# BirchKwok/lynsedb

Hardware: AMD Instinct MI355X
Metric: queries/sec, FLAT-IP 10000000x768 float32, batch=256, k=10 (higher is better)
Workload: dtype f32

## Files before the change

### include/lynse_hip.h

```cpp
#ifndef LYNSE_HIP_H
#define LYNSE_HIP_H

#include <stddef.h>
#include <stdint.h>

#ifdef __cplusplus
extern "C" {
#endif

#define LYNSE_HIP_ABI_VERSION 1

enum {
    LYNSE_OK = 0,
    LYNSE_ERR_INVALID_ARGUMENT = 1,
    LYNSE_ERR_DIMENSION_MISMATCH = 2,
    LYNSE_ERR_UNKNOWN_METRIC = 3,
    LYNSE_ERR_NOT_FINALIZED = 4,
    LYNSE_ERR_OUT_OF_MEMORY = 5,
    LYNSE_ERR_DEVICE = 6,
    LYNSE_ERR_INTERNAL = 7,
    LYNSE_ERR_INDEX_NOT_BUILT = 8,
    LYNSE_ERR_UNSUPPORTED = 9,
    LYNSE_ERR_TIMEOUT = 10
};
// ... 163 lines not shown
int lynse_hip_spann_replica_count(const lynse_hip_ivf *h, uint32_t *replica_count);
int lynse_hip_ivf_insert_f32(lynse_hip_ivf *h, const float *rows, uint64_t n);
int lynse_hip_ivf_delete_rows(lynse_hip_ivf *h, const uint64_t *row_ids, uint64_t n_ids);
int lynse_hip_ivf_assign_f32(lynse_hip_ivf *h, const float *rows, uint64_t n, uint32_t *out_assignments);
int lynse_hip_ivf_destroy(lynse_hip_ivf *h);
uint64_t lynse_hip_ivf_len(const lynse_hip_ivf *h);
uint32_t lynse_hip_ivf_nlist(const lynse_hip_ivf *h);
int lynse_hip_ivf_export(const lynse_hip_ivf *h, float *centroids, uint32_t *assignments,
                         uint64_t *offsets, uint32_t *original_ids);
int lynse_hip_ivf_set_row_map(lynse_hip_ivf *h, uint64_t stride, uint64_t offset);
int lynse_hip_ivf_set_routing(lynse_hip_ivf *h, int ivfflat_routing);
int lynse_hip_ivf_set_fused_search(lynse_hip_ivf *h, int on);
int lynse_hip_ivf_search_f32(lynse_hip_ivf *h, const float *queries, uint64_t nq, uint32_t k,
                             uint32_t nprobe, uint64_t *out_rows, float *out_dists,
                             uint32_t *out_counts);
int lynse_hip_ivf_build_device(const float *d_rows, uint64_t n, uint32_t dim, uint32_t nlist,
                               uint32_t max_iter, int metric, int l2_partitions, int device,
                               lynse_hip_ivf **out);
int lynse_hip_ivf_load_device(const float *d_rows, uint64_t n, uint32_t dim, const float *centroids,
                              uint32_t nlist, const uint32_t *assignments, int metric, int device,
                              lynse_hip_ivf **out);
int lynse_hip_ivf_search_f32_device(lynse_hip_ivf *h, const float *d_queries, uint64_t nq, uint32_t k,
                                    uint32_t nprobe, uint64_t *d_out_rows, float *d_out_dists,
                                    uint32_t *d_out_counts);
int lynse_hip_ivf_search_metric_f32(lynse_hip_ivf *h, const float *queries, uint64_t nq, uint32_t k,
                                    uint32_t nprobe, int metric, uint64_t *out_rows, float *out_dists,
                                    uint32_t *out_counts);
int lynse_hip_ivf_search_filtered_f32(lynse_hip_ivf *h, const float *queries, uint64_t nq, uint32_t k,
                                      uint32_t nprobe, const uint64_t *subset_rows, uint64_t n_subset,
                                      uint64_t *out_rows, float *out_dists, uint32_t *out_counts);
int lynse_hip_ivf_profile_enable(lynse_hip_ivf *h, int on);
int lynse_hip_ivf_profile_get(lynse_hip_ivf *h, lynse_hip_profile *out, int reset);

typedef struct lynse_hip_comm lynse_hip_comm;
int lynse_hip_comm_load_rccl(const char *path );
int lynse_hip_comm_unique_id(uint8_t *id128);
int lynse_hip_comm_create(const uint8_t *id128, int rank, int world, int device, lynse_hip_comm **out);
int lynse_hip_comm_destroy(lynse_hip_comm *c);
int lynse_hip_comm_rank(const lynse_hip_comm *c);
int lynse_hip_comm_world(const lynse_hip_comm *c);
int lynse_hip_comm_ranks_seen(lynse_hip_comm *c, int *out);
int lynse_hip_flat_search_sharded_f32_device(lynse_hip_flat *h, lynse_hip_comm *c, const float *d_queries,
                                             uint64_t nq, uint32_t k, int metric, uint64_t *d_out_rows,
                                             float *d_out_dists, uint32_t *d_out_counts);
int lynse_hip_flat_search_sharded_packed_u64_device(lynse_hip_flat *h, lynse_hip_comm *c,
                                                    const uint64_t *d_query_words, uint64_t nq, uint32_t k,
                                                    int metric, uint64_t *d_out_rows, float *d_out_dists,
                                                    uint32_t *d_out_counts);
int lynse_hip_ivf_search_sharded_f32_device(lynse_hip_ivf *h, lynse_hip_comm *c, const float *d_queries, uint64_t nq,
                                            uint32_t k, uint32_t nprobe, uint64_t *d_out_rows, float *d_out_dists,
                                            uint32_t *d_out_counts);
typedef int (*lynse_hip_reduce_fn)(void *ctx, void *buf, uint64_t count, int dtype);
int lynse_hip_ivf_kmeans_sharded(const float *rows_local, uint64_t n_local, int rows_on_device, uint64_t n_global,
                                 uint32_t rank, uint32_t world, uint32_t dim, uint32_t nlist, uint32_t max_iter, int metric,
                                 int device, lynse_hip_comm *c, lynse_hip_reduce_fn reduce, void *reduce_ctx,
                                 float *out_centroids, uint32_t *out_assignments, uint32_t *out_k);

int lynse_hip_ivf_build_sharded_device(const float *d_rows_local, uint64_t n_local, uint64_t n_global, uint32_t rank,
                                       uint32_t world, uint32_t dim, uint32_t nlist, uint32_t max_iter, int metric,
                                       int ivfflat_routing, int device, lynse_hip_comm *c, lynse_hip_reduce_fn reduce,
                                       void *reduce_ctx, lynse_hip_ivf **out);

typedef struct lynse_hip_ticket lynse_hip_ticket;
int lynse_hip_flat_search_submit_f32_device(lynse_hip_flat *h, lynse_hip_comm *c, const float *d_queries, uint64_t nq,
                                            uint32_t k, int metric, uint64_t *d_out_rows, float *d_out_dists,
                                            uint32_t *d_out_counts, lynse_hip_ticket **out);
int lynse_hip_flat_search_submit_packed_u64_device(lynse_hip_flat *h, lynse_hip_comm *c,
                                                   const uint64_t *d_query_words, uint64_t nq, uint32_t k, int metric,
                                                   uint64_t *d_out_rows, float *d_out_dists, uint32_t *d_out_counts,
                                                   lynse_hip_ticket **out);
int lynse_hip_flat_search_wait(lynse_hip_ticket *t);
int lynse_hip_set_wait_timeout_ms(uint32_t ms);

typedef struct lynse_hip_ivf_ticket lynse_hip_ivf_ticket;
int lynse_hip_ivf_search_submit_f32_device(lynse_hip_ivf *h, lynse_hip_comm *c, const float *d_queries, uint64_t nq, uint32_t k,
                                           uint32_t nprobe, uint64_t *d_out_rows, float *d_out_dists, uint32_t *d_out_counts,
                                           lynse_hip_ivf_ticket **out);
int lynse_hip_ivf_search_wait(lynse_hip_ivf_ticket *t);
int lynse_hip_ivf_ticket_stats(lynse_hip_ivf *h, uint64_t *out);

int lynse_hip_flat_coarse_scores(lynse_hip_flat *h, const float *queries, uint64_t nq, int metric, int coarse,
                                 float *out_scores, float *out_bound, int *out_form);


typedef struct lynse_hip_sparse lynse_hip_sparse;
int lynse_hip_sparse_normalize(const uint64_t *indptr , const uint32_t *indices, const float *values, uint64_t n,
                               uint64_t *out_indptr , uint32_t *out_indices, float *out_values);
int lynse_hip_sparse_create(int device, lynse_hip_sparse **out);
int lynse_hip_sparse_destroy(lynse_hip_sparse *h);
int lynse_hip_sparse_set_rows(lynse_hip_sparse *h, const uint64_t *indptr , const uint32_t *indices,
                              const float *values, uint64_t n);
int lynse_hip_sparse_len(lynse_hip_sparse *h, uint64_t *out_rows, uint64_t *out_nnz);
uint64_t lynse_hip_sparse_hbm_bytes(lynse_hip_sparse *h);
int lynse_hip_sparse_search(lynse_hip_sparse *h, const uint64_t *q_indptr , const uint32_t *q_indices,
                            const float *q_values, uint64_t nq, uint32_t k,
                            const uint64_t *bitset_words , uint64_t n_words,
                            uint64_t *out_rows , float *out_scores, uint32_t *out_counts ,
                            uint64_t *out_passed );
int lynse_hip_sparse_profile_enable(lynse_hip_sparse *h, int on);
int lynse_hip_sparse_profile_get(lynse_hip_sparse *h, lynse_hip_profile *out, int reset);


int lynse_hip_filter_tombstoned_limit(const uint64_t *ids, const float *dists, uint64_t n,
                                      const uint64_t *tombstones, uint64_t n_tombstones, uint64_t limit,
                                      uint64_t *out_ids, float *out_dists, uint64_t *out_n);
int lynse_hip_merge_row_results(const uint64_t *left_ids, const float *left_dists, uint64_t n_left,
                                const uint64_t *right_ids, const float *right_dists, uint64_t n_right,
                                uint64_t limit, int metric, uint64_t *out_ids, float *out_dists,
                                uint64_t *out_n);
int lynse_hip_encode_search_result(const uint64_t *ids, const float *dists, uint32_t n,
                                   const uint8_t *fields_json, uint32_t fields_len, uint8_t *buf,
                                   uint64_t cap, uint64_t *out_len);
int lynse_hip_decode_search_result(const uint8_t *buf, uint64_t len, uint64_t offset, uint64_t *out_ids,
                                   float *out_dists, uint32_t cap_n, uint32_t *out_n,
                                   uint64_t *fields_offset, uint32_t *fields_len, uint64_t *next_offset);

#ifdef __cplusplus
}
#endif
#endif
```

### lynsedb_amd/_lib.py

```python
from __future__ import annotations

import ctypes as C
from pathlib import Path

try:
    import torch as _torch
except ImportError:
    _torch = None

_HERE = Path(__file__).resolve().parent
LIB_PATH = _HERE / "liblynse_hip.so"

OK = 0
ERR_INVALID_ARGUMENT, ERR_DIMENSION_MISMATCH, ERR_UNKNOWN_METRIC, ERR_NOT_FINALIZED = 1, 2, 3, 4
ERR_OUT_OF_MEMORY, ERR_DEVICE, ERR_INTERNAL, ERR_INDEX_NOT_BUILT, ERR_UNSUPPORTED, ERR_TIMEOUT = 5, 6, 7, 8, 9, 10

METRIC_IP, METRIC_L2, METRIC_COSINE, METRIC_HAMMING, METRIC_JACCARD, METRIC_DICE, METRIC_TANIMOTO = range(7)
METRIC_L1, METRIC_CHEBYSHEV, METRIC_CANBERRA, METRIC_BRAY_CURTIS = 7, 8, 9, 10
IPFORM_AUTO, IPFORM_SINGLE, IPFORM_BATCH8 = 0, 1, 2


class Profile(C.Structure):
    _fields_ = [("searches", C.c_uint64), ("scan_launches", C.c_uint64), ("scan_us", C.c_double),
                ("scan_rows", C.c_uint64), ("scan_bytes", C.c_uint64), ("total_us", C.c_double),
# ... 45 lines not shown
    "lynse_hip_flat_drop_rabitq": (C.c_int, [_vp]),
    "lynse_hip_flat_search_rabitq_f32": (C.c_int, [_vp, _vp, C.c_uint64, C.c_uint32, C.c_int, C.c_uint32, _vp, _vp, _vp]),
    "lynse_hip_flat_rabitq_stage_times": (C.c_int, [_vp, _vp, C.c_int]),
    "lynse_hip_rabitq_sign_words": (C.c_int, [C.c_uint64, C.c_uint64, _vp]),
    "lynse_hip_flat_search_range_f32": (C.c_int, [_vp, _vp, C.c_uint64, _vp, C.c_uint32, C.c_int, _vp, C.c_uint64, _vp, _vp, _vp, _vp]),
    "lynse_hip_flat_set_dtype": (C.c_int, [_vp, C.c_int]),
    "lynse_hip_flat_append_f16_bits": (C.c_int, [_vp, _vp, C.c_uint64]),
    "lynse_hip_flat_search_filtered_f32": (C.c_int, [_vp, _vp, C.c_uint64, C.c_uint32, C.c_int, _vp, C.c_uint64, _vp, _vp, _vp]),
    "lynse_hip_flat_search_filtered_bitset_f32": (C.c_int, [_vp, _vp, C.c_uint64, C.c_uint32, C.c_int, _vp, C.c_uint64, _vp, _vp, _vp]),
    "lynse_hip_flat_search_f32_device": (C.c_int, [_vp, _vp, C.c_uint64, C.c_uint32, C.c_int, _vp, _vp, _vp, _vp]),
    "lynse_hip_flat_search_packed_u64": (C.c_int, [_vp, _vp, C.c_uint64, C.c_uint32, C.c_int, _vp, _vp, _vp]),
    "lynse_hip_flat_search_packed_u64_device": (C.c_int, [_vp, _vp, C.c_uint64, C.c_uint32, C.c_int, _vp, _vp, _vp, _vp]),
    "lynse_hip_flat_profile_enable": (C.c_int, [_vp, C.c_int]),
    "lynse_hip_flat_profile_get": (C.c_int, [_vp, C.POINTER(Profile), C.c_int]),
    "lynse_hip_flat_coarse_state": (C.c_int, [_vp, C.POINTER(C.c_int), _u64p]),
    "lynse_hip_flat_bpm_rows": (C.c_uint64, [_vp]),
    "lynse_hip_flat_prepare": (C.c_int, [_vp, C.c_int, C.c_uint64]),
    "lynse_hip_flat_hbm_bytes": (C.c_uint64, [_vp]),
    "lynse_hip_flat_set_fused_search": (C.c_int, [_vp, C.c_int]),
    "lynse_hip_flat_set_plan": (C.c_int, [_vp, C.c_uint32, C.c_uint32, C.c_uint32]),
    "lynse_hip_compute_distance": (C.c_int, [_vp, _vp, C.c_uint32, C.c_int, C.c_int, _f32p]),
    "lynse_hip_top_k_search": (C.c_int, [_vp, _vp, C.c_uint64, C.c_uint32, C.c_uint32, C.c_int, C.c_int, _vp, _vp, _u32p]),
    "lynse_hip_pack_binary_f32": (C.c_int, [_vp, C.c_uint64, C.c_uint32, C.c_int, _vp]),
    "lynse_hip_merge_topk": (C.c_int, [_vp, _vp, _vp, C.c_uint32, C.c_uint32, C.c_uint32, C.c_int, _vp, _vp, _u32p]),
    "lynse_hip_merge_topk_device": (C.c_int, [_vp, C.c_uint64, C.c_uint64, C.c_uint64, C.c_uint64, C.c_uint32,
                                              C.c_uint64, C.c_uint32, C.c_int, _vp, _vp, _vp, _vp]),
    "lynse_hip_ivf_build": (C.c_int, [_vp, C.c_uint64, C.c_uint32, C.c_uint32, C.c_uint32, C.c_int, C.c_int, C.c_int, C.POINTER(_vp)]),
    "lynse_hip_ivf_load": (C.c_int, [_vp, C.c_uint64, C.c_uint32, _vp, C.c_uint32, _vp, C.c_int, C.c_int, C.POINTER(_vp)]),
    "lynse_hip_ivf_load_binary": (C.c_int, [_vp, C.c_uint64, C.c_uint32, _vp, C.c_uint32, _vp, C.c_int, _vp, C.c_int, C.POINTER(_vp)]),
    "lynse_hip_ivf_thresholds": (C.c_int, [_vp, _vp, C.POINTER(C.c_int)]),
    "lynse_hip_ivf_destroy": (C.c_int, [_vp]),
    "lynse_hip_ivf_len": (C.c_uint64, [_vp]),
    "lynse_hip_ivf_nlist": (C.c_uint32, [_vp]),
    "lynse_hip_ivf_export": (C.c_int, [_vp, _vp, _vp, _vp, _vp]),
    "lynse_hip_ivf_set_row_map": (C.c_int, [_vp, C.c_uint64, C.c_uint64]),
    "lynse_hip_ivf_set_routing": (C.c_int, [_vp, C.c_int]),
    "lynse_hip_ivf_set_fused_search": (C.c_int, [_vp, C.c_int]),
    "lynse_hip_ivf_search_f32": (C.c_int, [_vp, _vp, C.c_uint64, C.c_uint32, C.c_uint32, _vp, _vp, _vp]),
    "lynse_hip_ivf_build_device": (C.c_int, [_vp, C.c_uint64, C.c_uint32, C.c_uint32, C.c_uint32, C.c_int, C.c_int, C.c_int, C.POINTER(_vp)]),
    "lynse_hip_ivf_load_device": (C.c_int, [_vp, C.c_uint64, C.c_uint32, _vp, C.c_uint32, _vp, C.c_int, C.c_int, C.POINTER(_vp)]),
    "lynse_hip_ivf_search_f32_device": (C.c_int, [_vp, _vp, C.c_uint64, C.c_uint32, C.c_uint32, _vp, _vp, _vp]),
    "lynse_hip_ivf_search_metric_f32": (C.c_int, [_vp, _vp, C.c_uint64, C.c_uint32, C.c_uint32, C.c_int, _vp, _vp, _vp]),
    "lynse_hip_ivf_search_filtered_f32": (C.c_int, [_vp, _vp, C.c_uint64, C.c_uint32, C.c_uint32, _vp, C.c_uint64, _vp, _vp, _vp]),
    "lynse_hip_ivf_profile_enable": (C.c_int, [_vp, C.c_int]),
    "lynse_hip_filter_tombstoned_limit": (C.c_int, [_vp, _vp, C.c_uint64, _vp, C.c_uint64, C.c_uint64, _vp, _vp, C.POINTER(C.c_uint64)]),
    "lynse_hip_merge_row_results": (C.c_int, [_vp, _vp, C.c_uint64, _vp, _vp, C.c_uint64, C.c_uint64, C.c_int, _vp, _vp, C.POINTER(C.c_uint64)]),
    "lynse_hip_encode_search_result": (C.c_int, [_vp, _vp, C.c_uint32, _vp, C.c_uint32, _vp, C.c_uint64, C.POINTER(C.c_uint64)]),
    "lynse_hip_decode_search_result": (C.c_int, [_vp, C.c_uint64, C.c_uint64, _vp, _vp, C.c_uint32, C.POINTER(C.c_uint32),
                                                C.POINTER(C.c_uint64), C.POINTER(C.c_uint32), C.POINTER(C.c_uint64)]),
    "lynse_hip_ivf_profile_get": (C.c_int, [_vp, C.POINTER(Profile), C.c_int]),
    "lynse_hip_ivf_insert_f32": (C.c_int, [_vp, _vp, C.c_uint64]),
    "lynse_hip_ivf_search_sharded_f32_device": (C.c_int, [_vp, _vp, _vp, C.c_uint64, C.c_uint32, C.c_uint32, _vp, _vp, _vp]),
    "lynse_hip_ivf_delete_rows": (C.c_int, [_vp, _vp, C.c_uint64]),
    "lynse_hip_ivf_assign_f32": (C.c_int, [_vp, _vp, C.c_uint64, _vp]),
    "lynse_hip_ivf_build_sq8": (C.c_int, [_vp, C.c_uint64, C.c_uint32, C.c_uint32, C.c_uint32, C.c_int, C.c_int, C.POINTER(_vp)]),
    "lynse_hip_ivf_load_sq8": (C.c_int, [_vp, C.c_uint64, C.c_uint32, _vp, C.c_uint32, _vp, _vp, _vp, C.c_int, C.c_int, C.POINTER(_vp)]),
    "lynse_hip_ivf_sq8_params": (C.c_int, [_vp, _vp, _vp]),
    "lynse_hip_ivf_sq8_stage_times": (C.c_int, [_vp, _vp, C.c_int]),
    "lynse_hip_spann_build": (C.c_int, [_vp, C.c_uint64, C.c_uint32, C.c_uint32, C.c_uint32, C.c_int, C.c_uint32, C.c_int, C.c_int, C.POINTER(_vp)]),
    "lynse_hip_spann_load": (C.c_int, [_vp, C.c_uint64, C.c_uint32, _vp, C.c_uint32, _vp, _vp, C.c_uint32, C.c_int, _vp, _vp, C.c_int, C.POINTER(_vp)]),
    "lynse_hip_spann_postings": (C.c_int, [_vp, _vp, _vp, _vp]),
    "lynse_hip_spann_replica_count": (C.c_int, [_vp, _vp]),
    "lynse_hip_comm_load_rccl": (C.c_int, [C.c_char_p]),
    "lynse_hip_comm_unique_id": (C.c_int, [_vp]),
    "lynse_hip_comm_create": (C.c_int, [_vp, C.c_int, C.c_int, C.c_int, C.POINTER(_vp)]),
    "lynse_hip_comm_destroy": (C.c_int, [_vp]),
    "lynse_hip_comm_rank": (C.c_int, [_vp]),
    "lynse_hip_comm_world": (C.c_int, [_vp]),
    "lynse_hip_comm_ranks_seen": (C.c_int, [_vp, C.POINTER(C.c_int)]),
    "lynse_hip_flat_search_sharded_f32_device": (C.c_int, [_vp, _vp, _vp, C.c_uint64, C.c_uint32, C.c_int, _vp, _vp, _vp]),
    "lynse_hip_flat_search_sharded_packed_u64_device": (C.c_int, [_vp, _vp, _vp, C.c_uint64, C.c_uint32, C.c_int, _vp, _vp, _vp]),
    "lynse_hip_flat_search_submit_f32_device": (C.c_int, [_vp, _vp, _vp, C.c_uint64, C.c_uint32, C.c_int, _vp, _vp, _vp, C.POINTER(_vp)]),
    "lynse_hip_flat_search_submit_packed_u64_device": (C.c_int, [_vp, _vp, _vp, C.c_uint64, C.c_uint32, C.c_int, _vp, _vp, _vp, C.POINTER(_vp)]),
    "lynse_hip_flat_search_wait": (C.c_int, [_vp]),
    "lynse_hip_set_wait_timeout_ms": (C.c_int, [C.c_uint32]),
    "lynse_hip_ivf_search_submit_f32_device": (C.c_int, [_vp, _vp, _vp, C.c_uint64, C.c_uint32, C.c_uint32, _vp, _vp, _vp, C.POINTER(_vp)]),
    "lynse_hip_ivf_search_wait": (C.c_int, [_vp]),
    "lynse_hip_ivf_ticket_stats": (C.c_int, [_vp, _vp]),
    "lynse_hip_ivf_kmeans_sharded": (C.c_int, [_vp, C.c_uint64, C.c_int, C.c_uint64, C.c_uint32, C.c_uint32, C.c_uint32, C.c_uint32, C.c_uint32, C.c_int, C.c_int,
                                              _vp, _vp, _vp, _vp, _vp, C.POINTER(C.c_uint32)]),
    "lynse_hip_ivf_build_sharded_device": (C.c_int, [_vp, C.c_uint64, C.c_uint64, C.c_uint32, C.c_uint32, C.c_uint32, C.c_uint32, C.c_uint32, C.c_int, C.c_int, C.c_int,
                                                    _vp, _vp, _vp, C.POINTER(_vp)]),
    "lynse_hip_flat_coarse_scores": (C.c_int, [_vp, _vp, C.c_uint64, C.c_int, C.c_int, _vp, _vp, C.POINTER(C.c_int)]),
    "lynse_hip_sparse_normalize": (C.c_int, [_vp, _vp, _vp, C.c_uint64, _vp, _vp, _vp]),
    "lynse_hip_sparse_create": (C.c_int, [C.c_int, C.POINTER(_vp)]),
    "lynse_hip_sparse_destroy": (C.c_int, [_vp]),
    "lynse_hip_sparse_set_rows": (C.c_int, [_vp, _vp, _vp, _vp, C.c_uint64]),
    "lynse_hip_sparse_len": (C.c_int, [_vp, _u64p, _u64p]),
    "lynse_hip_sparse_hbm_bytes": (C.c_uint64, [_vp]),
    "lynse_hip_sparse_search": (C.c_int, [_vp, _vp, _vp, _vp, C.c_uint64, C.c_uint32, _vp, C.c_uint64, _vp, _vp, _vp, _vp]),
    "lynse_hip_sparse_profile_enable": (C.c_int, [_vp, C.c_int]),
    "lynse_hip_sparse_profile_get": (C.c_int, [_vp, C.POINTER(Profile), C.c_int]),
}

REDUCE_FN = C.CFUNCTYPE(C.c_int, C.c_void_p, C.c_void_p, C.c_uint64, C.c_int)

if not LIB_PATH.exists():
    raise ImportError(
        f"{LIB_PATH} is missing: the HIP extension has not been built and lynsedb_amd has no CPU "
        "fallback. Run `make -C lynsedb_amd/csrc` (hipcc --offload-arch=gfx950).")

lib = C.CDLL(str(LIB_PATH))
for _name, (_res, _args) in SIGNATURES.items():
    _fn = getattr(lib, _name)
    _fn.restype = _res
    _fn.argtypes = _args

if lib.lynse_hip_abi_version() != 1:
    raise ImportError("liblynse_hip.so ABI version mismatch; rebuild it")


class LynseHipError(RuntimeError):
    def __init__(self, code: int, message: str):
        super().__init__(message)
        self.code = code


class LynseUnsupportedError(LynseHipError, NotImplementedError):
    """LYNSE_ERR_UNSUPPORTED: valid in the reference, outside what this library implements (e.g. the metric 'l1')."""


def last_error() -> str:
    buf = C.create_string_buffer(1024)
    lib.lynse_hip_last_error(buf, 1024)
    return buf.value.decode("utf-8", "replace")


def check(code: int) -> None:
    if code == OK:
        return
    msg = last_error() or f"lynse_hip error {code}"
    if code in (ERR_INVALID_ARGUMENT, ERR_DIMENSION_MISMATCH, ERR_UNKNOWN_METRIC):
        raise ValueError(msg)
    if code == ERR_OUT_OF_MEMORY:
        raise MemoryError(msg)
    if code == ERR_UNSUPPORTED:
        raise LynseUnsupportedError(code, msg)
    if code == ERR_TIMEOUT:
        raise TimeoutError(msg)
    raise LynseHipError(code, msg)


def device_count() -> int:
    n = C.c_int(0)
    rc = lib.lynse_hip_device_count(C.byref(n))
    return n.value if rc == OK else 0
```

### lynsedb_amd/core.py

```python
from __future__ import annotations

import ctypes as C
import os
from pathlib import Path
from typing import Iterable, Optional, Sequence

import numpy as np

from . import _lib
from ._lib import check, lib

_METRIC_IS_BINARY = {_lib.METRIC_HAMMING, _lib.METRIC_JACCARD, _lib.METRIC_DICE, _lib.METRIC_TANIMOTO}


def visible_devices() -> list:
    v = os.environ.get("LYNSE_HIP_DEVICES", "").strip()
    if v:
        try:
            devs = [int(x) for x in v.split(",") if x.strip() != ""]
        except ValueError:
            raise ValueError(f"LYNSE_HIP_DEVICES must be a comma-separated list of device ordinals, got {v!r}") from None
        if not devs or min(devs) < 0:
            raise ValueError(f"LYNSE_HIP_DEVICES must name at least one non-negative device ordinal, got {v!r}")
        return devs
# ... 472 lines not shown
        rows, dists, counts = self.search_filtered_batch_arrays(q.reshape(1, -1), k, metric, subset_rows)
        c = int(counts[0])
        return rows[0, :c].astype(np.uint32), dists[0, :c].copy()

    def search_packed_arrays(self, query_words, k: int, metric):
        m = metric if isinstance(metric, int) else metric_from_str(metric)
        qw = np.ascontiguousarray(query_words, dtype=np.uint64)
        if qw.ndim == 1:
            qw = qw.reshape(1, -1)
        nq, k = qw.shape[0], int(k)
        rows = np.empty((nq, max(k, 1)), np.uint64)
        dists = np.empty((nq, max(k, 1)), np.float32)
        counts = np.zeros(nq, np.uint32)
        check(lib.lynse_hip_flat_search_packed_u64(self._h, _ptr(qw), nq, k, m, _ptr(rows), _ptr(dists), _ptr(counts)))
        return rows[:, :k], dists[:, :k], counts

    def search(self, query, k: int = 10, metric: str = "ip"):
        m = metric_from_str(metric)
        q = _f32(query, 1, "query")
        rows, dists, counts = self.search_batch_arrays(q.reshape(1, -1), k, m)
        c = int(counts[0])
        return rows[0, :c].astype(np.uint32), dists[0, :c].copy()

    def batch_search(self, queries, k: int = 10, metric: str = "ip"):
        m = metric_from_str(metric)
        rows, dists, counts = self.search_batch_arrays(queries, k, m)
        return [(rows[i, :int(c)].astype(np.uint32), dists[i, :int(c)].copy()) for i, c in enumerate(counts)]

    def search_device(self, d_queries, k: int, metric, d_rows, d_dists, d_counts, stream=None):
        m = metric if isinstance(metric, int) else metric_from_str(metric)
        nq = d_queries.shape[0]
        _sync_producer(d_queries)
        check(lib.lynse_hip_flat_search_f32_device(
            self._h, C.c_void_p(d_queries.data_ptr()), nq, int(k), m, C.c_void_p(d_rows.data_ptr()),
            C.c_void_p(d_dists.data_ptr()), C.c_void_p(d_counts.data_ptr()),
            C.c_void_p(stream) if stream else None))

    def search_packed_device(self, d_qwords, k: int, metric, d_rows, d_dists, d_counts, stream=None):
        m = metric if isinstance(metric, int) else metric_from_str(metric)
        nq = d_qwords.shape[0]
        _sync_producer(d_qwords)
        check(lib.lynse_hip_flat_search_packed_u64_device(
            self._h, C.c_void_p(d_qwords.data_ptr()), nq, int(k), m, C.c_void_p(d_rows.data_ptr()),
            C.c_void_p(d_dists.data_ptr()), C.c_void_p(d_counts.data_ptr()),
            C.c_void_p(stream) if stream else None))

    def search_submit(self, d_queries, k: int, metric, d_rows, d_dists, d_counts, comm=None) -> "SearchTicket":
        m = metric if isinstance(metric, int) else metric_from_str(metric)
        if _lib.METRIC_HAMMING <= m <= _lib.METRIC_TANIMOTO and d_queries.is_floating_point():
            if comm is not None:
                raise ValueError("sharded searches of a binary metric take packed u64 query words")
            self.search_device(d_queries, k, m, d_rows, d_dists, d_counts)
            return SearchTicket(None, None)
        _sync_producer(d_queries)
        t = C.c_void_p()
        fn = lib.lynse_hip_flat_search_submit_packed_u64_device if _lib.METRIC_HAMMING <= m <= _lib.METRIC_TANIMOTO else lib.lynse_hip_flat_search_submit_f32_device
        check(fn(self._h, comm, C.c_void_p(d_queries.data_ptr()), d_queries.shape[0], int(k), m, C.c_void_p(d_rows.data_ptr()),
                 C.c_void_p(d_dists.data_ptr()), C.c_void_p(d_counts.data_ptr()), C.byref(t)))
        return SearchTicket(t, (d_queries, d_rows, d_dists, d_counts))

    def profile_enable(self, on=True) -> None:
        check(lib.lynse_hip_flat_profile_enable(self._h, int(on)))

    def profile_get(self, reset: bool = True) -> dict:
        p = _lib.Profile()
        check(lib.lynse_hip_flat_profile_get(self._h, C.byref(p), 1 if reset else 0))
        return {f: getattr(p, f) for f, _ in _lib.Profile._fields_}

    def prepare(self, metric, nq: int = 256) -> None:
        m = metric if isinstance(metric, int) else metric_from_str(metric)
        check(lib.lynse_hip_flat_prepare(self._h, m, int(nq)))

    def hbm_bytes(self) -> int:
        return int(lib.lynse_hip_flat_hbm_bytes(self._h))

    def coarse_scores(self, queries, metric, coarse: str = "i8"):
        q = np.ascontiguousarray(np.atleast_2d(queries), dtype=np.float32)
        m = metric if isinstance(metric, int) else metric_from_str(metric)
        scores = np.empty((q.shape[0], len(self)), np.float32)
        bound = np.empty(q.shape[0], np.float32)
        form = C.c_int(0)
        check(lib.lynse_hip_flat_coarse_scores(self._h, _ptr(q), q.shape[0], m, 1 if coarse in ("i8", "int8", 1, True) else 0, _ptr(scores), _ptr(bound), C.byref(form)))
        return scores, bound, form.value

    def coarse_state(self) -> dict:
        strikes, rows = C.c_int(0), C.c_uint64(0)
        check(lib.lynse_hip_flat_coarse_state(self._h, C.byref(strikes), C.byref(rows)))
        return {"i8c_strikes": strikes.value, "sq8_rows": rows.value, "bpm_rows": int(lib.lynse_hip_flat_bpm_rows(self._h))}


class SearchTicket:

    def __init__(self, handle, keep, ivf: bool = False):
        self._t, self._keep, self._ivf = handle, keep, ivf

    def wait(self) -> None:
        t, self._t = self._t, None
        if t is not None:
            try:
                check((lib.lynse_hip_ivf_search_wait if self._ivf else lib.lynse_hip_flat_search_wait)(t))
            finally:
                self._keep = None

    def __del__(self):
        try:
            self.wait()
        except Exception:
            pass


class IvfFlatIndex:

    def __init__(self, handle, dim: int, sq8: bool = False):
        self._h = handle
        self._dim = dim
        self._sq8 = sq8

    def profile_enable(self, on=True) -> None:
        check(lib.lynse_hip_ivf_profile_enable(self._h, int(on)))

    def profile_get(self, reset: bool = True) -> dict:
        p = _lib.Profile()
        check(lib.lynse_hip_ivf_profile_get(self._h, C.byref(p), 1 if reset else 0))
        return {f: getattr(p, f) for f, _ in _lib.Profile._fields_}

    def __del__(self):
        h, self._h = getattr(self, "_h", None), None
        if h:
            lib.lynse_hip_ivf_destroy(h)

    @staticmethod
    def build(path, data, dim: int, n_partitions: int = 256, n_iters: int = 20, metric: str = "ip",
              device: Optional[int] = None, l2_partitions: bool = True, quantizer: Optional[str] = None) -> "IvfFlatIndex":
        m = metric if isinstance(metric, int) else metric_from_str(metric)
        a = _f32(data, 2, "data")
        if a.shape[1] != dim:
            raise ValueError(f"data dimension mismatch: expected {dim}, got {a.shape[1]}")
        if n_partitions <= 0:
            raise IOError("IVF partition count must be greater than zero")
        if quantizer is not None and str(quantizer).lower() != "sq8":
            raise NotImplementedError(f"IVF quantizer {quantizer!r} is outside this path (sq8 and the binary metrics are built)")
        if a.shape[0] < n_partitions and quantizer is None:
            raise IOError("IVF requires at least as many vectors as partitions")
        h = C.c_void_p()
        dev = default_device() if device is None else int(device)
        if quantizer is not None:
            check(lib.lynse_hip_ivf_build_sq8(_ptr(a), a.shape[0], dim, n_partitions, n_iters, m, dev, C.byref(h)))
            return IvfFlatIndex(h, dim, sq8=True)
        if m >= 3:
            l2_partitions = False
        check(lib.lynse_hip_ivf_build(_ptr(a), a.shape[0], dim, n_partitions, n_iters, m,
                                      1 if l2_partitions else 0, dev, C.byref(h)))
        return IvfFlatIndex(h, dim)

    @staticmethod
    def build_device(d_rows, dim: int, n_partitions: int = 256, n_iters: int = 20, metric: str = "ip",
                     l2_partitions: bool = True) -> "IvfFlatIndex":
        m = metric if isinstance(metric, int) else metric_from_str(metric)
        if d_rows.dim() != 2 or d_rows.shape[1] != dim or not d_rows.is_contiguous():
            raise ValueError("rows must be a contiguous (n, dim) float32 device tensor")
        _sync_producer(d_rows)
        h = C.c_void_p()
        check(lib.lynse_hip_ivf_build_device(C.c_void_p(d_rows.data_ptr()), d_rows.shape[0], dim, n_partitions, n_iters, m,
                                             1 if l2_partitions else 0, d_rows.device.index or 0, C.byref(h)))
        return IvfFlatIndex(h, dim)

# ... 1003 lines not shown
```

### lynsedb_amd/csrc/kernels.h

```cpp
#pragma once

#include "common.h"
#include <utility>

namespace lynse {

typedef _Float16 half8 __attribute__((ext_vector_type(8)));
typedef _Float16 half4 __attribute__((ext_vector_type(4)));
typedef float f32x16 __attribute__((ext_vector_type(16)));
typedef uint32_t u32x4 __attribute__((ext_vector_type(4)));
typedef float f32x4 __attribute__((ext_vector_type(4)));

#define LY_INF __builtin_huge_valf()

__device__ __forceinline__ float hsum8(float a) {
    float t = __fadd_rn(a, __shfl_xor(a, 4, 8));
    t = __fadd_rn(t, __shfl_xor(t, 1, 8));
    t = __fadd_rn(t, __shfl_xor(t, 2, 8));
    return t;
}

__device__ __forceinline__ float exact_score_f16seq(int metric, const float* __restrict__ q, const float* __restrict__ v_as_f32,
                                                    uint32_t D, int g) {
    const _Float16* __restrict__ v = reinterpret_cast<const _Float16*>(v_as_f32);
// ... 1956 lines not shown
                    volatile uint32_t* flag = reinterpret_cast<volatile uint32_t*>(const_cast<char*>(stv));
                    bool ok = fs_grid_sync(gs, gs + 2, gridDim.x, flag, tid);
                    if (stamp && tid == 0) stamp[2] = __builtin_amdgcn_s_memtime();
                    if (ok) {
                        for (uint32_t q = blockIdx.x; q < ea->nq; q += gridDim.x)
                            fused_sample_threshold<NW * 64>(ea->cand + (size_t)q * ea->cap, gridDim.x * (2 * WR * 2), ea->k, ea->marg2[q], METRIC, ea->ip_form,
                                                            ea->Qf + (size_t)q * ea->D, ea->V, ea->ld, ea->D, ea->thr_out + q, const_cast<char*>(stv),
                                                            const_cast<char*>(stq), tid);
                        if (stamp && tid == 0) stamp[3] = __builtin_amdgcn_s_memtime();
                        ok = fs_grid_sync(gs + 1, gs + 2, gridDim.x, flag, tid);
                        if (stamp && tid == 0) stamp[4] = __builtin_amdgcn_s_memtime();
                    }
                    if (!ok) return;
                    load_qc_thr(ea->thr, ea->nq);
                    if (stamp && tid == 0) stamp[5] = __builtin_amdgcn_s_memtime();
                }
            }
            if constexpr (!DEFER) s_in_tile = 0;
            tile += gridDim.x;
        }
        if constexpr (DEFER) {
            if (g == G) break;
            if (tile_done) load_frags(0, 0);
            ly_static_for<HK / 16 - 1>([&](auto kkc) {
                constexpr int kk = decltype(kkc)::value, cur = kk & 1;
                load_frags(kk + 1, cur ^ 1);
                __builtin_amdgcn_sched_barrier(0);
                ly_static_for<TR>([&](auto ic) {
                    group_at(std::integral_constant<int, cur>{}, ic);
                    slot_pieces(TR + kk * TR + decltype(ic)::value);
                });
                __builtin_amdgcn_sched_barrier(0);
            });
            q_advance();
            v_advance();
            pend_done = ++s_in_tile == a.nslab;
            if (pend_done) s_in_tile = 0;
        }
        if (timing) {
            asm volatile("" ::"v"(acc[0][0][0]));
            const unsigned long long t = __builtin_amdgcn_s_memtime(); t_comp += t - tp; tp = t;
        }
    }
#ifdef LYNSE_EXPERIMENTS
    if (timing && lane == 0) {
        unsigned long long* o = a.dbg + ((size_t)blockIdx.x * NW + wave) * 4;
        o[0] = t_wait; o[1] = t_bar; o[2] = (t_iq << 32) | (t_iv & 0xffffffffull); o[3] = t_comp;
    }
#endif
    if (!TILED) {
        const EpiArgsPtr ea = epi_args();
        if (FS && (ea->debug_flags & 128) && tid == 0) reinterpret_cast<unsigned long long*>(ea->gsync + 64)[(size_t)blockIdx.x * 8 + 6] = __builtin_amdgcn_s_memtime();
        if (ea->seg && (hi == 0 || DENSE)) {
#pragma unroll
            for (int j = 0; j < TQ; ++j) {
                const uint32_t n = qchunk + wq * (TQ * 32) + j * 32 + l32;
                const uint32_t sgm = DENSE ? (blockIdx.x * WR + wr) * 2 + hi : blockIdx.x * WR + wr;
                if (n < ea->nq) ea->segcnt[(size_t)n * ea->nseg + sgm] = (uint8_t)((segpk >> (8 * j)) & 0xffu);
            }
        }
    }
    asm volatile("s_waitcnt vmcnt(0)" ::: "memory");
}

template <typename T>
__global__ void __launch_bounds__(256) k_sq8_minmax(const T* __restrict__ V, uint32_t ld, uint32_t D, uint64_t n,
                                                    uint32_t* __restrict__ omin, uint32_t* __restrict__ omax,
                                                    const float* __restrict__ row_scale = nullptr) {
    const uint64_t rows_per_block = (n + gridDim.y - 1) / gridDim.y;
    const uint64_t r0 = (uint64_t)blockIdx.y * rows_per_block, r1 = r0 + rows_per_block < n ? r0 + rows_per_block : n;
    const uint32_t d = blockIdx.x * 256 + threadIdx.x;
    if (d >= D) return;
    float mn = LY_INF, mx = -LY_INF;
    for (uint64_t r = r0; r < r1; ++r) {
        const float v = row_scale ? __fmul_rn((float)V[r * ld + d], row_scale[r]) : (float)V[r * ld + d];
        if (v < mn) mn = v;
        if (v > mx) mx = v;
    }
    atomicMin(&omin[d], f32_to_ord(mn));
    atomicMax(&omax[d], f32_to_ord(mx));
}

__global__ void __launch_bounds__(256) k_sq8_scales(const uint32_t* __restrict__ omin, const uint32_t* __restrict__ omax, uint32_t D,
                                                    float* __restrict__ mins, float* __restrict__ scales) {
    const uint32_t d = blockIdx.x * 256 + threadIdx.x;
    if (d >= D) return;
    const float mn = ord_to_f32(omin[d]), mx = ord_to_f32(omax[d]);
    const float range = __fsub_rn(mx, mn);
    mins[d] = mn;
    scales[d] = range > 1e-30f ? __fdiv_rn(255.0f, range) : 0.0f;
}

__global__ void __launch_bounds__(256) k_mm_changed(const uint32_t* __restrict__ now, const uint32_t* __restrict__ before, uint32_t n, uint32_t* __restrict__ flag) {
    const uint32_t i = blockIdx.x * 256 + threadIdx.x;
    if (i < n && now[i] != before[i]) atomicOr(flag, 1u);
}

__global__ void __launch_bounds__(256) k_vec_minmax(const float* __restrict__ x, uint64_t n, uint32_t* __restrict__ omin, uint32_t* __restrict__ omax,
                                                    uint32_t ncopies) {
    float mn = LY_INF, mx = -LY_INF;
    for (uint64_t i = (uint64_t)blockIdx.x * blockDim.x + threadIdx.x; i < n; i += (uint64_t)gridDim.x * blockDim.x) {
        const float v = x[i];
        if (v < mn) mn = v;
        if (v > mx) mx = v;
    }
    for (int o = 32; o > 0; o >>= 1) { mn = fminf(mn, __shfl_xor(mn, o, 64)); mx = fmaxf(mx, __shfl_xor(mx, o, 64)); }
    if ((threadIdx.x & 63) == 0)
        for (uint32_t j = 0; j < ncopies; ++j) { atomicMin(omin + j, f32_to_ord(mn)); atomicMax(omax + j, f32_to_ord(mx)); }
}

__device__ __forceinline__ int sq8_code(float v, float mn, float sc) {
    float q = roundf(__fmul_rn(__fsub_rn(v, mn), sc));
    if (!(q == q)) return 0;
    q = q < 0.0f ? 0.0f : (q > 255.0f ? 255.0f : q);
    return (int)q;
}

template <typename T>
__global__ void __launch_bounds__(256) k_sq8_quantize(const T* __restrict__ V, uint32_t ld, uint32_t D, uint64_t n,
                                                      const float* __restrict__ mins, const float* __restrict__ scales,
                                                      int8_t* __restrict__ out, uint32_t ld8, int* __restrict__ sums,
                                                      int* __restrict__ sums2, uint32_t* __restrict__ stats,
                                                      const float* __restrict__ extra_col = nullptr, uint32_t n_extra = 0,
                                                      const float* __restrict__ row_scale = nullptr) {
    const int lane = threadIdx.x & 63;
    const uint64_t wave = ((uint64_t)blockIdx.x * blockDim.x + threadIdx.x) >> 6;
    const uint64_t nwaves = ((uint64_t)gridDim.x * blockDim.x) >> 6;
    uint32_t a1max = 0, a2max = 0, nonfinite = 0;
    float e2max = 0.0f;
    for (uint64_t row = wave; row < n; row += nwaves) {
        int s1 = 0, s2 = 0, l1 = 0;
        float e2 = 0.0f, e1 = 0.0f;
        for (uint32_t d = lane; d < ld8; d += 64) {
            int c = 0;
            if (d < D || (extra_col && d < D + n_extra)) {
                const float v = d < D ? (row_scale ? __fmul_rn((float)V[row * ld + d], row_scale[row]) : (float)V[row * ld + d]) : extra_col[row];
                if (!(fabsf(v) < LY_INF)) nonfinite += 1;
                const int code = sq8_code(v, mins[d], scales[d]);
                c = code - 128;
                s1 += c;
                s2 += c * c;
                l1 += c < 0 ? -c : c;
                const float e = __fsub_rn(__fmul_rn(__fsub_rn(v, mins[d]), scales[d]), (float)code);
                const float ea = fabsf(e);
                if (ea == ea) { e2 = __fmaf_rn(e, e, e2); e1 += ea; }
            }
            out[row * ld8 + d] = (int8_t)c;
        }
        for (int o = 32; o > 0; o >>= 1) {
            s1 += __shfl_xor(s1, o, 64); s2 += __shfl_xor(s2, o, 64); l1 += __shfl_xor(l1, o, 64);
            e2 += __shfl_xor(e2, o, 64); e1 += __shfl_xor(e1, o, 64);
        }
        if (lane == 0 && sums) { sums[row] = s1; sums2[row] = s2; }
        a1max = a1max > (uint32_t)l1 ? a1max : (uint32_t)l1;
        a2max = a2max > (uint32_t)s2 ? a2max : (uint32_t)s2;
        const float e2b = (e2 + 1.22e-4f * e1 + (float)(D + n_extra) * 3.8e-9f) * 1.00002f;
        e2max = e2b > e2max ? e2b : e2max;
    }
    for (int o = 32; o > 0; o >>= 1) nonfinite += __shfl_xor(nonfinite, o, 64);
    if (lane == 0 && stats) {
        atomicMax(&stats[0], a1max);
        if (nonfinite) atomicAdd(&stats[1], nonfinite);
        atomicMax(&stats[2], a2max);
        atomicMax(&stats[3], __float_as_uint(e2max));
    }
}

__global__ void __launch_bounds__(256) k_sq8_prep_queries(const float* __restrict__ Q, uint32_t D, uint32_t qpad, uint32_t nslab,
                                                          const float* __restrict__ mins, const float* __restrict__ scales,
                                                          int8_t* __restrict__ img, float* __restrict__ qconst, float* __restrict__ thr,
                                                          uint32_t* __restrict__ count, uint32_t* __restrict__ overflow, int ip) {
    __shared__ int red[2][4];
    const uint32_t q = blockIdx.x;
    const int tid = threadIdx.x, lane = tid & 63, wave = tid >> 6;
    int s1 = 0, s2 = 0;
    const uint32_t total = nslab * 128;
    for (uint32_t i = tid; i < total; i += 256) {
        int c = 0;
        if (i < D) {
            c = sq8_code(Q[(size_t)q * D + i], mins[i], scales[i]) - 128;
            s1 += c;
            s2 += c * c;
        }
        const uint32_t s = i / 128, k = i % 128, l = k >> 4, e = k & 15, p = l ^ ((q >> 1) & 7);
        img[(((size_t)s * qpad + q) * 8 + p) * 16 + e] = (int8_t)c;
    }
    for (int o = 32; o > 0; o >>= 1) { s1 += __shfl_xor(s1, o, 64); s2 += __shfl_xor(s2, o, 64); }
    if (lane == 0) { red[0][wave] = s1; red[1][wave] = s2; }
    __syncthreads();
    if (tid == 0) {
        s1 = red[0][0] + red[0][1] + red[0][2] + red[0][3];
        s2 = red[1][0] + red[1][1] + red[1][2] + red[1][3];
        const int c = ip ? 128 * s1 + 16384 * (int)D : s2;
        qconst[q] = __builtin_bit_cast(float, c);
        thr[q] = ip ? -LY_INF : LY_INF;
        count[q] = 0u;
        overflow[q] = 0u;
    }
}

struct I8cPrepArgs {
    const float* Q;
    uint32_t D, qpad, nslab;
    uint32_t nq;
    const float *mins, *scales;
    uint32_t a1;
    uint32_t a2sq;
    float eps2;
    float vmax;
    int8_t* img;
    float *sq, *bq, *marg2, *thr;
    uint32_t *count, *overflow;
    uint32_t* gsync;
    int aug;
    int l2n;
    int cosine;
    const int8_t* codes;
    uint32_t ld8, n_rows, tile_rows, dyn_ks, seed_rows;
    int *dyn_thr, *dyn_slot, *dyn_marg;
};

__global__ void __launch_bounds__(256) k_i8c_prep_queries(I8cPrepArgs a) {
    __shared__ double red[5][4];
    __shared__ float s_sq;
    __shared__ int s_slot[32];
    extern __shared__ __attribute__((aligned(16))) int8_t s_u[];
    const uint32_t q = blockIdx.x;
    const int tid = threadIdx.x, lane = tid & 63, wave = tid >> 6;
    if (a.nq && q >= a.nq) {
        for (uint32_t i = tid; i < a.nslab * 128; i += 256) a.img[((size_t)(i / 128) * a.qpad + q) * 128 + (i % 128)] = 0;
        return;
    }
    const float* qv = a.Q + (size_t)q * a.D;
    const uint32_t DA = a.D + (uint32_t)a.aug;
    double qrn = 1.0;
    if (a.cosine) {
        __shared__ double rs[4];
        double t = 0.0;
        for (uint32_t i = tid; i < a.D; i += 256) { const double o = (double)qv[i]; t += o * o; }
        for (int o = 32; o > 0; o >>= 1) t += __shfl_xor(t, o, 64);
        if (lane == 0) rs[wave] = t;
        __syncthreads();
        t = (rs[0] + rs[1]) + (rs[2] + rs[3]);
        qrn = t > 0.0 ? 1.0 / sqrt(t) : 0.0;
        __syncthreads();
    }
    auto qel = [&](uint32_t i) -> double {
        if (a.cosine) return (double)qv[i] * qrn;
        if (!a.aug) return (double)qv[i];
        return i < a.D ? 2.0 * (double)qv[i] : -1.0 / (double)a.aug;
    };
    double wmax = 0.0, sw = 0.0, swabs = 0.0, sqm = 0.0, s2 = 0.0, sw2 = 0.0;
    for (uint32_t i = tid; i < DA; i += 256) {
        const double x = qel(i);
        const float sc = a.scales[i];
        const double w = sc > 0.0f ? x / (double)sc : 0.0;
        wmax = fmax(wmax, fabs(w));
        sw += w;
        swabs += fabs(w);
        sw2 += w * w;
        sqm += x * (double)a.mins[i];
        if (i < a.D) { const double o = (double)qv[i]; s2 += o * o; }
    }
    for (int o = 32; o > 0; o >>= 1) {
        wmax = fmax(wmax, __shfl_xor(wmax, o, 64));
        sw += __shfl_xor(sw, o, 64);
        swabs += __shfl_xor(swabs, o, 64);
        sqm += __shfl_xor(sqm, o, 64);
        s2 += __shfl_xor(s2, o, 64);
        sw2 += __shfl_xor(sw2, o, 64);
    }
    __shared__ double red2[2][4];
    if (lane == 0) { red[0][wave] = wmax; red[1][wave] = sw; red[2][wave] = swabs; red[3][wave] = sqm; red[4][wave] = s2; red2[0][wave] = sw2; }
    __syncthreads();
    if (tid == 0) {
        wmax = fmax(fmax(red[0][0], red[0][1]), fmax(red[0][2], red[0][3]));
        float sq = 1.0f;
        if (wmax > 0.0 && wmax < 1.0e30) {
            sq = (float)(wmax / 127.0);
            if ((double)sq * 127.0 < wmax) sq = nextafterf(sq, LY_INF);
            if (!(sq > 0.0f)) sq = 1.1754944e-38f;
        }
        s_sq = sq;
    }
    __syncthreads();
    const double inv = 1.0 / (double)s_sq;
    const uint32_t total = a.nslab * 128;
    double eta2 = 0.0;
    for (uint32_t i = tid; i < total; i += 256) {
        int u = 0;
        if (i < DA) {
            const float sc = a.scales[i];
            const double w = sc > 0.0f ? qel(i) / (double)sc : 0.0;
            const double t = w * inv;
            double r = rint(t);
            r = r < -127.0 ? -127.0 : (r > 127.0 ? 127.0 : r);
            u = (r == r) ? (int)r : 0;
            const double eta = t - (double)u;
            if (eta == eta) eta2 += eta * eta;
        }
        const uint32_t s = i / 128, k = i % 128, l = k >> 4, e = k & 15, p = l ^ ((q >> 1) & 7);
        a.img[(((size_t)s * a.qpad + q) * 8 + p) * 16 + e] = (int8_t)u;
        if (a.dyn_thr) s_u[i] = (int8_t)u;
    }
    for (int o = 32; o > 0; o >>= 1) eta2 += __shfl_xor(eta2, o, 64);
    if (lane == 0) red2[1][wave] = eta2;
    __syncthreads();
    if (tid == 0) {
        wmax = fmax(fmax(red[0][0], red[0][1]), fmax(red[0][2], red[0][3]));
        sw = (red[1][0] + red[1][1]) + (red[1][2] + red[1][3]);
        swabs = (red[2][0] + red[2][1]) + (red[2][2] + red[2][3]);
        sqm = (red[3][0] + red[3][1]) + (red[3][2] + red[3][3]);
        s2 = (red[4][0] + red[4][1]) + (red[4][2] + red[4][3]);
        sw2 = (red2[0][0] + red2[0][1]) + (red2[0][2] + red2[0][3]);
        eta2 = (red2[1][0] + red2[1][1]) + (red2[1][2] + red2[1][3]);
        const float sq = s_sq;
        const double bq = sqm + 128.0 * sw - (a.aug ? s2 : 0.0) - (a.cosine ? 1.0 : 0.0);
        const float bqf = (float)bq;
        const double a1 = (double)a.a1;
        const double gam = 10.0 * (double)a.D * 5.9604645e-8;
        const double ref_term = a.cosine ? 9.0 * ((double)a.D + 8.0) * 5.9604645e-8
                                : a.aug  ? 8.0 * ((double)a.D + 8.0) * 5.9604645e-8 * (s2 + (double)a.vmax * (double)a.vmax)
                                         : gam * sqrt(s2) * (double)a.vmax;
        double tq = 0.5001 * (double)sq * a1, tr = 0.5001 * swabs;
        if (a.a2sq) { const double c2 = 1.0002 * (double)sq * sqrt(eta2) * sqrt((double)a.a2sq); tq = c2 < tq ? c2 : tq; }
        if (a.eps2 > 0.0f) { const double c2 = 1.0002 * sqrt(sw2) * sqrt((double)a.eps2); tr = c2 < tr ? c2 : tr; }
        double E = tr + tq + 2.5e-7 * (fabs(bq) + (a.cosine ? 1.0 : fabs(s2)) + 127.0 * (double)sq * a1) + ref_term;
        float bq_out = bqf;
        if (a.l2n) {
            const double vm2 = (double)a.vmax * (double)a.vmax;
            E = 2.0 * (tr + tq) + 5.0e-7 * (2.0 * fabs(bq) + s2 + vm2 + 2.0 * 127.0 * (double)sq * a1) +
                8.0 * ((double)a.D + 8.0) * 5.9604645e-8 * (s2 + vm2);
            bq_out = (float)(s2 - 2.0 * bq);
        }
        E *= 1.02;
        if (!(wmax < 1.0e30) || !(E == E) || E > 3.0e38) E = 3.0e38;
        a.sq[q] = sq;
        a.bq[q] = bq_out;
        a.marg2[q] = (float)(2.0 * E);
        a.thr[q] = a.l2n ? LY_INF : -LY_INF;
        a.count[q] = 0u;
        a.overflow[q] = 0u;
        if (q == 0 && a.gsync) { a.gsync[0] = 0u; a.gsync[1] = 0u; a.gsync[2] = 0u; }
        if (a.dyn_thr) {
            const double delta = 2.4e-7 * (fabs(bq) + 127.0 * (double)sq * a1);
            double md = ceil((2.0 * E + 2.0 * delta) / (double)sq) + 1.0;
            if (!(md < 1073741824.0)) md = 1073741824.0;
            a.dyn_marg[q] = (int)md;
        }
    }
    __syncthreads();
    if (a.dyn_thr) {
        const uint32_t ks = a.dyn_ks, rt = a.tile_rows;
        const uint32_t ntiles = (a.n_rows + rt - 1) / rt;
        if (tid < 32) s_slot[tid] = -2147483647 - 1;
        __syncthreads();
        const uint32_t per = a.seed_rows / ks;
        for (uint32_t i = tid; i < per * ks; i += 256) {
            const uint32_t p = i % ks, m = i / ks;
            const uint32_t up = (ntiles > p) ? (ntiles - p + ks - 1) / ks : 0u;
            if (!up) continue;
            const uint32_t u_idx = (uint32_t)(((uint64_t)m * up) / per);
            uint64_t row = (uint64_t)(p + ks * u_idx) * rt + (i * 7u) % rt;
            if (row >= a.n_rows) row = (uint64_t)(p + ks * u_idx) * rt;
            const int8_t* src = a.codes + row * a.ld8;
            int dot = 0;
            const uint32_t nb = a.nslab * 128;
            for (uint32_t d = 0; d < nb && d < a.ld8; d += 16) {
                typedef int i32x4_t __attribute__((ext_vector_type(4)));
                const i32x4_t c = *reinterpret_cast<const i32x4_t*>(src + d);
                const i32x4_t w = *reinterpret_cast<const i32x4_t*>(s_u + d);
#if defined(__HIP_DEVICE_COMPILE__)
                dot = __builtin_amdgcn_sdot4(c[0], w[0], dot, false);
                dot = __builtin_amdgcn_sdot4(c[1], w[1], dot, false);
                dot = __builtin_amdgcn_sdot4(c[2], w[2], dot, false);
                dot = __builtin_amdgcn_sdot4(c[3], w[3], dot, false);
#else
                (void)c; (void)w;
#endif
            }
            atomicMax(&s_slot[p], dot);
        }
        __syncthreads();
        if (tid < 32) a.dyn_slot[(size_t)q * 32 + tid] = tid < (int)ks ? s_slot[tid] : 2147483647;
        if (tid == 0) {
            int mn = 2147483647;
            for (uint32_t j = 0; j < ks; ++j) mn = s_slot[j] < mn ? s_slot[j] : mn;
            a.dyn_thr[q] = mn;
        }
    }
}

__global__ void __launch_bounds__(256) k_bits_to_fp4(const uint64_t* __restrict__ P, uint32_t W, uint32_t D, uint64_t r0, uint64_t r1,
                                                     uint8_t* __restrict__ out, uint32_t ldb) {
    const uint32_t cpr = ldb / 16;
    const uint64_t total = (r1 - r0) * cpr;
    for (uint64_t i = (uint64_t)blockIdx.x * blockDim.x + threadIdx.x; i < total; i += (uint64_t)gridDim.x * blockDim.x) {
        const uint64_t r = r0 + i / cpr;
        const uint32_t c0 = (uint32_t)(i % cpr) * 32;
        const uint32_t w = c0 >> 6;
        const uint32_t bits = w < W ? (uint32_t)(P[r * W + w] >> (c0 & 63)) : 0u;
        u32x4 v;
#pragma unroll
        for (int j = 0; j < 4; ++j) {
            uint32_t word = 0;
#pragma unroll
            for (int b = 0; b < 8; ++b) {
                const uint32_t col = c0 + j * 8 + b;
                const uint32_t nib = col < D ? (((bits >> (j * 8 + b)) & 1u) ? 0x2u : 0xAu) : 0u;
                word |= nib << (4 * b);
// ... 1634 lines not shown
```

### lynsedb_amd/csrc/lynse_hip.hip

```cpp
#include <algorithm>
#include <atomic>
#include <chrono>
#include <cmath>
#include <cstdio>
#include <cstring>
#include <functional>
#include <condition_variable>
#include <memory>
#include <mutex>
#include <shared_mutex>
#include <string>
#include <thread>
#include <type_traits>
#include <vector>
#include <sched.h>

#include "kernels.h"
#include "scan_qs.h"
#include "scan_qh.h"
#include "ivf.h"
#include "pq.h"
#include "rabitq.h"
#include "range.h"
#include "additive.h"
// ... 179 lines not shown
    uint32_t* h_hdr = nullptr;
    uint8_t* h_out = nullptr;
    unsigned long long* pool_total = nullptr;
    uint32_t* gsync = nullptr;
    int* dyn = nullptr;
    uint64_t* small_part = nullptr;
    uint32_t* small_ticket = nullptr;
    void release() {
        if (h_hdr) (void)hipHostFree(h_hdr);
        if (h_out) (void)hipHostFree(h_out);
        for (void* p : {(void*)cand, (void*)candB, (void*)segcnt, (void*)count, (void*)thr, (void*)qinv, (void*)qn2,
                        (void*)qrinv, (void*)marg2, (void*)Q16, (void*)Qf, (void*)QW, (void*)QWp, (void*)out_rows,
                        (void*)out_dists, (void*)out_counts, (void*)pool_total, (void*)small_part, (void*)small_ticket, (void*)gsync, (void*)dyn})
            if (p) (void)hipFree(p);
        *this = Workspace();
    }
};

struct PqState;
struct RbqState;
struct RangeState;

struct lynse_hip_flat {
    uint32_t dim = 0, ld = 0, words = 0;
    int device = 0;
    int num_cu = 256;
    std::shared_mutex rw;
    struct Ctx {
        hipStream_t stream = nullptr;
        Workspace ws;
        std::vector<hipEvent_t> ev_pool;
        uint32_t* d_mask = nullptr;
        uint64_t mask_words = 0;
        uint64_t* d_subset = nullptr;
        uint64_t subset_cap = 0;
    };
    static constexpr int MAX_CTX = 8;
    Ctx ctx[MAX_CTX];
    int n_ctx = 4;
    std::mutex ctx_mu;
    std::condition_variable ctx_cv;
    uint32_t ctx_busy = 0;
    std::mutex prof_mu;
    std::atomic<int> inflight{0};

    uint64_t n = 0, capacity = 0;
    float* rows = nullptr;
    _Float16* rows_h = nullptr;
    bool shadow_alias = false;
    _Float16* rows16 = nullptr;
    uint32_t ld16 = 0;
    uint64_t n16 = 0, cap16 = 0;
    float sv16 = 0.0f;
    uint64_t n_packed = 0, packed_capacity = 0;
    uint64_t* packed = nullptr;
    bool packed_only = false;

    uint64_t n_stats = 0;
    uint64_t stats_capacity = 0;
    float *vn2 = nullptr, *vrinv = nullptr;
    uint32_t* d_stats = nullptr;
    int rows_integer = 0, rows_nonneg = 0;
    float amax = 0.f, vmax = 0.f, vmin = 0.f, sv = 1.f;
    int cos_degenerate = 0;

    uint64_t row_stride = 1, row_offset = 0;
    int ip_form = LYNSE_IPFORM_AUTO;
    int no_fused = 0;
    uint32_t qchunk = 256;
    int dtype = LYNSE_DTYPE_F32;
    uint32_t stage0_rows = 4096, growth = 8, cap = 16384;

    int8_t* sq8 = nullptr;
    uint32_t ld8 = 0;
    uint64_t n_sq8 = 0, sq8_cap = 0;
    float *sq8_mins = nullptr, *sq8_scales = nullptr;
    int *sq8_sum = nullptr, *sq8_sum2 = nullptr;
    uint32_t* sq8_mm = nullptr;
    uint32_t* sq8_stats = nullptr;
    uint32_t* sq8_mm_prev = nullptr;
    uint32_t sq8_a1 = 0, sq8_a2sq = 0;
    float sq8_eps2 = 0.0f;
    bool sq8_finite = false;
    int8_t* sq8a = nullptr;
    uint32_t ld8a = 0, aug_cols = 1;
    uint64_t n_sq8a = 0, sq8a_cap = 0;
    float *sq8a_mins = nullptr, *sq8a_scales = nullptr;
    uint32_t *sq8a_mm = nullptr, *sq8a_stats = nullptr;
    uint32_t sq8a_a1 = 0, sq8a_a2sq = 0;
    float sq8a_eps2 = 0.0f;
    bool sq8a_finite = false;
    std::atomic<int> i8c_strikes_l2{0};
    int8_t* sq8c = nullptr;
    uint64_t n_sq8c = 0, sq8c_cap = 0;
    float *sq8c_mins = nullptr, *sq8c_scales = nullptr;
    uint32_t *sq8c_mm = nullptr, *sq8c_stats = nullptr;
    uint32_t sq8c_a1 = 0, sq8c_a2sq = 0;
    float sq8c_eps2 = 0.0f;
    bool sq8c_finite = false;
    std::atomic<int> i8c_strikes_cos{0};
    std::atomic<int> i8c_strikes{0};
    uint8_t* bpm = nullptr;
    uint32_t ld_bpm = 0;
    uint64_t n_bpm = 0, bpm_cap = 0;
    bool bpm_failed = false;
    _Float16* g_rows16 = nullptr;
    float *g_vn2 = nullptr, *g_vrinv = nullptr;
    uint32_t* g_ids32 = nullptr;
    uint64_t g_cap = 0;

    PqState* pq = nullptr;
    RbqState* rbq = nullptr;
    RangeState* range = nullptr;

    std::atomic<bool> profiling{false};
    std::atomic<uint32_t> prof_rate{1};
    std::atomic<uint32_t> prof_seq{0};
    lynse_hip_profile prof{};
};

static void pq_release(lynse_hip_flat* h);
static void rbq_release(lynse_hip_flat* h);
static void range_release(lynse_hip_flat* h);

static inline bool is_f16(const lynse_hip_flat* h) { return h->dtype == LYNSE_DTYPE_F16; }
static inline const float* score_rows(const lynse_hip_flat* h) { return is_f16(h) ? reinterpret_cast<const float*>(h->rows_h) : h->rows; }
static inline uint32_t score_ld(const lynse_hip_flat* h) { return is_f16(h) ? h->ld16 / 2 : h->ld; }

static thread_local bool tl_prof = false;
static thread_local int tl_ctx_slot = 0;
static inline lynse_hip_flat::Ctx& cur(lynse_hip_flat* h) { return h->ctx[tl_ctx_slot]; }
static inline const lynse_hip_flat::Ctx& cur(const lynse_hip_flat* h) { return h->ctx[tl_ctx_slot]; }

struct CtxLease {
    lynse_hip_flat* h = nullptr;
    int slot = 0, prev = 0;
    int acquire(lynse_hip_flat* hh) {
        h = hh;
        {
            std::unique_lock<std::mutex> lk(h->ctx_mu);
            for (;;) {
                int s = 0;
                while (s < h->n_ctx && ((h->ctx_busy >> s) & 1u)) ++s;
                if (s < h->n_ctx) { slot = s; h->ctx_busy |= 1u << s; break; }
                if (h->inflight.load(std::memory_order_acquire) >= h->n_ctx) {
                    h = nullptr;
                    return set_error(LYNSE_ERR_INVALID_ARGUMENT, "every search context of the handle is held by a ticket: wait for one first (LYNSE_HIP_CONTEXTS)");
                }
                h->ctx_cv.wait(lk);
            }
        }
        prev = tl_ctx_slot;
        tl_ctx_slot = slot;
        if (!h->ctx[slot].stream && hipStreamCreateWithFlags(&h->ctx[slot].stream, hipStreamNonBlocking) != hipSuccess) {
            release();
            return set_error(LYNSE_ERR_DEVICE, "hipStreamCreate failed");
        }
        return LYNSE_OK;
    }
    void release() {
        if (!h) return;
        tl_ctx_slot = prev;
        {
            std::lock_guard<std::mutex> lk(h->ctx_mu);
            h->ctx_busy &= ~(1u << slot);
        }
// ... 6 lines not shown

static int writer_lock(lynse_hip_flat* h, std::unique_lock<std::shared_mutex>& lk) {
    lk = std::unique_lock<std::shared_mutex>(h->rw);
    if (h->inflight.load(std::memory_order_acquire) != 0) {
        lk.unlock();
        return set_error(LYNSE_ERR_INVALID_ARGUMENT, "searches are in flight on this handle: wait for the outstanding tickets first");
    }
    return LYNSE_OK;
}
#define LY_WRITER(h, lk) std::unique_lock<std::shared_mutex> lk; LY_TRY(writer_lock((h), lk))

static bool profile_begin_search(lynse_hip_flat* h) {
    const uint32_t rate = h->prof_rate.load();
    tl_prof = h->profiling.load() && (rate <= 1 || h->prof_seq.fetch_add(1) % rate == 0);
    return tl_prof;
}

static int use_device(const lynse_hip_flat* h) {
    LY_HIP(hipSetDevice(h->device));
    return LYNSE_OK;
}

static uint32_t round_up(uint32_t x, uint32_t m) { return (x + m - 1) / m * m; }

extern "C" int lynse_hip_flat_create(uint32_t dim, int device, lynse_hip_flat** out) {
    if (!out) return set_error(LYNSE_ERR_INVALID_ARGUMENT, "out is NULL");
    *out = nullptr;
    if (dim == 0) return set_error(LYNSE_ERR_INVALID_ARGUMENT, "dimension must be greater than zero");
    int ndev = 0;
    LY_TRY(lynse_hip_device_count(&ndev));
    if (ndev <= 0) return set_error(LYNSE_ERR_DEVICE, "no HIP device available (this library has no CPU fallback)");
    if (device < 0 || device >= ndev) return set_error(LYNSE_ERR_INVALID_ARGUMENT, "device ordinal out of range");
    LY_HIP(hipSetDevice(device));
    auto* h = new lynse_hip_flat();
    h->dim = dim;
    h->ld = round_up(dim, 4);
    h->ld16 = round_up(dim, 8);
    if (((dim >= 48 && dim < 64) || (dim >= 96 && dim < 128)) && env_on("LYNSE_HIP_SHADOW_PAD", true))
        h->ld16 = round_up(dim, 64);
    h->ld8 = round_up(dim, 16);
    h->ld_bpm = round_up(dim, 256) / 2;
    h->ld8a = round_up(dim + 1, 128);
    while (h->aug_cols * 2 <= 32 && dim + h->aug_cols * 2 <= h->ld8a) h->aug_cols *= 2;
    h->words = (dim + 63) / 64;
    h->device = device;
    hipDeviceProp_t prop;
    if (hipGetDeviceProperties(&prop, device) == hipSuccess && prop.multiProcessorCount > 0)
        h->num_cu = prop.multiProcessorCount;
    if (const char* ce = env_str("LYNSE_HIP_CONTEXTS")) h->n_ctx = std::max(1, std::min((int)lynse_hip_flat::MAX_CTX, atoi(ce)));
    hipError_t e = hipStreamCreateWithFlags(&h->ctx[0].stream, hipStreamNonBlocking);
    if (e != hipSuccess) {
        delete h;
        return set_error(LYNSE_ERR_DEVICE, std::string("hipStreamCreate: ") + hipGetErrorString(e));
    }
    e = hipMalloc(&h->d_stats, 5 * sizeof(uint32_t));
    if (e != hipSuccess) {
        (void)hipStreamDestroy(cur(h).stream);
        delete h;
        return set_error(LYNSE_ERR_OUT_OF_MEMORY, "hipMalloc(stats)");
    }
    const uint32_t init[5] = {0u, 0u, 0x7f800000u, 0u, 0u};
    (void)h2d_done(h->d_stats, init, sizeof init);
    *out = h;
    return LYNSE_OK;
}

extern "C" int lynse_hip_flat_destroy(lynse_hip_flat* h) {
    if (!h) return LYNSE_OK;
    (void)hipSetDevice(h->device);
    pq_release(h);
    rbq_release(h);
    range_release(h);
    for (auto& c : h->ctx) {
        if (c.stream) (void)hipStreamSynchronize(c.stream);
        c.ws.release();
        if (c.d_mask) (void)hipFree(c.d_mask);
        if (c.d_subset) (void)hipFree(c.d_subset);
        for (auto e : c.ev_pool) (void)hipEventDestroy(e);
    }
    if (h->shadow_alias) h->rows16 = nullptr;
    for (void* p : {(void*)h->rows, (void*)h->rows_h, (void*)h->rows16, (void*)h->packed, (void*)h->vn2, (void*)h->vrinv, (void*)h->d_stats,
                    (void*)h->g_rows16, (void*)h->g_vn2, (void*)h->g_vrinv, (void*)h->g_ids32,
                    (void*)h->bpm, (void*)h->sq8c, (void*)h->sq8c_mins, (void*)h->sq8c_scales, (void*)h->sq8c_mm, (void*)h->sq8c_stats, (void*)h->sq8a, (void*)h->sq8a_mins, (void*)h->sq8a_scales, (void*)h->sq8a_mm, (void*)h->sq8a_stats,
                    (void*)h->sq8, (void*)h->sq8_mins, (void*)h->sq8_scales, (void*)h->sq8_sum, (void*)h->sq8_sum2, (void*)h->sq8_mm, (void*)h->sq8_stats, (void*)h->sq8_mm_prev})
        if (p) (void)hipFree(p);
    for (auto& c : h->ctx)
        if (c.stream) (void)hipStreamDestroy(c.stream);
    delete h;
    return LYNSE_OK;
}

static int realloc_rows_h(lynse_hip_flat* h, uint64_t cap) {
    _Float16* nr = nullptr;
    LY_HIP(hipMalloc(&nr, (size_t)cap * h->ld16 * sizeof(_Float16) + 256));
    if (h->rows_h && h->n)
        LY_HIP(hipMemcpyAsync(nr, h->rows_h, (size_t)h->n * h->ld16 * sizeof(_Float16), hipMemcpyDeviceToDevice, cur(h).stream));
    LY_HIP(hipStreamSynchronize(cur(h).stream));
    if (h->rows_h) (void)hipFree(h->rows_h);
    h->rows_h = nr;
    h->capacity = cap;
    if (h->shadow_alias) { h->rows16 = h->rows_h; h->cap16 = cap; }
    return LYNSE_OK;
}

static int grow_rows(lynse_hip_flat* h, uint64_t need) {
    if (need <= h->capacity) return LYNSE_OK;
    uint64_t cap = std::max<uint64_t>(need, h->capacity + h->capacity / 2);
    cap = std::max<uint64_t>(cap, 1024);
    if (is_f16(h)) return realloc_rows_h(h, cap);
    float* nr = nullptr;
    LY_HIP(hipMalloc(&nr, (size_t)cap * h->ld * sizeof(float)));
    if (h->rows && h->n)
        LY_HIP(hipMemcpyAsync(nr, h->rows, (size_t)h->n * h->ld * sizeof(float), hipMemcpyDeviceToDevice, cur(h).stream));
    LY_HIP(hipStreamSynchronize(cur(h).stream));
    if (h->rows) (void)hipFree(h->rows);
    h->rows = nr;
    h->capacity = cap;
    return LYNSE_OK;
}

static int grow_packed(lynse_hip_flat* h, uint64_t need) {
    if (need <= h->packed_capacity) return LYNSE_OK;
    uint64_t cap = std::max<uint64_t>(need, h->packed_capacity + h->packed_capacity / 2);
    cap = std::max<uint64_t>(cap, 1024);
    uint64_t* np = nullptr;
    LY_HIP(hipMalloc(&np, (size_t)cap * h->words * sizeof(uint64_t)));
    if (h->packed && h->n_packed)
        LY_HIP(hipMemcpyAsync(np, h->packed, (size_t)h->n_packed * h->words * 8, hipMemcpyDeviceToDevice, cur(h).stream));
    LY_HIP(hipStreamSynchronize(cur(h).stream));
    if (h->packed) (void)hipFree(h->packed);
    h->packed = np;
    h->packed_capacity = cap;
    return LYNSE_OK;
}

extern "C" int lynse_hip_flat_reserve(lynse_hip_flat* h, uint64_t rows) {
    if (!h) return set_error(LYNSE_ERR_INVALID_ARGUMENT, "handle is NULL");
    LY_WRITER(h, lk);
    LY_TRY(use_device(h));
    if (rows > 0xfffffff0ull) return set_error(LYNSE_ERR_INVALID_ARGUMENT, "row count exceeds the u32 id capacity of one shard");
    if (h->packed_only) return grow_packed(h, rows);
    if (rows > h->capacity && is_f16(h)) return realloc_rows_h(h, rows);
    if (rows > h->capacity) {
        float* nr = nullptr;
        LY_HIP(hipMalloc(&nr, (size_t)rows * h->ld * sizeof(float)));
        if (h->rows && h->n)
            LY_HIP(hipMemcpyAsync(nr, h->rows, (size_t)h->n * h->ld * sizeof(float), hipMemcpyDeviceToDevice, cur(h).stream));
        LY_HIP(hipStreamSynchronize(cur(h).stream));
        if (h->rows) (void)hipFree(h->rows);
        h->rows = nr;
        h->capacity = rows;
    }
    return LYNSE_OK;
}

static int copy_rows_kernel(lynse_hip_flat* h, float* dst, uint32_t dp, const float* src, uint32_t sp, uint32_t width,
                            uint64_t n, int zero_pad) {
    const uint64_t total = n * (zero_pad ? dp : width);
    const uint32_t blocks = (uint32_t)std::min<uint64_t>((total + 255) / 256, (uint64_t)h->num_cu * 32);
    hipLaunchKernelGGL(k_copy_rows, dim3(std::max<uint32_t>(blocks, 1)), dim3(256), 0, cur(h).stream, dst, dp, src, sp, width, n, zero_pad);
    LY_HIP(hipGetLastError());
    return LYNSE_OK;
}

static int decode_rows_kernel(lynse_hip_flat* h, float* dst, uint32_t dp, uint64_t first, uint64_t n) {
    const uint64_t total = n * h->dim;
    hipLaunchKernelGGL(k_f16_to_f32_rows, dim3((uint32_t)std::max<uint64_t>(1, std::min<uint64_t>((total + 255) / 256, (uint64_t)h->num_cu * 32))), dim3(256), 0,
// ... 984 lines not shown
    h->n16 = h->n;
    h->sv16 = h->sv;
    return LYNSE_OK;
}

static int launch_scan_binary(const BinArgs& a, int metric, uint32_t grid, size_t lds, hipStream_t st) {
    constexpr size_t LDS_MAX = 160 * 1024 - 64;
    switch (metric) {
    case M_HAMMING: LY_TRY(ensure_lds<k_scan_binary<0>>(LDS_MAX)); hipLaunchKernelGGL(k_scan_binary<0>, dim3(grid), dim3(256), lds, st, a); break;
    case M_DICE: LY_TRY(ensure_lds<k_scan_binary<2>>(LDS_MAX)); hipLaunchKernelGGL(k_scan_binary<2>, dim3(grid), dim3(256), lds, st, a); break;
    default: LY_TRY(ensure_lds<k_scan_binary<1>>(LDS_MAX)); hipLaunchKernelGGL(k_scan_binary<1>, dim3(grid), dim3(256), lds, st, a); break;
    }
    LY_HIP(hipGetLastError());
    return LYNSE_OK;
}

static int launch_scan_binary_wide(const BinArgs& a, int metric, uint32_t grid, hipStream_t st) {
    switch (metric) {
    case M_HAMMING: hipLaunchKernelGGL(k_scan_binary_wide<0>, dim3(grid), dim3(256), 0, st, a); break;
    case M_DICE: hipLaunchKernelGGL(k_scan_binary_wide<2>, dim3(grid), dim3(256), 0, st, a); break;
    default: hipLaunchKernelGGL(k_scan_binary_wide<1>, dim3(grid), dim3(256), 0, st, a); break;
    }
    LY_HIP(hipGetLastError());
    return LYNSE_OK;
}

template <int KIND>
static int launch_scan_binary_rows_k(const BinArgs& a, uint32_t grid, hipStream_t st) {
    auto lds = [](int wcap) { return (size_t)4 * 64 * bin_rows_stride(wcap); };
    if (a.W & 1u) {
        if (a.W <= 1) return launch_lds<k_scan_binary_rows<KIND, 1, true>>(grid, 256, lds(1), st, a);
        if (a.W <= 4) return launch_lds<k_scan_binary_rows<KIND, 4, true>>(grid, 256, lds(4), st, a);
        if (a.W <= 8) return launch_lds<k_scan_binary_rows<KIND, 8, true>>(grid, 256, lds(8), st, a);
        if (a.W <= 16) return launch_lds<k_scan_binary_rows<KIND, 16, true>>(grid, 256, lds(16), st, a);
        if (a.W <= 32) return launch_lds<k_scan_binary_rows<KIND, 32, true>>(grid, 256, lds(32), st, a);
        return launch_lds<k_scan_binary_rows<KIND, 64, true>>(grid, 256, lds(64), st, a);
    }
    if (a.W <= 2) return launch_lds<k_scan_binary_rows<KIND, 2, false>>(grid, 256, lds(2), st, a);
    if (a.W <= 4) return launch_lds<k_scan_binary_rows<KIND, 4, false>>(grid, 256, lds(4), st, a);
    if (a.W <= 8) return launch_lds<k_scan_binary_rows<KIND, 8, false>>(grid, 256, lds(8), st, a);
    if (a.W <= 16) return launch_lds<k_scan_binary_rows<KIND, 16, false>>(grid, 256, lds(16), st, a);
    if (a.W <= 32) return launch_lds<k_scan_binary_rows<KIND, 32, false>>(grid, 256, lds(32), st, a);
    return launch_lds<k_scan_binary_rows<KIND, 64, false>>(grid, 256, lds(64), st, a);
}
static int launch_scan_binary_rows(const BinArgs& a, int metric, uint32_t grid, hipStream_t st) {
    switch (metric) {
    case M_HAMMING: return launch_scan_binary_rows_k<0>(a, grid, st);
    case M_DICE: return launch_scan_binary_rows_k<2>(a, grid, st);
    default: return launch_scan_binary_rows_k<1>(a, grid, st);
    }
}

constexpr size_t SEL_LDS_MAX = 150 * 1024;
static inline uint32_t sel_lds_bytes(uint32_t cap, uint32_t nq = 0) {
    if (nq > 512) return cap * 8u;
    static const size_t extra = (size_t)env_int("LYNSE_HIP_SEL_SCRATCH_KB", 48) * 1024;
    return (uint32_t)std::min<size_t>((size_t)cap * 8 + extra, SEL_LDS_MAX);
}

static int get_event(lynse_hip_flat* h, size_t idx, hipEvent_t* out) {
    while (cur(h).ev_pool.size() <= idx) {
        hipEvent_t e;
        LY_HIP(hipEventCreate(&e));
        cur(h).ev_pool.push_back(e);
    }
    *out = cur(h).ev_pool[idx];
    return LYNSE_OK;
}

static int dense_env_now() { return env_int("LYNSE_HIP_DENSE", -1); }
static int dense_env() { static const int v = dense_env_now(); return v; }
static int debug_flags_env() { static const int v = env_int("LYNSE_HIP_DEBUG_FLAGS", 0); return v; }
static int no_lane_max_env() { static const int v = env_int("LYNSE_HIP_NO_LANE_MAX", 0); return v; }
static bool i8c_cs_on() { static const bool v = env_on("LYNSE_HIP_I8C_CS", true); return v; }
static bool sel_stamps_on() { return env_str("LYNSE_HIP_SEL_STAMPS") != nullptr; }
static int fused_env() { static const int v = env_int("LYNSE_HIP_FUSED", 1); return v; }
#ifdef LYNSE_EXPERIMENTS
template <int DFLT>
static int scan_w16_env() { static const int v = env_int("LYNSE_HIP_SCAN_W16", DFLT); return v; }
#endif

static bool l2_plain(const lynse_hip_flat* h, uint64_t nqc, bool masked = false);
static thread_local bool tl_coarse_dump = false;
static thread_local bool tl_assign = false;

static int run_chunk(lynse_hip_flat* h, uint32_t nq, uint32_t k, uint32_t out_k, int metric, int level, hipStream_t st,
                     size_t* ev_used, std::vector<std::pair<size_t, uint64_t>>* scan_events, bool* sampled_plan,
                     const uint32_t* mask = nullptr, const uint32_t* row_ids = nullptr, bool i8c = false,
                     uint64_t* r_dst = nullptr, float* d_dst = nullptr, uint32_t* c2_dst = nullptr, uint32_t* any_ovf = nullptr,
                     const float* qsrc = nullptr, bool hdr_direct = false, bool allow_sts = true, bool* used_sts = nullptr) {
    Workspace& w = cur(h).ws;
    const float* Qf = qsrc ? qsrc : w.Qf;
    const bool binary = metric >= M_HAMMING;
    const bool asc = metric_ascending(metric);
    const bool h16 = scan_variant() == 3;
    const bool glds = scan_variant() == 0;
    const bool bin_mfma = h16 && bin_mfma_eligible(h, metric, mask != nullptr || row_ids != nullptr, nq) && h->bpm && h->n_bpm == h->n;
    if (bin_mfma) i8c = true;
    const bool l2n = i8c && !bin_mfma && metric == M_L2 && !row_ids && l2_plain(h, nq, mask != nullptr);
    const bool aug = i8c && !bin_mfma && metric == M_L2 && !l2n;
    const bool cosq = i8c && !bin_mfma && metric == M_COS;
    const int key_metric = (bin_mfma || aug || cosq) ? (int)M_IP : metric;
    const uint32_t nslab = bin_mfma ? h->ld_bpm / 128 : i8c ? ((aug ? h->dim + h->aug_cols : h->dim) + 127) / 128 : glds ? (h->dim + GL_BK - 1) / GL_BK : (h->dim + SCAN_BK - 1) / SCAN_BK;
    const bool small = nq <= SCAN_BQ_SMALL;
    const int mid_env = env_int("LYNSE_HIP_MID_TILINGS", 1);
    const bool qs_mid = env_on("LYNSE_HIP_QS_MID", true) && qs_variant() >= 1 && qs_variant() <= 3 && i8c && !bin_mfma &&
                        !small && !row_ids && h16 && !aug && qs_width_ok(h->ld8, (h->dim + 127) / 128, mask != nullptr) && !(l2n && (h->dim + 127) / 128 == 8) && nq <= 256 &&
                        (h->ld8 == 768 || nq > 64) &&
                        (!mask || (!l2n && qs_variant() != 2 && qs_masked_on()));
    const bool mid_ok = mid_env && !qs_mid && i8c && !bin_mfma && !small && !row_ids && h16 && (!mask || (aug ? h->ld8a : h->ld8) % 128 == 0);
    const bool mid64 = mid_ok && nq <= 64, mid128 = mid_ok && !mid64 && nq <= 128;
    const bool narrow = small || mid64;
    const uint32_t qpad = small ? SCAN_BQ_SMALL : mid64 ? 64u : mid128 ? 128u : round_up(nq, SCAN_BQ_LARGE);
    const uint32_t qchunks = (small || mid64 || mid128) ? 1u : qpad / SCAN_BQ_LARGE;
    if (qchunks > 1 && (binary || i8c || mask || row_ids || !h16 || h->n > w.cap || nq > w.qcap))
        return set_error(LYNSE_ERR_INTERNAL, "more than 256 queries per pass need the widened float pipeline over <= cap rows");
    int ip_form = h->ip_form;
    if (ip_form == LYNSE_IPFORM_AUTO) ip_form = h->n < 4096 ? LYNSE_IPFORM_SINGLE : LYNSE_IPFORM_BATCH8;
    if (mask || row_ids) ip_form = LYNSE_IPFORM_SINGLE;
    if (h->dtype == LYNSE_DTYPE_F16) ip_form = LYNSE_IPFORM_F16SEQ;

    LY_TRY(ensure_lds<k_select<SEL_NT>>(SEL_LDS_MAX));
    LY_TRY(ensure_lds<k_final<SEL_NT>>(SEL_LDS_MAX));
    LY_TRY(ensure_lds<k_select_final<SEL_NT>>(SEL_LDS_MAX));

    const uint32_t sts_ld8 = cosq ? h->ld8 : h->ld8;
    const bool sts = allow_sts && sts_env_on() && level == 0 && i8c && !bin_mfma && !aug && !l2n && !small && !mid64 && !mid128 && !mask && !row_ids && h16 &&
                     k >= 1 && k <= 32 && qs_variant() >= 1 && qs_variant() <= 3 && sts_ld8 == 768 && nslab == 6 && qpad == 256 && h->n >= 65536 &&
                     h->n < 0xffffff00ull && (metric == M_IP || cosq);
    if (used_sts) *used_sts = sts;
    if (bin_mfma) {
        BpmPrepArgs p{};
        p.QW = w.QW; p.W = h->words; p.D = h->dim; p.qpad = qpad; p.nslab = nslab; p.nq = nq; p.img = reinterpret_cast<uint8_t*>(w.Q16);
        p.sq = w.qinv; p.bq = w.qn2; p.marg2 = w.marg2; p.thr = w.thr; p.count = w.count; p.overflow = w.overflow;
        hipLaunchKernelGGL(k_bpm_prep_queries, dim3(qpad), dim3(256), 0, st, p);
        LY_HIP(hipGetLastError());
    } else if (binary) {
        std::vector<float> thr0(nq, INFINITY);
        LY_HIP(hipMemcpyAsync(w.thr, thr0.data(), nq * 4, hipMemcpyHostToDevice, st));
        LY_HIP(hipMemsetAsync(w.count, 0, nq * 4, st));
        LY_HIP(hipMemsetAsync(w.overflow, 0, nq * 4, st));
        LY_HIP(hipStreamSynchronize(st));
    } else if (i8c) {
        I8cPrepArgs p{};
        p.Q = Qf; p.D = h->dim; p.qpad = qpad; p.nslab = nslab; p.nq = nq; p.mins = aug ? h->sq8a_mins : (cosq ? h->sq8c_mins : h->sq8_mins);
        p.scales = aug ? h->sq8a_scales : (cosq ? h->sq8c_scales : h->sq8_scales);
        p.a1 = aug ? h->sq8a_a1 : (cosq ? h->sq8c_a1 : h->sq8_a1); p.vmax = h->vmax;
        if (i8c_cs_on()) { p.a2sq = aug ? h->sq8a_a2sq : (cosq ? h->sq8c_a2sq : h->sq8_a2sq); p.eps2 = aug ? h->sq8a_eps2 : (cosq ? h->sq8c_eps2 : h->sq8_eps2); } p.cosine = cosq ? 1 : 0; p.img = reinterpret_cast<int8_t*>(w.Q16); p.aug = aug ? (int)h->aug_cols : 0; p.l2n = l2n ? 1 : 0;
        p.sq = w.qinv; p.bq = w.qn2; p.marg2 = w.marg2; p.thr = w.thr; p.count = w.count; p.overflow = w.overflow;
        p.gsync = w.gsync;
        if (sts) {
            p.codes = cosq ? h->sq8c : h->sq8; p.ld8 = sts_ld8; p.n_rows = (uint32_t)h->n; p.tile_rows = 64; p.dyn_ks = k;
            p.seed_rows = std::min<uint32_t>(1024u, 32u * k);
            p.dyn_thr = w.dyn; p.dyn_marg = w.dyn + w.qcap; p.dyn_slot = w.dyn + 2 * (size_t)w.qcap;
        }
        hipLaunchKernelGGL(k_i8c_prep_queries, dim3(qpad), dim3(256), sts ? (size_t)nslab * 128 : 0, st, p);
        LY_HIP(hipGetLastError());
    } else {
        PrepArgs p{};
        p.Q = Qf; p.D = h->dim; p.nq = nq; p.qpad = qpad; p.nslab = nslab; p.metric = metric; p.layout = glds ? 1 : (h16 ? 2 : 0);
        p.sv = h->sv; p.vmax = h->vmax; p.vmin = h->vmin; p.cos_degenerate = h->cos_degenerate; p.rows_integer = h->rows_integer; p.rows_nonneg = h->rows_nonneg; p.amax_v = h->amax;
        p.Q16 = w.Q16; p.qinv = w.qinv; p.qn2 = w.qn2; p.qrinv = w.qrinv; p.marg2 = w.marg2; p.thr = w.thr;
        p.count = w.count; p.overflow = w.overflow;
        hipLaunchKernelGGL(k_prep_queries, dim3(qpad), dim3(256), 0, st, p);
        LY_HIP(hipGetLastError());
    }

    const uint32_t plan_tile = (h16 && !binary) ? (narrow ? 128u : 256u) : 0u;
    static const int no_sample = env_int("LYNSE_HIP_NO_SAMPLE_PLAN", 0);
#ifdef LYNSE_EXPERIMENTS
    const int w16env = scan_w16_env<-1>();
#else
    constexpr int w16env = -1;
#endif
    const bool filt = mask != nullptr || row_ids != nullptr;
    const int waves16 = l2n ? 0 : i8c ? 3 : (w16env >= 0 ? w16env : ((metric == M_IP && !filt) ? 3 : 0));
    const bool can_threshold_only = h16 && !binary && !filt && !no_lane_max_env() && k <= 128;
    Stage assign_stage{0u, (uint32_t)h->n};
    assign_stage.sample_tiles = (uint32_t)((h->n + 255) / 256);
    assign_stage.sample_stride = 256;
    const std::vector<Stage> plan = tl_assign ? std::vector<Stage>{assign_stage}
                                    : (sts || tl_coarse_dump) ? std::vector<Stage>{Stage{0u, (uint32_t)h->n}}
                                        : make_plan(h, k, (level == 0 && (!plan_tile || no_sample)) ? 1 : level, plan_tile, can_threshold_only,
                                                    (h16 && !i8c && !binary && k >= 64) ? 4u : 0u);
    const Stage sample = (!plan.empty() && plan[0].sample_tiles) ? plan[0] : Stage{0, 0};
    *sampled_plan = sample.sample_tiles != 0;
    const uint32_t sample_keys_per_tile = (small || mid64 || mid128 || waves16 != 0) ? 16u : 8u;
    const bool sample_threshold_only = h16 && !binary && !filt && sample.sample_tiles && !no_lane_max_env() && sample_keys_per_tile &&
                                       (k <= sample_keys_per_tile || (uint64_t)sample.sample_tiles * sample_keys_per_tile >= 8ull * k);
    const int fs_env = env_int("LYNSE_HIP_FUSED_SAMPLE", 0);
    const bool fs = fs_env != 0 && !debug_flags_env() && i8c && !aug && !cosq && !l2n && !bin_mfma && !mid64 && !mid128 && h->ld8 % 128 == 0 && sample_threshold_only && plan.size() >= 2 && k <= 32 &&
                    sample.sample_tiles == (uint32_t)h->num_cu && (plan[1].r1 - plan[1].r0 + 255) / 256 >= (uint32_t)h->num_cu &&
                    (uint64_t)k * 50000ull > (uint64_t)sample.sample_tiles * plan_tile &&
                    dense_env_now() != 0;
    bool plan_used_segments = false, plan_used_qs = false, plan_qs_sample = false, plan_used_qh = false;
    const int fused_tail_env = env_int("LYNSE_HIP_FUSED_TAIL", 1);
    const bool fused_tail = fused_tail_env != 0 && !plan.empty();
    SelectArgs sa_last{};
    for (size_t si = 0; si < plan.size(); ++si) {
        const Stage s = plan[si];
        const bool emit_all = si == 0 && !sts;
        if (fs && si == 0) continue;
        const bool fs_stage = fs && si == 1;
        uint32_t qs_sample_keys = 0;
        hipEvent_t e0 = nullptr, e1 = nullptr;
        if (tl_prof) {
            LY_TRY(get_event(h, (*ev_used)++, &e0));
            LY_TRY(get_event(h, (*ev_used)++, &e1));
            LY_HIP(hipEventRecord(e0, st));
        }
        uint32_t st_nseg = 0, st_seg = 0;
        int a_emit_all_last = -1;
        if (binary && !bin_mfma) {
            BinArgs b{};
            b.P = h->packed; b.W = h->words; b.row0 = s.r0; b.row1 = s.r1; b.QW = w.QW; b.nq = nq;
            b.thr = w.thr; b.cand = w.cand; b.count = w.count; b.cap = w.cap; b.emit_all = emit_all ? 1 : 0;
            b.mask = mask;
            static const int rows_minq = env_int("LYNSE_HIP_BIN_ROWS_MINQ", 1);
            if (h->words > 16u * BIN_MAX_CHUNKS) {
                const uint32_t groups = (s.r1 - s.r0 + 31) / 32;
                const uint32_t grid = std::max<uint32_t>(1, std::min<uint32_t>(groups, (uint32_t)h->num_cu * 8));
                LY_TRY(launch_scan_binary_wide(b, metric, grid, st));
            } else if ((int)nq >= rows_minq || mask) {
                uint32_t wcap = 1;
                while (wcap < h->words) wcap <<= 1;
                if (wcap != h->words) {
                    if (si == 0) {
                        hipLaunchKernelGGL(k_pad_words, dim3((nq * wcap + 255) / 256), dim3(256), 0, st, w.QW, h->words, w.QWp, wcap, nq);
                        LY_HIP(hipGetLastError());
                    }
                    b.QW = w.QWp;
                }
                const uint32_t groups = (s.r1 - s.r0 + 255) / 256;
                const uint32_t grid = std::max<uint32_t>(1, std::min<uint32_t>(groups, (uint32_t)h->num_cu * 8));
                LY_TRY(launch_scan_binary_rows(b, metric, grid, st));
            } else {
                const uint32_t groups = (s.r1 - s.r0 + 31) / 32;
                const uint32_t grid = std::max<uint32_t>(1, std::min<uint32_t>(groups, (uint32_t)h->num_cu * 8));
                const size_t lds = (size_t)nq * h->words * 8 + (size_t)nq * 4;
                LY_TRY(launch_scan_binary(b, metric, grid, lds, st));
            }
        } else {
            ScanArgs a{};
            a.V = score_rows(h); a.ld = score_ld(h); a.D = h->dim; a.row0 = s.r0; a.row1 = s.r1; a.Q16 = w.Q16;
            a.mask = mask;
            a.row_ids = row_ids;
            a.tile_stride = s.sample_stride;
            if (!s.sample_tiles && sample.sample_tiles && !sample_threshold_only) { a.skip_stride = sample.sample_stride; a.skip_tiles = sample.sample_tiles; }
            static const int big_rows = env_int("LYNSE_HIP_SCAN_BR", 256);
            uint32_t tile_rows = (glds && !small && big_rows == 256) ? 256u : (uint32_t)SCAN_BR;
            if (h16) tile_rows = narrow ? 128u : 256u;
            a.V16 = h->rows16; a.ld16 = h->ld16;
            if (i8c) { a.V16 = reinterpret_cast<const _Float16*>(bin_mfma ? (const int8_t*)h->bpm : (aug ? h->sq8a : (cosq ? h->sq8c : h->sq8))); a.ld16 = bin_mfma ? h->ld_bpm : (aug ? h->ld8a : h->ld8); }
            if (glds && !small && big_rows == 192 && metric == M_IP) tile_rows = 192u;
            a.qpad = qpad; a.nq = nq; a.nslab = nslab; a.ntiles = (s.r1 - s.r0 + tile_rows - 1) / tile_rows;
            if (s.sample_tiles) a.ntiles = s.sample_tiles;
            a.qinv = w.qinv; a.qn2 = w.qn2; a.qrinv = w.qrinv; a.thr = w.thr; a.vn2 = h->vn2; a.vrinv = h->vrinv;
            a.sv = h->sv; a.vmax2 = h->vmax * h->vmax; a.cand = w.cand; a.count = w.count; a.cap = w.cap; a.emit_all = emit_all ? 1 : 0;
            if (sample_threshold_only && s.sample_tiles) a.emit_all = 2;
            const int dbg = debug_flags_env();
            a.debug_flags = dbg;
            if (dbg & 2) a.emit_all = 0;
            if (dbg & 64) {
                static unsigned long long* d_dbg = nullptr;
                if (!d_dbg) LY_HIP(hipMalloc(&d_dbg, 4096 * 32 * 8));
                if (si == 0) LY_HIP(hipMemsetAsync(d_dbg, 0, 4096 * 32 * 8, st));
                a.dbg = d_dbg + (size_t)std::min<size_t>(plan.size() - 1 - si, 15) * 8192;
                g_dbg_ptr = d_dbg;
            }
            const int variant = scan_variant();
            if (i8c && small) {
                a.candB = w.candB; a.segcnt = w.segcnt;
                const uint32_t grid = std::min<uint32_t>(a.ntiles, (uint32_t)h->num_cu * 2);
                if (!a.emit_all) seg_geometry(grid, 4, &a.nseg, &a.seg);
                LY_TRY(launch_scan_i8c_small(a, grid, st, l2n, filt));
            } else if (mid64 || mid128) {
                a.candB = w.candB; a.segcnt = w.segcnt;
                const uint32_t grid = std::min<uint32_t>(a.ntiles, (uint32_t)h->num_cu * (mid64 ? 2u : 1u));
                if (!a.emit_all) seg_geometry(grid, 4, &a.nseg, &a.seg);
                LY_TRY(launch_scan_i8c_mid(a, grid, st, mid128, l2n, filt));
            } else if (l2n) {
                a.candB = w.candB; a.segcnt = w.segcnt;
                uint32_t grid = std::min<uint32_t>(a.ntiles, (uint32_t)h->num_cu);
                const uint64_t seen_before = s.sample_tiles ? 0 : (sample.sample_tiles ? std::max<uint64_t>((uint64_t)sample.sample_tiles * plan_tile, s.r0) : s.r0);
                a.dense = (!a.emit_all && seen_before) ? 1 : 0;
                const uint32_t qs_rt = qs_l2_rows(a);
                if (qs_rt) {
                    grid = std::min<uint32_t>((a.row1 - a.row0 + qs_rt - 1) / qs_rt, (uint32_t)h->num_cu);
                    seg_geometry(grid, 2, &a.nseg, &a.seg);
                    plan_used_qs = true;
                } else if (!a.emit_all) seg_geometry(grid, a.dense ? 4 : 2, &a.nseg, &a.seg);
                LY_TRY(launch_scan_i8l2(a, grid, st, qs_rt != 0));
            } else if (i8c) {
                a.candB = w.candB; a.segcnt = w.segcnt;
                const uint32_t grid = std::min<uint32_t>(a.ntiles, (uint32_t)h->num_cu);
                const uint64_t seen_before = s.sample_tiles ? 0 : (sample.sample_tiles ? std::max<uint64_t>((uint64_t)sample.sample_tiles * plan_tile, s.r0) : s.r0);
                a.dense = (!a.emit_all && a.ld16 % 128 == 0 && seen_before &&
                           (filt || (dense_env() >= 0 ? dense_env() != 0 : (uint64_t)k * 50000ull > seen_before))) ? 1 : 0;
                const bool ag = ag_env() && a.ld16 % 128 == 0 && !a.emit_all && !fs_stage && !filt && !bin_mfma;
                if (sts) {
                    a.dyn_thr = w.dyn; a.dyn_marg = w.dyn + w.qcap; a.dyn_slot = w.dyn + 2 * (size_t)w.qcap; a.dyn_ks = k;
                    a.dyn_warm = h->n >= 4000000ull ? 4u : 2u;
                }
                if (s.sample_tiles && !sts && qs_sample_ok(a, fs_stage, filt, bin_mfma, plan_tile)) {
                    const uint32_t nt64 = s.sample_tiles * 4u;
                    const uint32_t sgrid = std::min<uint32_t>(nt64, (uint32_t)h->num_cu);
                    if ((uint64_t)sgrid * 4u >= 8ull * k && sgrid * 4u <= w.cap && (nt64 + sgrid - 1) / sgrid <= 32u) {
                        a.ntiles = nt64;
                        LY_TRY(launch_scan_qs_sample(a, sgrid, st));
                        qs_sample_keys = sgrid * 4u;
                        plan_qs_sample = true;
                    }
                }
                if (!qs_sample_keys) {
                const bool qs = sts || (!ag && qs_scan_ok(a, fs_stage, filt, bin_mfma));
                uint32_t launch_grid = qs ? qs_grid(a, (uint32_t)h->num_cu) : grid;
                if (sts) {
                    const uint32_t nt = (a.row1 - a.row0 + 63) / 64;
                    uint32_t pitch = (nt + launch_grid - 1) / launch_grid;
                    auto gcd = [](uint32_t x, uint32_t y) { while (y) { const uint32_t t = x % y; x = y; y = t; } return x; };
                    while (gcd(pitch, k) != 1) ++pitch;
                    a.dyn_pitch = pitch;
                    launch_grid = (nt + pitch - 1) / pitch;
                }
                if (qs) { seg_geometry(launch_grid, 2, &a.nseg, &a.seg); plan_used_qs = true; }
                else
                if (!a.emit_all) seg_geometry(grid, (a.dense ? 8 : 4) / (ag ? 2 : 1), &a.nseg, &a.seg);
                if (fs_stage) {
                    a.fs_stride = sample.sample_stride; a.fs_rows = (uint32_t)h->n; a.gsync = w.gsync; a.Qf = Qf; a.marg2 = w.marg2;
                    a.thr_out = w.thr; a.k = k; a.ip_form = ip_form; a.metric = metric;
                    if (env_str("LYNSE_HIP_FS_STAMPS")) a.debug_flags |= 128;
                }
                LY_TRY(launch_scan_i8c(a, launch_grid, st, fs_stage, filt, bin_mfma, qs));
                }
            } else if (h16) {
                a.candB = w.candB; a.segcnt = w.segcnt;
// ... 23 lines not shown
                    if (waves16 == 2) { LY_TRY((launch_scan_h16<2, 4, 4, 2, 2, 2, false>(a, metric, grid, st))); }
                    else
#endif
                    if (waves16 == 3) { LY_TRY((launch_scan_h16<2, 4, 4, 2, 3, 2, false>(a, metric, grid, st, qchunks))); }
                    else { LY_TRY((launch_scan_h16<4, 2, 2, 4, 2, 2, false>(a, metric, grid, st, qchunks))); }
                }
            }
#ifdef LYNSE_EXPERIMENTS
            else if (glds) {
                const bool scale = h->sv != 1.0f;
                if (small) {
                    const uint32_t grid = std::min<uint32_t>(a.ntiles, (uint32_t)h->num_cu * 2);
                    LY_TRY((launch_scan_glds<1, 4, 1, 1, 4>(a, metric, scale, grid, st)));
                } else if (tile_rows == 192) {
                    const uint32_t grid = std::min<uint32_t>(a.ntiles, (uint32_t)h->num_cu);
                    LY_TRY((launch_scan_glds<4, 2, 2, 3, 4>(a, metric, scale, grid, st)));
                } else if (tile_rows == 256) {
                    const int gw16 = scan_w16_env<2>();
                    const uint32_t grid = std::min<uint32_t>(a.ntiles, (uint32_t)h->num_cu);
                    if (gw16 == 3) LY_TRY((launch_scan_glds<1, 8, 8, 1, 3>(a, metric, scale, grid, st)));
                    else if (gw16 == 0) LY_TRY((launch_scan_glds<4, 2, 2, 4, 3>(a, metric, scale, grid, st)));
                    else LY_TRY((launch_scan_glds<2, 4, 4, 2, 3>(a, metric, scale, grid, st)));
                } else {
                    const uint32_t grid = std::min<uint32_t>(a.ntiles, (uint32_t)h->num_cu);
                    LY_TRY((launch_scan_glds<4, 2, 2, 2, 4>(a, metric, scale, grid, st)));
                }
            } else {
                if (small) {
                    const uint32_t grid = std::min<uint32_t>(a.ntiles, (uint32_t)h->num_cu * 3);
                    if (variant == 1) LY_TRY((launch_scan<1, 4, 1, 1, 1>(h, a, metric, grid, st)));
                    else LY_TRY((launch_scan<1, 4, 1, 1, 2>(h, a, metric, grid, st)));
                } else {
                    const uint32_t grid = std::min<uint32_t>(a.ntiles, (uint32_t)h->num_cu);
                    if (variant == 1) LY_TRY((launch_scan<4, 2, 2, 2, 1>(h, a, metric, grid, st)));
                    else LY_TRY((launch_scan<4, 2, 2, 2, 2>(h, a, metric, grid, st)));
                }
            }
#endif
            (void)variant;
            a_emit_all_last = (int)a.emit_all;
            st_nseg = a.seg ? a.nseg : 0; st_seg = a.seg;
            plan_used_segments = plan_used_segments || a.seg != 0;
        }
        if (tl_coarse_dump) return LYNSE_OK;
        if (tl_assign) {
            if (a_emit_all_last != 2) return set_error(LYNSE_ERR_INTERNAL, "the assignment scan must run in lane-max mode");
            return LYNSE_OK;
        }
        if (tl_prof) {
            LY_HIP(hipEventRecord(e1, st));
            scan_events->push_back({*ev_used - 2, s.sample_tiles ? (uint64_t)s.sample_tiles * plan_tile
                                                                  : (uint64_t)(s.r1 - s.r0) + (fs_stage ? (uint64_t)sample.sample_tiles * plan_tile : 0ull)});
        }
        SelectArgs sa{};
        sa.cand = w.cand; sa.count = w.count; sa.overflow = w.overflow; sa.thr = w.thr; sa.marg2 = w.marg2;
        sa.k = k; sa.cap = w.cap; sa.keep_max = w.cap / 2; sa.metric = key_metric; sa.ip_form = ip_form;
        sa.neg_metric1 = (aug || cosq) ? metric + 1 : 0;
        sa.exact = binary ? 1 : 0;
        static const int tighten_env = env_int("LYNSE_HIP_TIGHTEN", 1);
        sa.tighten = (!binary && tighten_env && (i8c || k <= 32)) ? 1 : 0;
        sa.drop_sentinels = (mask && emit_all) ? 1 : 0;
        sa.emit_all_n = emit_all ? (s.sample_tiles ? (int)(s.sample_tiles * plan_tile) : (int)(s.r1 - s.r0)) : -1;
        if (!binary && emit_all && sample_threshold_only) {
            sa.threshold_only = 1;
            sa.drop_sentinels = 1;
            sa.emit_all_n = qs_sample_keys ? (int)qs_sample_keys : (int)(s.sample_tiles * sample_keys_per_tile);
        }
        sa.Qf = Qf; sa.V = score_rows(h); sa.ld = score_ld(h); sa.D = h->dim;
        sa.candB = w.candB; sa.segcnt = w.segcnt; sa.seg = st_seg; sa.nseg = st_nseg;
        sa.abort_word = fs_stage ? w.gsync + 2 : nullptr;
        if (sel_stamps_on())
            sa.stamps = reinterpret_cast<unsigned long long*>(w.gsync + 64) + (size_t)si * 256 * 8;
        if (fs_stage && env_str("LYNSE_HIP_DEBUG_FS")) return LYNSE_OK;
        if (fused_tail && si + 1 == plan.size()) { sa_last = sa; continue; }
        sa.lds_bytes = sel_lds_bytes(w.cap, nq);
        hipLaunchKernelGGL(k_select<SEL_NT>, dim3(nq), dim3(SEL_NT), sa.lds_bytes, st, sa);
        LY_HIP(hipGetLastError());
    }
    if (tl_prof && (!binary || bin_mfma)) {
        const uint64_t tiling = plan_used_qs ? 0x81u : plan_used_qh ? 0x82u : (small || mid64) ? 0x14u : ((mid128 || waves16 == 3 || waves16 == 2) ? 0x24u : 0x42u);
        std::lock_guard<std::mutex> plk(h->prof_mu);
        h->prof.last_plan = (sample.sample_tiles ? 1u : 0u) | ((sample.sample_tiles && sample_threshold_only) ? 2u : 0u) | (i8c ? 4u : 0u) |
                            (plan_used_segments ? 8u : 0u) | (small ? 16u : 0u) | (fs ? 128u : 0u) | ((uint64_t)(plan.size() & 0xff) << 8) | (tiling << 16) |
                            (sts ? (1ull << 24) : 0ull) | (plan_qs_sample ? (1ull << 25) : 0ull);
    }
    FinalArgs fa{};
    fa.cand = w.cand; fa.count = w.count; fa.k = k; fa.out_k = out_k; fa.cap = w.cap; fa.metric = key_metric; fa.ip_form = ip_form;
    fa.ham_dim = bin_mfma ? h->dim : 0u;
    fa.neg_metric1 = (aug || cosq) ? metric + 1 : 0;
    fa.exact = binary ? 1 : 0; fa.Qf = Qf; fa.V = score_rows(h); fa.ld = score_ld(h); fa.D = h->dim;
    fa.row_stride = h->row_stride; fa.row_offset = h->row_offset;
    fa.nan_rows = (!binary && !mask && !row_ids && h->n <= 0xffffffffull) ? (uint32_t)h->n : 0u;
    fa.out_rows = r_dst ? r_dst : w.out_rows; fa.out_dists = d_dst ? d_dst : w.out_dists; fa.out_counts = w.out_counts;
    fa.out_counts2 = c2_dst;
    fa.pool_total = tl_prof ? w.pool_total : nullptr;
    fa.overflow = w.overflow; fa.any_overflow = any_ovf;
    if (hdr_direct) { fa.h_hdr = w.h_hdr; fa.hdr_q = w.qcap; }
    if (fused_tail) {
        TailArgs ta{sa_last, fa};
        ta.s.hand_exact = env_int("LYNSE_HIP_HAND_EXACT", 1);
        ta.s.lds_bytes = ta.f.lds_bytes = sel_lds_bytes(w.cap, nq);
        hipLaunchKernelGGL(k_select_final<SEL_NT>, dim3(nq), dim3(SEL_NT), ta.s.lds_bytes, st, ta);
        LY_HIP(hipGetLastError());
        (void)asc;
        return LYNSE_OK;
    }
    if (i8c && !bin_mfma) {
        hipLaunchKernelGGL(k_rescore_pool<256>, dim3(nq, 4), dim3(256), 0, st, fa);
        LY_HIP(hipGetLastError());
        fa.exact = 1;
    }
    fa.lds_bytes = sel_lds_bytes(w.cap, nq);
    hipLaunchKernelGGL(k_final<SEL_NT>, dim3(nq), dim3(SEL_NT), fa.lds_bytes, st, fa);
    LY_HIP(hipGetLastError());
    (void)asc;
    return LYNSE_OK;
}

static int flat_assign_top1_device(lynse_hip_flat* h, const float* d_q, uint64_t nq, int metric, uint32_t* d_ids, uint32_t* d_redo,
                                   uint32_t* d_redo_count) {
    if (!h || !d_q || !d_ids || !d_redo || !d_redo_count) return set_error(LYNSE_ERR_INVALID_ARGUMENT, "NULL argument");
    if (metric < M_IP || metric > M_COS) return set_error(LYNSE_ERR_UNSUPPORTED, "float metrics only");
    LY_WRITER(h, lk);
    LY_TRY(use_device(h));
    if (scan_variant() != 3 || h->n == 0 || h->n > h->cap || h->qchunk <= QCHUNK || h->packed_only || h->dtype != LYNSE_DTYPE_F32)
        return set_error(LYNSE_ERR_UNSUPPORTED, "not the widened float shape of the assignment pass");
    struct Slot0 { int prev; Slot0() : prev(tl_ctx_slot) { tl_ctx_slot = 0; } ~Slot0() { tl_ctx_slot = prev; } } scope;
    LY_TRY(finalize_locked(h));
    if (metric == M_COS && h->cos_degenerate) return set_error(LYNSE_ERR_UNSUPPORTED, "degenerate norms: the exact search answers");
    LY_TRY(ensure_shadow_locked(h));
    LY_TRY(ensure_workspace(h, 1));
    Workspace& w = cur(h).ws;
    hipStream_t st = cur(h).stream;
    const uint32_t ntiles = (uint32_t)((h->n + 255) / 256);
    const uint32_t nkeys = ntiles * ((metric == M_IP) ? 16u : 8u);
    if (nkeys > w.cap) return set_error(LYNSE_ERR_UNSUPPORTED, "lane-max keys exceed the candidate slots");
    LY_HIP(hipMemsetAsync(d_redo_count, 0, 4, st));
    size_t ev_used = 0;
    std::vector<std::pair<size_t, uint64_t>> scan_events;
    struct Flag { Flag() { tl_assign = true; } ~Flag() { tl_assign = false; } } flag;
    const bool prof_prev = tl_prof;
    tl_prof = false;
    int rc = LYNSE_OK;
    for (uint64_t q0 = 0; q0 < nq && rc == LYNSE_OK; q0 += w.qcap) {
        const uint32_t nqc = (uint32_t)std::min<uint64_t>(w.qcap, nq - q0);
        bool sampled = false;
        rc = run_chunk(h, nqc, 1, 1, metric, 0, st, &ev_used, &scan_events, &sampled, nullptr, nullptr, false, nullptr, nullptr, nullptr, nullptr,
                       d_q + q0 * h->dim, false, false, nullptr);
        if (rc != LYNSE_OK) break;
        int ip_form = h->ip_form;
        if (ip_form == LYNSE_IPFORM_AUTO) ip_form = h->n < 4096 ? LYNSE_IPFORM_SINGLE : LYNSE_IPFORM_BATCH8;
        hipLaunchKernelGGL(k_assign_pick, dim3((nqc + 3) / 4), dim3(256), 0, st, w.cand, w.cap, nkeys, w.marg2, metric_ascending(metric) ? 1 : 0,
                           nqc, (uint32_t)q0, d_ids, d_redo, d_redo_count, d_q, score_rows(h), score_ld(h), h->dim, metric, ip_form);
        if (hipGetLastError() != hipSuccess) rc = set_error(LYNSE_ERR_DEVICE, "k_assign_pick launch failed");
    }
    tl_prof = prof_prev;
    if (rc != LYNSE_OK) { (void)hipStreamSynchronize(st); return rc; }
    LY_HIP(hipStreamSynchronize(st));
    return LYNSE_OK;
}

static bool small_path_ok(const lynse_hip_flat* h, uint64_t nq, uint32_t kk, int metric, bool filtered) {
    static const uint64_t max_bytes = (uint64_t)env_int("LYNSE_HIP_FUSED_MAX_MB", 64) << 20;
    return fused_env() && !h->no_fused && metric <= M_COS && !filtered && h->dtype == LYNSE_DTYPE_F32 && !h->packed_only && nq <= (uint64_t)SMALL_MAX_Q &&
           kk <= (uint32_t)SMALL_MAX_K && (uint64_t)h->n * h->ld * 4 * nq <= max_bytes &&
           (size_t)((h->dim + 3) / 4 * 4) * 4 + (size_t)128 * 1024 + 64 <= 150u * 1024u;
}
// ... 44 lines not shown
    if (small_dbg) {
        std::vector<unsigned long long> hd((size_t)grid * 4);
        LY_HIP(hipMemcpyAsync(hd.data(), d_dbg, hd.size() * 8, hipMemcpyDeviceToHost, st));
        LY_HIP(hipStreamSynchronize(st));
        unsigned long long t0 = ~0ull, s_last = 0, scan_end = 0, tick = 0, fin = 0, scan_end_min = ~0ull, scan_sum = 0, merge_sum = 0;
        for (uint32_t b = 0; b < grid; ++b) {
            t0 = std::min(t0, hd[b * 4]); s_last = std::max(s_last, hd[b * 4]);
            scan_end = std::max(scan_end, hd[b * 4 + 1]); scan_end_min = std::min(scan_end_min, hd[b * 4 + 1]);
            tick = std::max(tick, hd[b * 4 + 2]); fin = std::max(fin, hd[b * 4 + 3]);
            scan_sum += hd[b * 4 + 1] - hd[b * 4]; merge_sum += hd[b * 4 + 2] - hd[b * 4 + 1];
        }
        fprintf(stderr, "k_small_search grid %u lds %zu (10 ns ticks from the first start): last start %llu, first scan end %llu, last scan end %llu, last ticket %llu, end %llu; "
                        "mean scan %llu, mean wave merge %llu\n", grid, lds, s_last - t0, scan_end_min - t0, scan_end - t0, tick - t0, fin - t0, scan_sum / grid, merge_sum / grid);
    }
    if (timed) {
        LY_HIP(hipEventRecord(e1, st));
        scan_events->push_back({*ev_used - 2, (uint64_t)h->n * nq});
        std::lock_guard<std::mutex> plk(h->prof_mu);
        h->prof.last_plan = 32u | (1u << 8);
    }
    return LYNSE_OK;
}

static int sq8_merge_new_rows(lynse_hip_flat* h, uint32_t* mm, uint32_t D, uint64_t n_done, const float* row_scale, uint64_t* first_row, bool* mm_covers_all) {
    *first_row = 0;
    *mm_covers_all = false;
    if (n_done == 0 || n_done >= h->n) return LYNSE_OK;
    if (!h->sq8_mm_prev) LY_HIP(hipMalloc(&h->sq8_mm_prev, ((size_t)(h->dim + 64) * 2 + 1) * 4));
    hipStream_t st = cur(h).stream;
    uint32_t* flag = h->sq8_mm_prev + 2 * (size_t)D;
    LY_HIP(hipMemcpyAsync(h->sq8_mm_prev, mm, (size_t)D * 8, hipMemcpyDeviceToDevice, st));
    LY_HIP(hipMemsetAsync(flag, 0, 4, st));
    const uint64_t nn = h->n - n_done;
    const uint32_t gx = (D + 255) / 256;
    const uint32_t gy = (uint32_t)std::min<uint64_t>(std::max<uint64_t>(nn / 256, 1), (uint64_t)h->num_cu * 8);
    if (is_f16(h)) hipLaunchKernelGGL(k_sq8_minmax<_Float16>, dim3(gx, gy), dim3(256), 0, st, (const _Float16*)h->rows_h + n_done * h->ld16, h->ld16, D, nn, mm, mm + D,
                                      row_scale ? row_scale + n_done : nullptr);
    else hipLaunchKernelGGL(k_sq8_minmax<float>, dim3(gx, gy), dim3(256), 0, st, h->rows + n_done * h->ld, h->ld, D, nn, mm, mm + D, row_scale ? row_scale + n_done : nullptr);
    hipLaunchKernelGGL(k_mm_changed, dim3((2 * D + 255) / 256), dim3(256), 0, st, mm, h->sq8_mm_prev, 2 * D, flag);
    LY_HIP(hipGetLastError());
    uint32_t moved = 1;
    LY_HIP(hipMemcpyAsync(&moved, flag, 4, hipMemcpyDeviceToHost, st));
    LY_HIP(hipStreamSynchronize(st));
    *mm_covers_all = true;
    if (!moved) *first_row = n_done;
    return LYNSE_OK;
}

static int ensure_sq8_locked(lynse_hip_flat* h) {
    if (h->n_sq8 == h->n && h->sq8) return LYNSE_OK;
    bool kept = h->sq8 != nullptr && h->sq8_mins != nullptr && h->sq8_cap >= h->n;
    if (h->sq8_cap < h->n) {
        for (void* p : {(void*)h->sq8, (void*)h->sq8_sum, (void*)h->sq8_sum2})
            if (p) (void)hipFree(p);
        h->sq8 = nullptr; h->sq8_sum = nullptr; h->sq8_sum2 = nullptr;
        const uint64_t cap = std::max<uint64_t>(h->capacity, h->n);
        LY_HIP(hipMalloc(&h->sq8, (size_t)cap * h->ld8 + 256));
        LY_HIP(hipMalloc(&h->sq8_sum, ((size_t)cap + 256) * 4));
        LY_HIP(hipMalloc(&h->sq8_sum2, ((size_t)cap + 256) * 4));
        LY_HIP(hipMemsetAsync(h->sq8_sum, 0, ((size_t)cap + 256) * 4, cur(h).stream));
        LY_HIP(hipMemsetAsync(h->sq8_sum2, 0, ((size_t)cap + 256) * 4, cur(h).stream));
        h->sq8_cap = cap;
    }
    if (!h->sq8_mins) {
        LY_HIP(hipMalloc(&h->sq8_mins, (size_t)h->dim * 4));
        LY_HIP(hipMalloc(&h->sq8_scales, (size_t)h->dim * 4));
        LY_HIP(hipMalloc(&h->sq8_mm, (size_t)h->dim * 8));
        LY_HIP(hipMalloc(&h->sq8_stats, 16));
    }
    uint64_t r0 = 0;
    bool mm_done = false;
    if (kept) LY_TRY(sq8_merge_new_rows(h, h->sq8_mm, h->dim, h->n_sq8, nullptr, &r0, &mm_done));
    const uint32_t gx = (h->dim + 255) / 256;
    std::vector<uint32_t> init;
    if (!mm_done) {
        init.resize((size_t)h->dim * 2);
        for (uint32_t d = 0; d < h->dim; ++d) { init[d] = f32_to_ord(INFINITY); init[h->dim + d] = f32_to_ord(-INFINITY); }
        LY_HIP(hipMemcpyAsync(h->sq8_mm, init.data(), init.size() * 4, hipMemcpyHostToDevice, cur(h).stream));
        const uint32_t gy = (uint32_t)std::min<uint64_t>(std::max<uint64_t>(h->n / 256, 1), (uint64_t)h->num_cu * 8);
        if (is_f16(h)) hipLaunchKernelGGL(k_sq8_minmax<_Float16>, dim3(gx, gy), dim3(256), 0, cur(h).stream, (const _Float16*)h->rows_h, h->ld16, h->dim, h->n, h->sq8_mm, h->sq8_mm + h->dim);
        else hipLaunchKernelGGL(k_sq8_minmax<float>, dim3(gx, gy), dim3(256), 0, cur(h).stream, h->rows, h->ld, h->dim, h->n, h->sq8_mm, h->sq8_mm + h->dim);
    }
    if (r0 == 0) {
        LY_HIP(hipMemsetAsync(h->sq8_stats, 0, 16, cur(h).stream));
        hipLaunchKernelGGL(k_sq8_scales, dim3(gx), dim3(256), 0, cur(h).stream, h->sq8_mm, h->sq8_mm + h->dim, h->dim, h->sq8_mins, h->sq8_scales);
    }
    const uint64_t nn = h->n - r0;
    const uint32_t qgrid = (uint32_t)std::min<uint64_t>((nn + 3) / 4, (uint64_t)h->num_cu * 16);
    if (is_f16(h)) hipLaunchKernelGGL(k_sq8_quantize<_Float16>, dim3(qgrid), dim3(256), 0, cur(h).stream,
                       (const _Float16*)h->rows_h + r0 * h->ld16, h->ld16, h->dim, nn, h->sq8_mins, h->sq8_scales, h->sq8 + r0 * h->ld8, h->ld8, h->sq8_sum + r0, h->sq8_sum2 + r0, h->sq8_stats);
    else hipLaunchKernelGGL(k_sq8_quantize<float>, dim3(qgrid), dim3(256), 0, cur(h).stream,
                       h->rows + r0 * h->ld, h->ld, h->dim, nn, h->sq8_mins, h->sq8_scales, h->sq8 + r0 * h->ld8, h->ld8, h->sq8_sum + r0, h->sq8_sum2 + r0, h->sq8_stats);
    LY_HIP(hipGetLastError());
    uint32_t qst[4] = {0, 0, 0, 0};
    LY_HIP(hipMemcpyAsync(qst, h->sq8_stats, 16, hipMemcpyDeviceToHost, cur(h).stream));
    LY_HIP(hipStreamSynchronize(cur(h).stream));
    h->sq8_a1 = qst[0];
    h->sq8_a2sq = qst[2];
    memcpy(&h->sq8_eps2, &qst[3], 4);
    h->sq8_finite = qst[1] == 0;
    h->n_sq8 = h->n;
    return LYNSE_OK;
}

static int ensure_sq8a_locked(lynse_hip_flat* h) {
    if (h->n_sq8a == h->n && h->sq8a) return LYNSE_OK;
    const uint32_t DA = h->dim + h->aug_cols;
    if (h->sq8a_cap < h->n) {
        if (h->sq8a) (void)hipFree(h->sq8a);
        h->sq8a = nullptr;
        const uint64_t cap = std::max<uint64_t>(h->capacity, h->n);
        LY_HIP(hipMalloc(&h->sq8a, (size_t)cap * h->ld8a + 256));
        h->sq8a_cap = cap;
    }
    if (!h->sq8a_mins) {
        LY_HIP(hipMalloc(&h->sq8a_mins, (size_t)DA * 4));
        LY_HIP(hipMalloc(&h->sq8a_scales, (size_t)DA * 4));
        LY_HIP(hipMalloc(&h->sq8a_mm, (size_t)DA * 8));
        LY_HIP(hipMalloc(&h->sq8a_stats, 16));
    }
    LY_HIP(hipMemsetAsync(h->sq8a_stats, 0, 16, cur(h).stream));
    std::vector<uint32_t> init((size_t)DA * 2);
    for (uint32_t d = 0; d < DA; ++d) { init[d] = f32_to_ord(INFINITY); init[DA + d] = f32_to_ord(-INFINITY); }
    LY_HIP(hipMemcpyAsync(h->sq8a_mm, init.data(), init.size() * 4, hipMemcpyHostToDevice, cur(h).stream));
    const uint32_t gx = (h->dim + 255) / 256;
    const uint32_t gy = (uint32_t)std::min<uint64_t>(std::max<uint64_t>(h->n / 256, 1), (uint64_t)h->num_cu * 8);
    if (is_f16(h)) hipLaunchKernelGGL(k_sq8_minmax<_Float16>, dim3(gx, gy), dim3(256), 0, cur(h).stream, (const _Float16*)h->rows_h, h->ld16, h->dim, h->n, h->sq8a_mm, h->sq8a_mm + DA);
    else hipLaunchKernelGGL(k_sq8_minmax<float>, dim3(gx, gy), dim3(256), 0, cur(h).stream, h->rows, h->ld, h->dim, h->n, h->sq8a_mm, h->sq8a_mm + DA);
    hipLaunchKernelGGL(k_vec_minmax, dim3((uint32_t)std::min<uint64_t>((h->n + 255) / 256, (uint64_t)h->num_cu * 8)), dim3(256), 0, cur(h).stream,
                       h->vn2, h->n, h->sq8a_mm + h->dim, h->sq8a_mm + DA + h->dim, h->aug_cols);
    hipLaunchKernelGGL(k_sq8_scales, dim3((DA + 255) / 256), dim3(256), 0, cur(h).stream, h->sq8a_mm, h->sq8a_mm + DA, DA, h->sq8a_mins, h->sq8a_scales);
    if (is_f16(h)) hipLaunchKernelGGL(k_sq8_quantize<_Float16>, dim3((uint32_t)std::min<uint64_t>((h->n + 3) / 4, (uint64_t)h->num_cu * 16)), dim3(256), 0, cur(h).stream,
                       (const _Float16*)h->rows_h, h->ld16, h->dim, h->n, h->sq8a_mins, h->sq8a_scales, h->sq8a, h->ld8a, (int*)nullptr, (int*)nullptr, h->sq8a_stats, h->vn2, h->aug_cols);
    else hipLaunchKernelGGL(k_sq8_quantize<float>, dim3((uint32_t)std::min<uint64_t>((h->n + 3) / 4, (uint64_t)h->num_cu * 16)), dim3(256), 0, cur(h).stream,
                       h->rows, h->ld, h->dim, h->n, h->sq8a_mins, h->sq8a_scales, h->sq8a, h->ld8a, (int*)nullptr, (int*)nullptr, h->sq8a_stats, h->vn2, h->aug_cols);
    LY_HIP(hipGetLastError());
    uint32_t qst[4] = {0, 0, 0, 0};
    LY_HIP(hipMemcpyAsync(qst, h->sq8a_stats, 16, hipMemcpyDeviceToHost, cur(h).stream));
    LY_HIP(hipStreamSynchronize(cur(h).stream));
    h->sq8a_a1 = qst[0];
    h->sq8a_a2sq = qst[2];
    memcpy(&h->sq8a_eps2, &qst[3], 4);
    h->sq8a_finite = qst[1] == 0;
    h->n_sq8a = h->n;
    return LYNSE_OK;
}

static int ensure_sq8c_locked(lynse_hip_flat* h) {
    if (h->n_sq8c == h->n && h->sq8c) return LYNSE_OK;
    const uint32_t D = h->dim;
    const bool kept = h->sq8c != nullptr && h->sq8c_mins != nullptr && h->sq8c_cap >= h->n;
    if (h->sq8c_cap < h->n) {
        if (h->sq8c) (void)hipFree(h->sq8c);
        h->sq8c = nullptr;
        const uint64_t cap = std::max<uint64_t>(h->capacity, h->n);
        LY_HIP(hipMalloc(&h->sq8c, (size_t)cap * h->ld8 + 256));
        h->sq8c_cap = cap;
    }
    if (!h->sq8c_mins) {
        LY_HIP(hipMalloc(&h->sq8c_mins, (size_t)D * 4));
        LY_HIP(hipMalloc(&h->sq8c_scales, (size_t)D * 4));
        LY_HIP(hipMalloc(&h->sq8c_mm, (size_t)D * 8));
        LY_HIP(hipMalloc(&h->sq8c_stats, 16));
    }
    uint64_t r0 = 0;
    bool mm_done = false;
    if (kept) LY_TRY(sq8_merge_new_rows(h, h->sq8c_mm, D, h->n_sq8c, h->vrinv, &r0, &mm_done));
    const uint32_t gx = (D + 255) / 256;
    std::vector<uint32_t> init;
    if (!mm_done) {
        init.resize((size_t)D * 2);
        for (uint32_t d = 0; d < D; ++d) { init[d] = f32_to_ord(INFINITY); init[D + d] = f32_to_ord(-INFINITY); }
        LY_HIP(hipMemcpyAsync(h->sq8c_mm, init.data(), init.size() * 4, hipMemcpyHostToDevice, cur(h).stream));
        const uint32_t gy = (uint32_t)std::min<uint64_t>(std::max<uint64_t>(h->n / 256, 1), (uint64_t)h->num_cu * 8);
        if (is_f16(h)) hipLaunchKernelGGL(k_sq8_minmax<_Float16>, dim3(gx, gy), dim3(256), 0, cur(h).stream, (const _Float16*)h->rows_h, h->ld16, D, h->n, h->sq8c_mm, h->sq8c_mm + D, h->vrinv);
        else hipLaunchKernelGGL(k_sq8_minmax<float>, dim3(gx, gy), dim3(256), 0, cur(h).stream, h->rows, h->ld, D, h->n, h->sq8c_mm, h->sq8c_mm + D, h->vrinv);
    }
    if (r0 == 0) {
        LY_HIP(hipMemsetAsync(h->sq8c_stats, 0, 16, cur(h).stream));
        hipLaunchKernelGGL(k_sq8_scales, dim3(gx), dim3(256), 0, cur(h).stream, h->sq8c_mm, h->sq8c_mm + D, D, h->sq8c_mins, h->sq8c_scales);
    }
    const uint64_t nn = h->n - r0;
    const uint32_t qgrid = (uint32_t)std::min<uint64_t>((nn + 3) / 4, (uint64_t)h->num_cu * 16);
    if (is_f16(h)) hipLaunchKernelGGL(k_sq8_quantize<_Float16>, dim3(qgrid), dim3(256), 0, cur(h).stream,
                       (const _Float16*)h->rows_h + r0 * h->ld16, h->ld16, D, nn, h->sq8c_mins, h->sq8c_scales, h->sq8c + r0 * h->ld8, h->ld8, (int*)nullptr, (int*)nullptr, h->sq8c_stats,
                       (const float*)nullptr, 0u, h->vrinv + r0);
// ... 151 lines not shown
    if (c.load() >= 0) c.fetch_add(1);
}
static bool i8c_eligible(const lynse_hip_flat* h, int metric, bool filtered, uint64_t nqc, bool view = false, bool masked = false, bool ivf = false) {
    const int strikes = (metric == M_L2 ? h->i8c_strikes_l2 : (metric == M_COS ? h->i8c_strikes_cos : h->i8c_strikes)).load();
    static const int l2_off = []() { const char* e = env_str("LYNSE_HIP_COARSE_L2"); return e && !strcmp(e, "f16") ? 1 : 0; }();
    const bool l2_ok = metric == M_L2 && !l2_off &&
                       (l2_plain(h, nqc, masked) || (h->dim >= 256 && (uint64_t)h->ld8a * 4 <= (uint64_t)h->ld16 * 2 * 3));
    const bool cos_ok = metric == M_COS && !l2_off && h->dim >= 256 && !h->cos_degenerate;
    if (masked && metric != M_L2 && h->ld8 % 128 != 0) return false;
    static const int smallq = env_int("LYNSE_HIP_COARSE_SMALLQ", 1);
    const bool nq_ok = nqc > SCAN_BQ_SMALL || (smallq && nqc >= 1 && (coarse_env() == 2 || h->n >= 262144));
    const char* lowd_env = env_str("LYNSE_HIP_IP_LOWD");
    const bool lowd_i8 = lowd_env && !strcmp(lowd_env, "i8");
    if (metric == M_IP && !lowd_i8 && !ivf && !masked && !filtered && !view && coarse_env() != 2 && h->qchunk <= QCHUNK && qh_shape(h->ld16, nqc))
        return false;
    return (metric == M_IP || l2_ok || cos_ok) && !filtered && !view && nq_ok &&
           scan_variant() == 3 && coarse_env() != 1 && strikes >= 0 && strikes < 3 && (coarse_env() == 2 || h->n >= 65536);
}

static int search_large_k(lynse_hip_flat* h, const void* q_src, bool packed_queries, uint64_t nq, uint32_t k, int metric,
                          uint64_t* out_rows, float* out_dists, uint32_t* out_counts, bool on_device, hipStream_t user_stream,
                          const uint64_t* subset = nullptr, uint64_t n_subset = 0, bool filtered = false,
                          const uint64_t* bitset_words = nullptr, uint64_t n_words = 0);

static int prof_accumulate(lynse_hip_flat* h, lynse_hip_flat::Ctx& cx, hipEvent_t ev_begin, hipEvent_t ev_end,
                           const std::vector<std::pair<size_t, uint64_t>>& scan_events, bool binary, uint64_t fallback_queries) {
    LY_HIP(hipEventSynchronize(ev_end));
    float ms = 0.f;
    LY_HIP(hipEventElapsedTime(&ms, ev_begin, ev_end));
    std::lock_guard<std::mutex> plk(h->prof_mu);
    h->prof.total_us += (double)ms * 1000.0;
    const uint64_t row_bytes = binary ? (uint64_t)h->words * 8 : (uint64_t)h->dim * 4;
    for (auto& se : scan_events) {
        float sms = 0.f;
        LY_HIP(hipEventElapsedTime(&sms, cx.ev_pool[se.first], cx.ev_pool[se.first + 1]));
        h->prof.scan_us += (double)sms * 1000.0;
        h->prof.scan_launches += 1;
        h->prof.scan_rows += se.second;
        h->prof.scan_bytes += se.second * row_bytes;
    }
    h->prof.searches += 1;
    h->prof.fallback_queries += fallback_queries;
    return LYNSE_OK;
}

static int search_impl_once(lynse_hip_flat* h, const void* q_src, bool packed_queries, uint64_t nq, uint32_t k,
                            int metric, uint64_t* out_rows, float* out_dists, uint32_t* out_counts,
                            bool on_device, hipStream_t user_stream, const uint64_t* subset, uint64_t n_subset,
                            bool filtered, const uint64_t* bitset_words, uint64_t n_words, bool caller_holds_exclusive, bool force_shadow);
static int search_impl(lynse_hip_flat* h, const void* q_src, bool packed_queries, uint64_t nq, uint32_t k,
                       int metric, uint64_t* out_rows, float* out_dists, uint32_t* out_counts,
                       bool on_device, hipStream_t user_stream, const uint64_t* subset = nullptr, uint64_t n_subset = 0,
                       bool filtered = false, const uint64_t* bitset_words = nullptr, uint64_t n_words = 0,
                       bool caller_holds_exclusive = false) {
    int rc = search_impl_once(h, q_src, packed_queries, nq, k, metric, out_rows, out_dists, out_counts, on_device, user_stream, subset, n_subset,
                              filtered, bitset_words, n_words, caller_holds_exclusive, false);
    if (rc == LY_RESTART_EXCLUSIVE)
        rc = search_impl_once(h, q_src, packed_queries, nq, k, metric, out_rows, out_dists, out_counts, on_device, user_stream, subset, n_subset,
                              filtered, bitset_words, n_words, caller_holds_exclusive, true);
    return rc;
}
static int search_impl_once(lynse_hip_flat* h, const void* q_src, bool packed_queries, uint64_t nq, uint32_t k,
                            int metric, uint64_t* out_rows, float* out_dists, uint32_t* out_counts,
                            bool on_device, hipStream_t user_stream, const uint64_t* subset, uint64_t n_subset,
                            bool filtered, const uint64_t* bitset_words, uint64_t n_words, bool caller_holds_exclusive, bool force_shadow) {
    if (!h) return set_error(LYNSE_ERR_INVALID_ARGUMENT, "handle is NULL");
    LY_TRY(metric_check(metric));
    if (nq == 0) return LYNSE_OK;
    if (!q_src || !out_counts || (k && (!out_rows || !out_dists))) return set_error(LYNSE_ERR_INVALID_ARGUMENT, "NULL argument");
    LY_TRY(use_device(h));
    profile_begin_search(h);
    const bool binary = metric >= M_HAMMING;
    std::shared_lock<std::shared_mutex> rlk(h->rw, std::defer_lock);
    std::unique_lock<std::shared_mutex> xlk(h->rw, std::defer_lock);
    CtxLease lease;
    auto derived_ready = [&]() {
        if (binary) {
            if (!(h->packed_only || (h->packed != nullptr && h->n_packed == h->n))) return false;
            return !bin_mfma_eligible(h, metric, filtered, std::min<uint64_t>(nq, QCHUNK)) || (h->bpm && h->n_bpm == h->n);
        }
        if (h->packed_only) return true;
        if (h->n_stats != h->n) return false;
        if (force_shadow && !shadow_ready(h)) return false;
        if (i8c_eligible(h, metric, false, std::min<uint64_t>(nq, QCHUNK), caller_holds_exclusive, filtered)) return i8c_codes_ready(h, metric, std::min<uint64_t>(nq, QCHUNK), filtered);
        return shadow_ready(h) || small_path_ok(h, std::min<uint64_t>(nq, QCHUNK), (uint32_t)std::min<uint64_t>(k, h->n), metric, filtered);
    };
    auto needs_large_k = [&]() {
        if (h->n <= h->cap) return false;
        const uint64_t kk0 = std::min<uint64_t>(k, h->n);
        return (filtered ? std::min<uint64_t>(kk0, n_subset) : kk0) > h->cap / 4;
    };
    auto go_large_k = [&]() {
        return filtered ? search_large_k(h, q_src, packed_queries, nq, k, metric, out_rows, out_dists, out_counts, on_device, user_stream,
                                         subset, n_subset, true, bitset_words, n_words)
                        : search_large_k(h, q_src, packed_queries, nq, k, metric, out_rows, out_dists, out_counts, on_device, user_stream);
    };
    bool strategy_direct = false, strategy_known = false;
    auto choose_direct = [&]() -> bool {
        if (!filtered || binary) return false;
        const double rate = nq <= SCAN_BQ_SMALL ? 6.0e12 : 3.4e12;
        const double chunks = (double)((nq + QCHUNK - 1) / QCHUNK);
        const double row_b = (double)h->dim * 2.0;
        const double c_direct = (double)n_subset * row_b * 2.0 / 2.5e12 + (double)n_subset * row_b / rate * chunks + 120e-6;
        const bool mask_i8 = i8c_eligible(h, metric, false, std::min<uint64_t>(nq, QCHUNK), caller_holds_exclusive, true);
        const double c_scan = (mask_i8 ? (double)h->n * (double)h->dim / (nq <= SCAN_BQ_SMALL ? 6.5e12 : 3.6e12) : (double)h->n * row_b / rate) * chunks + 80e-6;
        const int force = env_int("LYNSE_HIP_FILTER_STRATEGY", 0);
        return (double)n_subset * row_b <= 8e9 && (force == 1 || (force == 0 && c_direct < c_scan));
    };
    if (!caller_holds_exclusive) {
        rlk.lock();
        if (needs_large_k()) { rlk.unlock(); return go_large_k(); }
        strategy_direct = filtered && n_subset != 0 && choose_direct();
        strategy_known = true;
        if (!user_stream && derived_ready() && !(filtered && (n_subset == 0 || strategy_direct))) {
            LY_TRY(lease.acquire(h));
        } else {
            rlk.unlock();
            LY_TRY(writer_lock(h, xlk));
            if (needs_large_k()) { xlk.unlock(); return go_large_k(); }
        }
    }
    hipStream_t st = user_stream ? user_stream : cur(h).stream;
    const hipMemcpyKind in_kind = on_device ? hipMemcpyDeviceToDevice : hipMemcpyHostToDevice;
    const hipMemcpyKind out_kind = on_device ? hipMemcpyDeviceToDevice : hipMemcpyDeviceToHost;

    if (packed_queries && !binary) return set_error(LYNSE_ERR_INVALID_ARGUMENT, "packed queries need a binary metric");
    if (!binary && h->packed_only) return set_error(LYNSE_ERR_INVALID_ARGUMENT, "store holds packed rows; float metrics unavailable");

    if (filtered && !binary && scan_variant() != 3)
        return set_error(LYNSE_ERR_UNSUPPORTED, "filtered search needs the default scan kernel (LYNSE_HIP_SCAN_VARIANT=3)");
    if (filtered && n_subset && !subset && !bitset_words) return set_error(LYNSE_ERR_INVALID_ARGUMENT, "subset is NULL");
    if (h->n == 0 || k == 0 || (filtered && n_subset == 0)) {
        if (on_device) LY_HIP(hipMemsetAsync(out_counts, 0, nq * 4, st));
        else memset(out_counts, 0, nq * 4);
        if (on_device) LY_HIP(hipStreamSynchronize(st));
        return LYNSE_OK;
    }
    uint32_t kk = (uint32_t)std::min<uint64_t>(k, h->n);
    if (filtered) kk = (uint32_t)std::min<uint64_t>(kk, n_subset);
    if (h->n > h->cap && kk > h->cap / 4)
        return set_error(LYNSE_ERR_UNSUPPORTED, "k > cap/4 over more than cap rows is not supported together with a subset filter");

    if (binary) {
        LY_TRY(ensure_packed_locked(h));
        if (xlk.owns_lock() && bin_mfma_eligible(h, metric, filtered, std::min<uint64_t>(nq, QCHUNK))) LY_TRY(ensure_bpm_locked(h));
    } else {
        LY_TRY(finalize_locked(h));
        if (force_shadow && (xlk.owns_lock() || caller_holds_exclusive)) LY_TRY(ensure_shadow_locked(h));
    }
    LY_TRY(ensure_workspace(h, k));
    Workspace& w = cur(h).ws;
    hipStream_t st0 = user_stream ? user_stream : cur(h).stream;
    auto need_shadow = [&]() -> int {
        if (binary || shadow_ready(h)) return LYNSE_OK;
        if (xlk.owns_lock() || caller_holds_exclusive) return ensure_shadow_locked(h);
        return LY_RESTART_EXCLUSIVE;
    };
    bool direct = false;
    std::vector<uint64_t> sorted_subset;
    auto& fc = cur(h);
    if (filtered) {
        direct = strategy_known ? strategy_direct : choose_direct();
        if (direct && !xlk.owns_lock() && !caller_holds_exclusive) return set_error(LYNSE_ERR_INTERNAL, "gathered-rows filter strategy without the exclusive lock");
        if (n_subset > fc.subset_cap && (direct || !bitset_words)) {
            if (fc.d_subset) (void)hipFree(fc.d_subset);
            fc.d_subset = nullptr;
            LY_HIP(hipMalloc(&fc.d_subset, n_subset * 8));
// ... 44 lines not shown
            if (words > fc.mask_words) {
                if (fc.d_mask) (void)hipFree(fc.d_mask);
                fc.d_mask = nullptr;
                LY_HIP(hipMalloc(&fc.d_mask, words * 4));
                fc.mask_words = words;
            }
            LY_HIP(hipMemsetAsync(fc.d_mask, 0, fc.mask_words * 4, st0));
            if (bitset_words) {
                const uint64_t bytes = std::min<uint64_t>(n_words * 8, (h->n + 63) / 64 * 8);
                LY_HIP(hipMemcpyAsync(fc.d_mask, bitset_words, bytes, hipMemcpyHostToDevice, st0));
            } else {
                const uint32_t blocks = (uint32_t)std::min<uint64_t>((n_subset + 255) / 256, (uint64_t)h->num_cu * 8);
                hipLaunchKernelGGL(k_mask_build, dim3(std::max<uint32_t>(blocks, 1)), dim3(256), 0, st0, fc.d_subset, n_subset, h->n, fc.d_mask);
                LY_HIP(hipGetLastError());
            }
        }
        if (direct && n_subset) {
            if (n_subset > h->g_cap) {
                for (void* p : {(void*)h->g_rows16, (void*)h->g_vn2, (void*)h->g_vrinv, (void*)h->g_ids32})
                    if (p) (void)hipFree(p);
                h->g_rows16 = nullptr; h->g_vn2 = h->g_vrinv = nullptr; h->g_ids32 = nullptr; h->g_cap = 0;
                LY_HIP(hipMalloc(&h->g_rows16, (size_t)n_subset * h->ld16 * 2 + 256));
                LY_HIP(hipMalloc(&h->g_vn2, ((size_t)n_subset + 256) * 4));
                LY_HIP(hipMalloc(&h->g_vrinv, ((size_t)n_subset + 256) * 4));
                LY_HIP(hipMalloc(&h->g_ids32, ((size_t)n_subset + 256) * 4));
                LY_HIP(hipMemsetAsync(h->g_vn2, 0, ((size_t)n_subset + 256) * 4, st0));
                LY_HIP(hipMemsetAsync(h->g_vrinv, 0, ((size_t)n_subset + 256) * 4, st0));
                h->g_cap = n_subset;
            }
            const uint64_t pieces = n_subset * (h->ld16 / 8);
            LY_TRY(need_shadow());
            hipLaunchKernelGGL(k_gather_rows16, dim3((uint32_t)std::min<uint64_t>((pieces + 255) / 256, (uint64_t)h->num_cu * 32)), dim3(256), 0,
                               st0, h->rows16, h->ld16, fc.d_subset, n_subset, h->g_rows16);
            LY_HIP(hipGetLastError());
            hipLaunchKernelGGL(k_gather_norms, dim3((uint32_t)std::min<uint64_t>((n_subset + 255) / 256, (uint64_t)h->num_cu * 8)), dim3(256), 0,
                               st0, h->vn2, h->vrinv, fc.d_subset, n_subset, h->g_vn2, h->g_vrinv, h->g_ids32);
            LY_HIP(hipGetLastError());
        }
        LY_HIP(hipStreamSynchronize(st0));
        if (direct && n_subset == 0) {
            if (on_device) LY_HIP(hipMemsetAsync(out_counts, 0, nq * 4, st0));
            else memset(out_counts, 0, nq * 4);
            if (on_device) LY_HIP(hipStreamSynchronize(st0));
            return LYNSE_OK;
        }
    }
    const uint32_t* mask = (filtered && !direct) ? fc.d_mask : nullptr;
    struct ViewGuard {
        lynse_hip_flat* h; bool on; _Float16* r16; uint64_t n; float *vn2, *vrinv;
        ~ViewGuard() { if (on) { h->rows16 = r16; h->n = n; h->vn2 = vn2; h->vrinv = vrinv; } }
    } view{h, direct, h->rows16, h->n, h->vn2, h->vrinv};
    if (direct) { h->rows16 = h->g_rows16; h->n = n_subset; h->vn2 = h->g_vn2; h->vrinv = h->g_vrinv; }

    hipEvent_t ev_begin = nullptr, ev_end = nullptr;
    size_t ev_used = 0;
    std::vector<std::pair<size_t, uint64_t>> scan_events;
    if (tl_prof) {
        LY_TRY(get_event(h, ev_used++, &ev_begin));
        LY_TRY(get_event(h, ev_used++, &ev_end));
        LY_HIP(hipEventRecord(ev_begin, st));
    }
    uint64_t fallback_queries = 0;
    bool i8c_attempted = false;

    const bool wide = h->qchunk > QCHUNK && !binary && !filtered && scan_variant() == 3 && h->n <= h->cap;
    const uint32_t QC = wide ? w.qcap : QCHUNK;
    for (uint64_t q0 = 0; q0 < nq; q0 += QC) {
        const uint32_t nqc = (uint32_t)std::min<uint64_t>(QC, nq - q0);
        if (binary) {
            if (packed_queries) {
                LY_HIP(hipMemcpyAsync(w.QW, (const uint64_t*)q_src + q0 * h->words, (size_t)nqc * h->words * 8, in_kind, st));
            } else {
                LY_HIP(hipMemcpyAsync(w.Qf, (const float*)q_src + q0 * h->dim, (size_t)nqc * h->dim * 4, in_kind, st));
                hipLaunchKernelGGL(k_pack_bits<float>, dim3((nqc + 3) / 4), dim3(256), 0, st, w.Qf, h->dim, h->dim, nqc, w.QW, h->words);
                LY_HIP(hipGetLastError());
            }
        } else if (!on_device) {
            LY_HIP(hipMemcpyAsync(w.Qf, (const float*)q_src + q0 * h->dim, (size_t)nqc * h->dim * 4, in_kind, st));
        }
        const float* qsrc = (on_device && !binary) ? (const float*)q_src + q0 * h->dim : nullptr;
        bool i8c = i8c_eligible(h, metric, filtered && direct, nqc, caller_holds_exclusive, filtered && !direct);
        if (i8c) {
            const bool msk = filtered && !direct;
            if (xlk.owns_lock()) LY_TRY(ensure_i8c_codes_locked(h, metric, nqc, msk));
            else if (!i8c_codes_ready(h, metric, nqc, msk)) i8c = false;
            if (i8c && !i8c_codes_finite(h, metric, nqc, msk)) { i8c_strike_counter(h, metric).store(-1); i8c = false; }
        }
        i8c_attempted = i8c_attempted || i8c;
        if (!binary && !i8c && !direct && !small_path_ok(h, nqc, kk, metric, filtered)) LY_TRY(need_shadow());
        if (small_path_ok(h, nqc, kk, metric, filtered)) {
            const size_t rows_b = (size_t)nqc * k * 8, dists_b = (size_t)nqc * k * 4;
            uint64_t* r_dst = on_device ? out_rows + q0 * k : reinterpret_cast<uint64_t*>(w.h_out);
            float* d_dst = on_device ? out_dists + q0 * k : reinterpret_cast<float*>(w.h_out + rows_b);
            uint32_t* c_dst = on_device ? out_counts + q0 : w.h_hdr;
            LY_TRY(run_small(h, nqc, kk, k, metric, st, &ev_used, &scan_events, r_dst, d_dst, c_dst, w.h_hdr + w.qcap,
                             on_device ? (const float*)q_src + q0 * h->dim : w.Qf));
            LY_HIP(hipStreamSynchronize(st));
            if (!on_device) {
                memcpy(out_rows + q0 * k, w.h_out, rows_b);
                memcpy(out_dists + q0 * k, w.h_out + rows_b, dists_b);
                memcpy(out_counts + q0, w.h_hdr, nqc * 4);
            }
            continue;
        }
        bool allow_sts = true;
        for (int level = 0; level < 3; ++level) {
            bool sampled = false, used_sts = false;
            const size_t rows_b = (size_t)nqc * k * 8, dists_b = (size_t)nqc * k * 4;
            const bool staged = !on_device && rows_b + dists_b <= H_OUT_BYTES;
            uint64_t* r_dst = on_device ? out_rows + q0 * k : (staged ? reinterpret_cast<uint64_t*>(w.h_out) : nullptr);
            float* d_dst = on_device ? out_dists + q0 * k : (staged ? reinterpret_cast<float*>(w.h_out + rows_b) : nullptr);
            LY_TRY(run_chunk(h, nqc, kk, k, metric, level, st, &ev_used, &scan_events, &sampled, mask, direct ? h->g_ids32 : nullptr, i8c,
                             r_dst, d_dst, on_device ? out_counts + q0 : nullptr, nullptr, qsrc, true, allow_sts, &used_sts));
            if (!on_device && !staged) {
                LY_HIP(hipMemcpyAsync(out_rows + q0 * k, w.out_rows, rows_b, out_kind, st));
                LY_HIP(hipMemcpyAsync(out_dists + q0 * k, w.out_dists, dists_b, out_kind, st));
            }
            LY_TRY(stream_wait(st));
            uint32_t nov = 0;
            for (uint32_t i = 0; i < nqc; ++i) nov += w.h_hdr[w.qcap + i] ? 1 : 0;
            if (nov == 0) {
                if (staged) { memcpy(out_rows + q0 * k, w.h_out, rows_b); memcpy(out_dists + q0 * k, w.h_out + rows_b, dists_b); }
                break;
            }
            if (level == 2) return set_error(LYNSE_ERR_INTERNAL, "candidate overflow on the exhaustive plan");
            fallback_queries += nov;
            if (used_sts) {
                allow_sts = false;
                --level;
                continue;
            }
            if (i8c) {
                i8c = false;
                i8c_add_strike(h, metric);
                LY_TRY(need_shadow());
                --level;
                continue;
            }
            if (level == 0 && !sampled) level = 1;
        }
        if (!on_device) memcpy(out_counts + q0, w.h_hdr, nqc * 4);
    }

    if (tl_prof) {
        LY_HIP(hipEventRecord(ev_end, st));
        LY_TRY(prof_accumulate(h, cur(h), ev_begin, ev_end, scan_events, binary, fallback_queries));
        if (i8c_attempted) {
            std::lock_guard<std::mutex> plk(h->prof_mu);
            h->prof.last_plan |= 64u;
        }
    }
    return LYNSE_OK;
}

extern "C" int lynse_hip_flat_coarse_scores(lynse_hip_flat* h, const float* queries, uint64_t nq, int metric, int coarse,
                                            float* out_scores, float* out_bound, int* out_form) {
    if (!h || !queries || !out_scores || !out_bound) return set_error(LYNSE_ERR_INVALID_ARGUMENT, "NULL argument");
    if (metric_additive(metric)) return metric_check(metric);
    if (metric < M_IP || metric > M_COS) return set_error(LYNSE_ERR_INVALID_ARGUMENT, "float metrics only");
    if (nq == 0 || nq > QCHUNK) return set_error(LYNSE_ERR_INVALID_ARGUMENT, "1..256 queries");
    LY_TRY(use_device(h));
    std::unique_lock<std::shared_mutex> xlk;
    LY_TRY(writer_lock(h, xlk));
    if (h->packed_only || h->n == 0 || h->n > h->cap) return set_error(LYNSE_ERR_INVALID_ARGUMENT, "a float shard of 1..cap rows");
    LY_TRY(finalize_locked(h));
    LY_TRY(ensure_workspace(h, 1));
    const bool i8c = coarse != 0;
    if (!i8c) LY_TRY(ensure_shadow_locked(h));
    if (i8c) {
        LY_TRY(ensure_i8c_codes_locked(h, metric, nq));
        if (!i8c_codes_finite(h, metric, nq)) return set_error(LYNSE_ERR_UNSUPPORTED, "the shard holds non-finite values: no int8 pass");
    }
    Workspace& w = cur(h).ws;
    hipStream_t st = cur(h).stream;
    LY_HIP(hipMemcpyAsync(w.Qf, queries, (size_t)nq * h->dim * 4, hipMemcpyHostToDevice, st));
    size_t ev_used = 0;
    std::vector<std::pair<size_t, uint64_t>> scan_events;
    bool sampled = false;
    tl_coarse_dump = true;
    const int rc = run_chunk(h, (uint32_t)nq, 1, 1, metric, 1, st, &ev_used, &scan_events, &sampled, nullptr, nullptr, i8c);
    tl_coarse_dump = false;
    LY_TRY(rc);
    LY_HIP(hipStreamSynchronize(st));
    const bool l2n = i8c && metric == M_L2 && l2_plain(h, nq, false);
    const bool aug = i8c && metric == M_L2 && !l2n, cosq = i8c && metric == M_COS;
    if (out_form) *out_form = (i8c ? 1 : 0) | (aug ? 2 : 0) | (l2n ? 4 : 0) | (cosq ? 8 : 0);
    const bool key_asc = metric_ascending((aug || cosq) ? (int)M_IP : metric);
    std::vector<uint64_t> keys(h->n);
    std::vector<float> m2(nq);
    LY_HIP(hipMemcpy(m2.data(), w.marg2, nq * 4, hipMemcpyDeviceToHost));
    for (uint64_t q = 0; q < nq; ++q) {
        LY_HIP(hipMemcpy(keys.data(), w.cand + (size_t)q * w.cap, (size_t)h->n * 8, hipMemcpyDeviceToHost));
        for (uint64_t r = 0; r < h->n; ++r) {
            if (key_row(keys[r]) != (uint32_t)r) return set_error(LYNSE_ERR_INTERNAL, "the emit-all stage did not leave row r in slot r");
            const float sc = key_score(keys[r], key_asc);
            out_scores[q * h->n + r] = (aug || cosq) ? -sc : sc;
        }
        out_bound[q] = 0.5f * m2[q];
    }
    return LYNSE_OK;
}

extern "C" int lynse_hip_flat_coarse_state(lynse_hip_flat* h, int* out_strikes, uint64_t* out_sq8_rows) {
    if (!h) return set_error(LYNSE_ERR_INVALID_ARGUMENT, "handle is NULL");
    std::shared_lock<std::shared_mutex> lk(h->rw);
    if (out_strikes) *out_strikes = h->i8c_strikes.load();
    if (out_sq8_rows) *out_sq8_rows = h->sq8 ? h->n_sq8 : 0;
    return LYNSE_OK;
}

extern "C" uint64_t lynse_hip_flat_bpm_rows(const lynse_hip_flat* h) {
    if (!h) return 0;
    std::shared_lock<std::shared_mutex> lk(const_cast<lynse_hip_flat*>(h)->rw);
    return h->bpm ? h->n_bpm : 0;
}

extern "C" int lynse_hip_flat_prepare(lynse_hip_flat* h, int metric, uint64_t nq) {
    if (!h) return set_error(LYNSE_ERR_INVALID_ARGUMENT, "handle is NULL");
    LY_TRY(metric_check(metric));
    LY_WRITER(h, lk);
    LY_TRY(use_device(h));
    if (h->n == 0) return LYNSE_OK;
    const uint64_t nqc = std::min<uint64_t>(std::max<uint64_t>(nq, 1), QCHUNK);
    if (metric >= M_HAMMING) {
        LY_TRY(ensure_packed_locked(h));
        if (bin_mfma_eligible(h, metric, false, nqc)) LY_TRY(ensure_bpm_locked(h));
        return LYNSE_OK;
    }
    if (h->packed_only) return set_error(LYNSE_ERR_INVALID_ARGUMENT, "store holds packed rows; float metrics unavailable");
    LY_TRY(finalize_locked(h));
    if (i8c_eligible(h, metric, false, nqc)) {
        LY_TRY(ensure_i8c_codes_locked(h, metric, nqc));
        if (!i8c_codes_finite(h, metric, nqc)) i8c_strike_counter(h, metric).store(-1);
    }
    if (!i8c_eligible(h, metric, false, nqc) && !small_path_ok(h, nqc, 10, metric, false)) LY_TRY(ensure_shadow_locked(h));
    return LYNSE_OK;
}

extern "C" uint64_t lynse_hip_flat_hbm_bytes(const lynse_hip_flat* h) {
    if (!h) return 0;
    std::shared_lock<std::shared_mutex> lk(const_cast<lynse_hip_flat*>(h)->rw);
    uint64_t b = 0;
    if (h->rows) b += h->capacity * h->ld * 4ull;
    if (h->rows_h) b += h->capacity * h->ld16 * 2ull;
    if (h->rows16 && !h->shadow_alias) b += h->cap16 * h->ld16 * 2ull;
    if (h->vn2) b += 2ull * (h->stats_capacity + 256) * 4;
    if (h->packed) b += h->packed_capacity * h->words * 8ull;
    if (h->sq8) b += h->sq8_cap * h->ld8 + 2ull * (h->sq8_cap + 256) * 4;
    if (h->sq8a) b += h->sq8a_cap * h->ld8a;
    if (h->sq8c) b += h->sq8c_cap * h->ld8;
    if (h->bpm) b += h->bpm_cap * h->ld_bpm;
    return b;
}

static int search_large_k(lynse_hip_flat* h, const void* q_src, bool packed_queries, uint64_t nq, uint32_t k, int metric,
                          uint64_t* out_rows, float* out_dists, uint32_t* out_counts, bool on_device, hipStream_t user_stream,
                          const uint64_t* subset, uint64_t n_subset, bool filtered, const uint64_t* bitset_words, uint64_t n_words) {
    LY_WRITER(h, xlk);
    LY_TRY(use_device(h));
    const bool binary = metric >= M_HAMMING;
    if (packed_queries && !binary) return set_error(LYNSE_ERR_INVALID_ARGUMENT, "packed queries need a binary metric");
    if (!binary && h->packed_only) return set_error(LYNSE_ERR_INVALID_ARGUMENT, "store holds packed rows; float metrics unavailable");
    if (binary) LY_TRY(ensure_packed_locked(h));
    else { LY_TRY(finalize_locked(h)); LY_TRY(ensure_shadow_locked(h)); }
    const uint64_t n = h->n, R = h->cap;
    std::vector<uint64_t> ids;
    if (filtered) {
        if (bitset_words) {
            const uint64_t nw = std::min<uint64_t>(n_words, (n + 63) / 64);
            for (uint64_t w = 0; w < nw; ++w)
                for (uint64_t bits = bitset_words[w]; bits; bits &= bits - 1) {
                    const uint64_t r = w * 64 + (uint64_t)__builtin_ctzll(bits);
                    if (r < n) ids.push_back(r);
                }
        } else {
            ids.assign(subset, subset + n_subset);
            std::sort(ids.begin(), ids.end());
            ids.erase(std::unique(ids.begin(), ids.end()), ids.end());
            while (!ids.empty() && ids.back() >= n) ids.pop_back();
        }
    }
    const uint32_t kk = (uint32_t)std::min<uint64_t>(std::min<uint64_t>(k, n), filtered ? ids.size() : n);
    const uint64_t n_ranges = (n + R - 1) / R;
    const size_t q_elems = packed_queries ? h->words : h->dim, q_bytes = q_elems * (packed_queries ? 8 : 4);
    if (kk == 0) {
        if (on_device) LY_TRY(memset_done(out_counts, 0, nq * 4));
        else memset(out_counts, 0, nq * 4);
        return LYNSE_OK;
    }
    std::vector<uint8_t> q_host;
    const uint8_t* qh = reinterpret_cast<const uint8_t*>(q_src);
    if (on_device) {
        q_host.resize((size_t)nq * q_bytes);
        LY_HIP(hipMemcpy(q_host.data(), q_src, q_host.size(), hipMemcpyDeviceToHost));
        qh = q_host.data();
    }
    struct View {
        lynse_hip_flat* h;
        float* rows; _Float16 *rows16, *rows_h; float *vn2, *vrinv; uint64_t* packed;
        uint64_t n, n_stats, n16, n_packed, row_offset;
        explicit View(lynse_hip_flat* hh) : h(hh), rows(hh->rows), rows16(hh->rows16), rows_h(hh->rows_h), vn2(hh->vn2), vrinv(hh->vrinv), packed(hh->packed),
                                            n(hh->n), n_stats(hh->n_stats), n16(hh->n16), n_packed(hh->n_packed), row_offset(hh->row_offset) {}
        void set(uint64_t r0, uint64_t r1) {
            h->rows = rows ? rows + r0 * h->ld : nullptr;
            h->rows_h = rows_h ? rows_h + r0 * h->ld16 : nullptr;
            h->rows16 = rows16 ? rows16 + r0 * h->ld16 : nullptr;
            h->vn2 = vn2 ? vn2 + r0 : nullptr;
            h->vrinv = vrinv ? vrinv + r0 : nullptr;
            h->packed = packed ? packed + r0 * h->words : nullptr;
            h->n = r1 - r0;
            h->n_stats = h->n; h->n16 = rows16 ? h->n : 0; h->n_packed = packed ? h->n : 0;
            h->row_offset = row_offset + r0 * h->row_stride;
        }
        ~View() {
            h->rows = rows; h->rows_h = rows_h; h->rows16 = rows16; h->vn2 = vn2; h->vrinv = vrinv; h->packed = packed;
            h->n = n; h->n_stats = n_stats; h->n16 = n16; h->n_packed = n_packed; h->row_offset = row_offset;
        }
    } view(h);
    struct FormGuard { lynse_hip_flat* h; int f; ~FormGuard() { h->ip_form = f; } } form_guard{h, h->ip_form};
    if (h->ip_form == LYNSE_IPFORM_AUTO) h->ip_form = n < 4096 ? LYNSE_IPFORM_SINGLE : LYNSE_IPFORM_BATCH8;
    const uint64_t qb = std::max<uint64_t>(1, std::min<uint64_t>(QCHUNK, (64ull << 20) / std::max<uint64_t>(1, n_ranges * kk * 12)));
    std::vector<uint64_t> l_rows((size_t)qb * n_ranges * kk), m_rows(kk);
    std::vector<float> l_dists((size_t)qb * n_ranges * kk), m_dists(kk);
    std::vector<uint32_t> l_counts((size_t)qb * n_ranges), r_counts(qb);
    std::vector<uint64_t> t_rows((size_t)qb * kk);
    std::vector<float> t_dists((size_t)qb * kk);
    std::vector<uint64_t> o_rows(on_device ? (size_t)nq * k : 0);
    std::vector<float> o_dists(on_device ? (size_t)nq * k : 0);
    std::vector<uint32_t> o_counts(on_device ? nq : 0);
    uint64_t* res_rows = on_device ? o_rows.data() : out_rows;
    float* res_dists = on_device ? o_dists.data() : out_dists;
// ... 106 lines not shown
    lk.unlock();
    for (uint64_t q = 0; q < nq; ++q) {
        LY_TRY(search_impl(h, queries + q * h->dim, false, 1, k, metric, out_rows + q * k, out_dists + q * k, out_counts + q, false, nullptr,
                           cand[q].data(), cand[q].size(), true));
        (void)kk;
    }
    return LYNSE_OK;
}

static int additive_search(lynse_hip_flat* h, const float* queries, uint64_t nq, uint32_t k, int metric, bool filtered,
                           const uint64_t* subset, uint64_t n_subset, const uint64_t* bitset_words, uint64_t n_words,
                           uint64_t* out_rows, float* out_dists, uint32_t* out_counts);

extern "C" int lynse_hip_flat_search_f32(lynse_hip_flat* h, const float* queries, uint64_t nq, uint32_t k, int metric,
                                         uint64_t* out_rows, float* out_dists, uint32_t* out_counts) {
    if (metric_additive(metric)) return additive_search(h, queries, nq, k, metric, false, nullptr, 0, nullptr, 0, out_rows, out_dists, out_counts);
    return search_impl(h, queries, false, nq, k, metric, out_rows, out_dists, out_counts, false, nullptr);
}

extern "C" int lynse_hip_flat_search_filtered_f32(lynse_hip_flat* h, const float* queries, uint64_t nq, uint32_t k, int metric,
                                                  const uint64_t* subset_rows, uint64_t n_subset, uint64_t* out_rows,
                                                  float* out_dists, uint32_t* out_counts) {
    if (metric_additive(metric)) return additive_search(h, queries, nq, k, metric, true, subset_rows, n_subset, nullptr, 0, out_rows, out_dists, out_counts);
    return search_impl(h, queries, false, nq, k, metric, out_rows, out_dists, out_counts, false, nullptr, subset_rows, n_subset, true);
}

extern "C" int lynse_hip_flat_search_filtered_bitset_f32(lynse_hip_flat* h, const float* queries, uint64_t nq, uint32_t k, int metric,
                                                         const uint64_t* bitset_words, uint64_t n_words, uint64_t* out_rows,
                                                         float* out_dists, uint32_t* out_counts) {
    if (!h) return set_error(LYNSE_ERR_INVALID_ARGUMENT, "handle is NULL");
    if (n_words && !bitset_words) return set_error(LYNSE_ERR_INVALID_ARGUMENT, "bitset is NULL");
    if (metric_additive(metric)) {
        static const uint64_t none = 0;
        return additive_search(h, queries, nq, k, metric, true, nullptr, 0, bitset_words ? bitset_words : &none, n_words, out_rows, out_dists, out_counts);
    }
    const uint64_t n = lynse_hip_flat_len(h);
    uint64_t count = 0;
    const uint64_t full = std::min<uint64_t>(n_words, n / 64);
    for (uint64_t w = 0; w < full; ++w) count += (uint64_t)__builtin_popcountll(bitset_words[w]);
    if (full < n_words && (n % 64)) count += (uint64_t)__builtin_popcountll(bitset_words[full] & ((1ull << (n % 64)) - 1ull));
    return search_impl(h, queries, false, nq, k, metric, out_rows, out_dists, out_counts, false, nullptr, nullptr, count, true,
                       bitset_words, n_words);
}

extern "C" int lynse_hip_flat_search_f32_device(lynse_hip_flat* h, const float* d_queries, uint64_t nq, uint32_t k,
                                                int metric, uint64_t* d_out_rows, float* d_out_dists,
                                                uint32_t* d_out_counts, void* stream) {
    return search_impl(h, d_queries, false, nq, k, metric, d_out_rows, d_out_dists, d_out_counts, true, (hipStream_t)stream);
}

extern "C" int lynse_hip_flat_search_packed_u64(lynse_hip_flat* h, const uint64_t* qw, uint64_t nq, uint32_t k, int metric,
                                                uint64_t* out_rows, float* out_dists, uint32_t* out_counts) {
    return search_impl(h, qw, true, nq, k, metric, out_rows, out_dists, out_counts, false, nullptr);
}

extern "C" int lynse_hip_flat_search_packed_u64_device(lynse_hip_flat* h, const uint64_t* d_qw, uint64_t nq, uint32_t k,
                                                       int metric, uint64_t* d_out_rows, float* d_out_dists,
                                                       uint32_t* d_out_counts, void* stream) {
    return search_impl(h, d_qw, true, nq, k, metric, d_out_rows, d_out_dists, d_out_counts, true, (hipStream_t)stream);
}

extern "C" int lynse_hip_top_k_search(const float* query, const float* candidates, uint64_t n, uint32_t dim, uint32_t k,
                                      int metric, int device, uint32_t* out_idx, float* out_dist, uint32_t* out_count) {
    if (!out_count) return set_error(LYNSE_ERR_INVALID_ARGUMENT, "out_count is NULL");
    *out_count = 0;
    if (!metric_valid(metric)) return set_error(LYNSE_ERR_UNKNOWN_METRIC, "Unknown metric id");
    if (dim == 0) return set_error(LYNSE_ERR_INVALID_ARGUMENT, "dimension must be greater than zero");
    if (n == 0 || k == 0) return LYNSE_OK;
    if (!query || !candidates || !out_idx || !out_dist) return set_error(LYNSE_ERR_INVALID_ARGUMENT, "NULL argument");
    struct Scratch {
        lynse_hip_flat* h = nullptr; int device = -1; uint32_t dim = 0;
        ~Scratch() { if (h) lynse_hip_flat_destroy(h); }
    };
    static thread_local Scratch sc;
    if (!sc.h || sc.device != device || sc.dim != dim) {
        if (sc.h) { lynse_hip_flat_destroy(sc.h); sc.h = nullptr; }
        LY_TRY(lynse_hip_flat_create(dim, device, &sc.h));
        sc.device = device; sc.dim = dim;
        LY_TRY(lynse_hip_flat_set_ip_form(sc.h, LYNSE_IPFORM_SINGLE));
    }
    lynse_hip_flat* h = sc.h;
    {
        std::unique_lock<std::shared_mutex> lk(h->rw);
        h->n = 0; h->n_stats = 0; h->n16 = 0; h->n_packed = 0; h->n_sq8 = 0; h->n_sq8a = 0; h->n_sq8c = 0; h->n_bpm = 0; h->i8c_strikes.store(0); h->i8c_strikes_l2.store(0); h->i8c_strikes_cos.store(0);
        h->amax = h->vmax = h->vmin = 0.f; h->sv = 1.f; h->cos_degenerate = 0; h->rows_integer = 0; h->rows_nonneg = 0;
        const uint32_t init[5] = {0u, 0u, 0x7f800000u, 0u, 0u};
        LY_TRY(use_device(h));
        LY_TRY(h2d_done(h->d_stats, init, sizeof init));
    }
    int rc = lynse_hip_flat_append_f32(h, candidates, n);
    const uint32_t kk = (uint32_t)std::min<uint64_t>(k, n);
    std::vector<uint64_t> rows(kk);
    uint32_t cnt = 0;
    if (rc == LYNSE_OK) rc = lynse_hip_flat_search_f32(h, query, 1, kk, metric, rows.data(), out_dist, &cnt);
    if (rc != LYNSE_OK) return rc;
    for (uint32_t i = 0; i < cnt; ++i) out_idx[i] = (uint32_t)rows[i];
    *out_count = cnt;
    return LYNSE_OK;
}

extern "C" int lynse_hip_compute_distance(const float* a, const float* b, uint32_t dim, int metric, int device, float* out) {
    if (!a || !b || !out) return set_error(LYNSE_ERR_INVALID_ARGUMENT, "NULL argument");
    uint32_t idx = 0, cnt = 0;
    float d = 0.f;
    LY_TRY(lynse_hip_top_k_search(a, b, 1, dim, 1, metric, device, &idx, &d, &cnt));
    if (cnt != 1) return set_error(LYNSE_ERR_INTERNAL, "distance kernel returned no result");
    *out = d;
    return LYNSE_OK;
}

extern "C" int lynse_hip_pack_binary_f32(const float* rows, uint64_t n, uint32_t dim, int device, uint64_t* out_words) {
    if (n == 0) return LYNSE_OK;
    if (!rows || !out_words) return set_error(LYNSE_ERR_INVALID_ARGUMENT, "NULL argument");
    lynse_hip_flat* h = nullptr;
    LY_TRY(lynse_hip_flat_create(dim, device, &h));
    int rc = lynse_hip_flat_append_f32(h, rows, n);
    if (rc == LYNSE_OK) rc = lynse_hip_flat_read_packed(h, 0, n, out_words);
    lynse_hip_flat_destroy(h);
    return rc;
}

extern "C" int lynse_hip_merge_topk(const uint64_t* ids, const float* dists, const uint32_t* counts, uint32_t n_lists,
                                    uint32_t stride, uint32_t k, int metric, uint64_t* out_ids, float* out_dists,
                                    uint32_t* out_count) {
    if (!out_count) return set_error(LYNSE_ERR_INVALID_ARGUMENT, "out_count is NULL");
    *out_count = 0;
    if (!metric_valid(metric)) return set_error(LYNSE_ERR_UNKNOWN_METRIC, "Unknown metric id");
    if (n_lists == 0 || k == 0) return LYNSE_OK;
    if (!ids || !dists || !counts || !out_ids || !out_dists) return set_error(LYNSE_ERR_INVALID_ARGUMENT, "NULL argument");
    const bool asc = metric_ascending(metric);
    struct E { float d; uint64_t id; };
    std::vector<E> all;
    for (uint32_t l = 0; l < n_lists; ++l) {
        if (counts[l] > stride) return set_error(LYNSE_ERR_INVALID_ARGUMENT, "count exceeds stride");
        for (uint32_t i = 0; i < counts[l]; ++i) all.push_back({dists[(size_t)l * stride + i], ids[(size_t)l * stride + i]});
    }
    auto before = [asc](const E& x, const E& y) {
        if (x.d < y.d) return asc;
        if (x.d > y.d) return !asc;
        return x.id < y.id;
    };
    const size_t kk = std::min<size_t>(k, all.size());
    std::partial_sort(all.begin(), all.begin() + kk, all.end(), before);
    for (size_t i = 0; i < kk; ++i) { out_ids[i] = all[i].id; out_dists[i] = all[i].d; }
    *out_count = (uint32_t)kk;
    return LYNSE_OK;
}

static int merge_topk_device_impl(const void* d_blocks, uint64_t block_bytes, uint64_t rows_off,
                                  uint64_t dists_off, uint64_t counts_off, uint32_t n_lists, uint64_t nq,
                                  uint32_t k, int metric, uint64_t* d_out_rows, float* d_out_dists,
                                  uint32_t* d_out_counts, void* stream, uint64_t status_off, uint32_t* out_status) {
    LY_TRY(metric_check(metric));
    if (nq == 0) return LYNSE_OK;
    if (!d_blocks || !d_out_counts || (k && (!d_out_rows || !d_out_dists))) return set_error(LYNSE_ERR_INVALID_ARGUMENT, "NULL argument");
    if (n_lists == 0) return set_error(LYNSE_ERR_INVALID_ARGUMENT, "n_lists is zero");
    if (k == 0) {
        LY_HIP(hipMemsetAsync(d_out_counts, 0, nq * 4, (hipStream_t)stream));
        return LYNSE_OK;
    }
    const uint64_t total = (uint64_t)n_lists * k;
    if (total > 8192) return set_error(LYNSE_ERR_UNSUPPORTED, "n_lists * k exceeds the merge kernel capacity (8192)");
    uint32_t np2 = 2;
    while (np2 < total) np2 <<= 1;
    LY_TRY(ensure_lds<k_merge<256>>(8192 * 12));
    MergeArgs a{};
    a.blocks = (const char*)d_blocks; a.block_bytes = block_bytes; a.rows_off = rows_off; a.dists_off = dists_off;
// ... 53 lines not shown
```

Measured before the change: 137,300.

## Add SQ7 zero-based int8 code copy for FLAT-IP coarse scan on nonnegative rows

Adds a second quantized copy of the rows using 7-bit codes (0..127, no -128 offset) for nonnegative data, used by the int8 coarse scan for FLAT-IP with 129..256-query chunks on stores of at least 10M rows. The per-query error bound is adjusted for the new offset, using the query rounding-error sum. A strike counter falls back to the SQ8 path if SQ7 results fail verification. This costs extra HBM for the copy and a build pass, and may cause reruns if the looser precision triggers fallbacks.

New measurement: 142,700 (median of 6 runs). 1.04x the previous value.

```diff
diff --git a/include/lynse_hip.h b/include/lynse_hip.h
--- a/include/lynse_hip.h
+++ b/include/lynse_hip.h
@@ -269,6 +269,9 @@
 int lynse_hip_flat_coarse_scores(lynse_hip_flat *h, const float *queries, uint64_t nq, int metric, int coarse,
                                  float *out_scores, float *out_bound, int *out_form);
 
+int lynse_hip_flat_coarse_scores_sq7(lynse_hip_flat *h, const float *queries, uint64_t nq, float *out_scores, float *out_bound, int *out_form);
+int lynse_hip_flat_sq7_state(lynse_hip_flat *h, uint64_t *out_rows, int *out_strikes);
+
 
 typedef struct lynse_hip_sparse lynse_hip_sparse;
 int lynse_hip_sparse_normalize(const uint64_t *indptr , const uint32_t *indices, const float *values, uint64_t n,
diff --git a/lynsedb_amd/_lib.py b/lynsedb_amd/_lib.py
--- a/lynsedb_amd/_lib.py
+++ b/lynsedb_amd/_lib.py
@@ -151,6 +151,8 @@
     "lynse_hip_ivf_build_sharded_device": (C.c_int, [_vp, C.c_uint64, C.c_uint64, C.c_uint32, C.c_uint32, C.c_uint32, C.c_uint32, C.c_uint32, C.c_int, C.c_int, C.c_int,
                                                     _vp, _vp, _vp, C.POINTER(_vp)]),
     "lynse_hip_flat_coarse_scores": (C.c_int, [_vp, _vp, C.c_uint64, C.c_int, C.c_int, _vp, _vp, C.POINTER(C.c_int)]),
+    "lynse_hip_flat_coarse_scores_sq7": (C.c_int, [_vp, _vp, C.c_uint64, _vp, _vp, C.POINTER(C.c_int)]),
+    "lynse_hip_flat_sq7_state": (C.c_int, [_vp, _u64p, C.POINTER(C.c_int)]),
     "lynse_hip_sparse_normalize": (C.c_int, [_vp, _vp, _vp, C.c_uint64, _vp, _vp, _vp]),
     "lynse_hip_sparse_create": (C.c_int, [C.c_int, C.POINTER(_vp)]),
     "lynse_hip_sparse_destroy": (C.c_int, [_vp]),
diff --git a/lynsedb_amd/core.py b/lynsedb_amd/core.py
--- a/lynsedb_amd/core.py
+++ b/lynsedb_amd/core.py
@@ -578,6 +578,19 @@
         form = C.c_int(0)
         check(lib.lynse_hip_flat_coarse_scores(self._h, _ptr(q), q.shape[0], m, 1 if coarse in ("i8", "int8", 1, True) else 0, _ptr(scores), _ptr(bound), C.byref(form)))
         return scores, bound, form.value
+
+    def coarse_scores_sq7(self, queries):
+        q = np.ascontiguousarray(np.atleast_2d(queries), dtype=np.float32)
+        scores = np.empty((q.shape[0], len(self)), np.float32)
+        bound = np.empty(q.shape[0], np.float32)
+        form = C.c_int(0)
+        check(lib.lynse_hip_flat_coarse_scores_sq7(self._h, _ptr(q), q.shape[0], _ptr(scores), _ptr(bound), C.byref(form)))
+        return scores, bound, form.value
+
+    def sq7_state(self) -> dict:
+        rows, strikes = C.c_uint64(0), C.c_int(0)
+        check(lib.lynse_hip_flat_sq7_state(self._h, C.byref(rows), C.byref(strikes)))
+        return {"sq7_rows": rows.value, "sq7_strikes": strikes.value}
 
     def coarse_state(self) -> dict:
         strikes, rows = C.c_int(0), C.c_uint64(0)
diff --git a/lynsedb_amd/csrc/kernels.h b/lynsedb_amd/csrc/kernels.h
--- a/lynsedb_amd/csrc/kernels.h
+++ b/lynsedb_amd/csrc/kernels.h
@@ -2062,13 +2062,13 @@
 }
 
 __global__ void __launch_bounds__(256) k_sq8_scales(const uint32_t* __restrict__ omin, const uint32_t* __restrict__ omax, uint32_t D,
-                                                    float* __restrict__ mins, float* __restrict__ scales) {
+                                                    float* __restrict__ mins, float* __restrict__ scales, float top = 255.0f) {
     const uint32_t d = blockIdx.x * 256 + threadIdx.x;
     if (d >= D) return;
     const float mn = ord_to_f32(omin[d]), mx = ord_to_f32(omax[d]);
     const float range = __fsub_rn(mx, mn);
-    mins[d] = mn;
-    scales[d] = range > 1e-30f ? __fdiv_rn(255.0f, range) : 0.0f;
+    if (mins) mins[d] = mn;
+    scales[d] = range > 1e-30f ? __fdiv_rn(top, range) : 0.0f;
 }
 
 __global__ void __launch_bounds__(256) k_mm_changed(const uint32_t* __restrict__ now, const uint32_t* __restrict__ before, uint32_t n, uint32_t* __restrict__ flag) {
@@ -2089,10 +2089,10 @@
         for (uint32_t j = 0; j < ncopies; ++j) { atomicMin(omin + j, f32_to_ord(mn)); atomicMax(omax + j, f32_to_ord(mx)); }
 }
 
-__device__ __forceinline__ int sq8_code(float v, float mn, float sc) {
+__device__ __forceinline__ int sq8_code(float v, float mn, float sc, float top = 255.0f) {
     float q = roundf(__fmul_rn(__fsub_rn(v, mn), sc));
     if (!(q == q)) return 0;
-    q = q < 0.0f ? 0.0f : (q > 255.0f ? 255.0f : q);
+    q = q < 0.0f ? 0.0f : (q > top ? top : q);
     return (int)q;
 }
 
@@ -2102,7 +2102,7 @@
                                                       int8_t* __restrict__ out, uint32_t ld8, int* __restrict__ sums,
                                                       int* __restrict__ sums2, uint32_t* __restrict__ stats,
                                                       const float* __restrict__ extra_col = nullptr, uint32_t n_extra = 0,
-                                                      const float* __restrict__ row_scale = nullptr) {
+                                                      const float* __restrict__ row_scale = nullptr, int sq7 = 0) {
     const int lane = threadIdx.x & 63;
     const uint64_t wave = ((uint64_t)blockIdx.x * blockDim.x + threadIdx.x) >> 6;
     const uint64_t nwaves = ((uint64_t)gridDim.x * blockDim.x) >> 6;
@@ -2116,11 +2116,12 @@
             if (d < D || (extra_col && d < D + n_extra)) {
                 const float v = d < D ? (row_scale ? __fmul_rn((float)V[row * ld + d], row_scale[row]) : (float)V[row * ld + d]) : extra_col[row];
                 if (!(fabsf(v) < LY_INF)) nonfinite += 1;
-                const int code = sq8_code(v, mins[d], scales[d]);
-                c = code - 128;
+                const int code = sq8_code(v, mins[d], scales[d], sq7 ? 127.0f : 255.0f);
+                c = sq7 ? code : code - 128;
+                const int cc = sq7 ? code - 64 : c;
                 s1 += c;
-                s2 += c * c;
-                l1 += c < 0 ? -c : c;
+                s2 += cc * cc;
+                l1 += cc < 0 ? -cc : cc;
                 const float e = __fsub_rn(__fmul_rn(__fsub_rn(v, mins[d]), scales[d]), (float)code);
                 const float ea = fabsf(e);
                 if (ea == ea) { e2 = __fmaf_rn(e, e, e2); e1 += ea; }
@@ -2195,6 +2196,7 @@
     int aug;
     int l2n;
     int cosine;
+    int sq7;
     const int8_t* codes;
     uint32_t ld8, n_rows, tile_rows, dyn_ks, seed_rows;
     int *dyn_thr, *dyn_slot, *dyn_marg;
@@ -2266,7 +2268,7 @@
     __syncthreads();
     const double inv = 1.0 / (double)s_sq;
     const uint32_t total = a.nslab * 128;
-    double eta2 = 0.0;
+    double eta2 = 0.0, eta1 = 0.0;
     for (uint32_t i = tid; i < total; i += 256) {
         int u = 0;
         if (i < DA) {
@@ -2277,14 +2279,15 @@
             r = r < -127.0 ? -127.0 : (r > 127.0 ? 127.0 : r);
             u = (r == r) ? (int)r : 0;
             const double eta = t - (double)u;
-            if (eta == eta) eta2 += eta * eta;
+            if (eta == eta) { eta2 += eta * eta; eta1 += eta; }
         }
         const uint32_t s = i / 128, k = i % 128, l = k >> 4, e = k & 15, p = l ^ ((q >> 1) & 7);
         a.img[(((size_t)s * a.qpad + q) * 8 + p) * 16 + e] = (int8_t)u;
         if (a.dyn_thr) s_u[i] = (int8_t)u;
     }
-    for (int o = 32; o > 0; o >>= 1) eta2 += __shfl_xor(eta2, o, 64);
-    if (lane == 0) red2[1][wave] = eta2;
+    for (int o = 32; o > 0; o >>= 1) { eta2 += __shfl_xor(eta2, o, 64); eta1 += __shfl_xor(eta1, o, 64); }
+    __shared__ double red3[4];
+    if (lane == 0) { red2[1][wave] = eta2; red3[wave] = eta1; }
     __syncthreads();
     if (tid == 0) {
         wmax = fmax(fmax(red[0][0], red[0][1]), fmax(red[0][2], red[0][3]));
@@ -2295,9 +2298,11 @@
         sw2 = (red2[0][0] + red2[0][1]) + (red2[0][2] + red2[0][3]);
         eta2 = (red2[1][0] + red2[1][1]) + (red2[1][2] + red2[1][3]);
         const float sq = s_sq;
-        const double bq = sqm + 128.0 * sw - (a.aug ? s2 : 0.0) - (a.cosine ? 1.0 : 0.0);
+        eta1 = (red3[0] + red3[1]) + (red3[2] + red3[3]);
+        const double bq = sqm + (a.sq7 ? 64.0 * (double)sq * eta1 : 128.0 * sw) - (a.aug ? s2 : 0.0) - (a.cosine ? 1.0 : 0.0);
         const float bqf = (float)bq;
         const double a1 = (double)a.a1;
+        const double a1mag = a.sq7 ? a1 + 64.0 * (double)DA : a1;
         const double gam = 10.0 * (double)a.D * 5.9604645e-8;
         const double ref_term = a.cosine ? 9.0 * ((double)a.D + 8.0) * 5.9604645e-8
                                 : a.aug  ? 8.0 * ((double)a.D + 8.0) * 5.9604645e-8 * (s2 + (double)a.vmax * (double)a.vmax)
@@ -2305,7 +2310,7 @@
         double tq = 0.5001 * (double)sq * a1, tr = 0.5001 * swabs;
         if (a.a2sq) { const double c2 = 1.0002 * (double)sq * sqrt(eta2) * sqrt((double)a.a2sq); tq = c2 < tq ? c2 : tq; }
         if (a.eps2 > 0.0f) { const double c2 = 1.0002 * sqrt(sw2) * sqrt((double)a.eps2); tr = c2 < tr ? c2 : tr; }
-        double E = tr + tq + 2.5e-7 * (fabs(bq) + (a.cosine ? 1.0 : fabs(s2)) + 127.0 * (double)sq * a1) + ref_term;
+        double E = tr + tq + 2.5e-7 * (fabs(bq) + (a.cosine ? 1.0 : fabs(s2)) + 127.0 * (double)sq * a1mag) + ref_term;
         float bq_out = bqf;
         if (a.l2n) {
             const double vm2 = (double)a.vmax * (double)a.vmax;
diff --git a/lynsedb_amd/csrc/lynse_hip.hip b/lynsedb_amd/csrc/lynse_hip.hip
--- a/lynsedb_amd/csrc/lynse_hip.hip
+++ b/lynsedb_amd/csrc/lynse_hip.hip
@@ -285,6 +285,14 @@
     uint32_t sq8_a1 = 0, sq8_a2sq = 0;
     float sq8_eps2 = 0.0f;
     bool sq8_finite = false;
+    uint64_t sq8_fit = 0;
+    int8_t* sq7 = nullptr;
+    uint64_t n_sq7 = 0, sq7_cap = 0, sq7_fit = 0;
+    float* sq7_scales = nullptr;
+    uint32_t* sq7_stats = nullptr;
+    uint32_t sq7_a1 = 0, sq7_a2sq = 0;
+    float sq7_eps2 = 0.0f;
+    std::atomic<int> sq7_strikes{0};
     int8_t* sq8a = nullptr;
     uint32_t ld8a = 0, aug_cols = 1;
     uint64_t n_sq8a = 0, sq8a_cap = 0;
@@ -457,7 +465,8 @@
     for (void* p : {(void*)h->rows, (void*)h->rows_h, (void*)h->rows16, (void*)h->packed, (void*)h->vn2, (void*)h->vrinv, (void*)h->d_stats,
                     (void*)h->g_rows16, (void*)h->g_vn2, (void*)h->g_vrinv, (void*)h->g_ids32,
                     (void*)h->bpm, (void*)h->sq8c, (void*)h->sq8c_mins, (void*)h->sq8c_scales, (void*)h->sq8c_mm, (void*)h->sq8c_stats, (void*)h->sq8a, (void*)h->sq8a_mins, (void*)h->sq8a_scales, (void*)h->sq8a_mm, (void*)h->sq8a_stats,
-                    (void*)h->sq8, (void*)h->sq8_mins, (void*)h->sq8_scales, (void*)h->sq8_sum, (void*)h->sq8_sum2, (void*)h->sq8_mm, (void*)h->sq8_stats, (void*)h->sq8_mm_prev})
+                    (void*)h->sq8, (void*)h->sq8_mins, (void*)h->sq8_scales, (void*)h->sq8_sum, (void*)h->sq8_sum2, (void*)h->sq8_mm, (void*)h->sq8_stats, (void*)h->sq8_mm_prev,
+                    (void*)h->sq7, (void*)h->sq7_scales, (void*)h->sq7_stats})
         if (p) (void)hipFree(p);
     for (auto& c : h->ctx)
         if (c.stream) (void)hipStreamDestroy(c.stream);
@@ -1608,13 +1617,17 @@
 
 static bool l2_plain(const lynse_hip_flat* h, uint64_t nqc, bool masked = false);
 static thread_local bool tl_coarse_dump = false;
+static int fused_sample_env() { return env_int("LYNSE_HIP_FUSED_SAMPLE", 0); }
+static bool sq7_wanted(const lynse_hip_flat* h, int metric, uint64_t nqc, bool masked);
+static bool sq7_ready(const lynse_hip_flat* h);
 static thread_local bool tl_assign = false;
 
 static int run_chunk(lynse_hip_flat* h, uint32_t nq, uint32_t k, uint32_t out_k, int metric, int level, hipStream_t st,
                      size_t* ev_used, std::vector<std::pair<size_t, uint64_t>>* scan_events, bool* sampled_plan,
                      const uint32_t* mask = nullptr, const uint32_t* row_ids = nullptr, bool i8c = false,
                      uint64_t* r_dst = nullptr, float* d_dst = nullptr, uint32_t* c2_dst = nullptr, uint32_t* any_ovf = nullptr,
-                     const float* qsrc = nullptr, bool hdr_direct = false, bool allow_sts = true, bool* used_sts = nullptr) {
+                     const float* qsrc = nullptr, bool hdr_direct = false, bool allow_sts = true, bool* used_sts = nullptr,
+                     bool allow_sq7 = false, bool* used_sq7 = nullptr) {
     Workspace& w = cur(h).ws;
     const float* Qf = qsrc ? qsrc : w.Qf;
     const bool binary = metric >= M_HAMMING;
@@ -1655,6 +1668,8 @@
                      k >= 1 && k <= 32 && qs_variant() >= 1 && qs_variant() <= 3 && sts_ld8 == 768 && nslab == 6 && qpad == 256 && h->n >= 65536 &&
                      h->n < 0xffffff00ull && (metric == M_IP || cosq);
     if (used_sts) *used_sts = sts;
+    const bool sq7 = allow_sq7 && i8c && !bin_mfma && !mask && !row_ids && sq7_wanted(h, metric, nq, false) && sq7_ready(h);
+    if (used_sq7) *used_sq7 = sq7;
     if (bin_mfma) {
         BpmPrepArgs p{};
         p.QW = w.QW; p.W = h->words; p.D = h->dim; p.qpad = qpad; p.nslab = nslab; p.nq = nq; p.img = reinterpret_cast<uint8_t*>(w.Q16);
@@ -1675,6 +1690,10 @@
         if (i8c_cs_on()) { p.a2sq = aug ? h->sq8a_a2sq : (cosq ? h->sq8c_a2sq : h->sq8_a2sq); p.eps2 = aug ? h->sq8a_eps2 : (cosq ? h->sq8c_eps2 : h->sq8_eps2); } p.cosine = cosq ? 1 : 0; p.img = reinterpret_cast<int8_t*>(w.Q16); p.aug = aug ? (int)h->aug_cols : 0; p.l2n = l2n ? 1 : 0;
         p.sq = w.qinv; p.bq = w.qn2; p.marg2 = w.marg2; p.thr = w.thr; p.count = w.count; p.overflow = w.overflow;
         p.gsync = w.gsync;
+        if (sq7) {
+            p.sq7 = 1; p.scales = h->sq7_scales; p.a1 = h->sq7_a1;
+            if (i8c_cs_on()) { p.a2sq = h->sq7_a2sq; p.eps2 = h->sq7_eps2; }
+        }
         if (sts) {
             p.codes = cosq ? h->sq8c : h->sq8; p.ld8 = sts_ld8; p.n_rows = (uint32_t)h->n; p.tile_rows = 64; p.dyn_ks = k;
             p.seed_rows = std::min<uint32_t>(1024u, 32u * k);
@@ -1714,7 +1733,7 @@
     const uint32_t sample_keys_per_tile = (small || mid64 || mid128 || waves16 != 0) ? 16u : 8u;
     const bool sample_threshold_only = h16 && !binary && !filt && sample.sample_tiles && !no_lane_max_env() && sample_keys_per_tile &&
                                        (k <= sample_keys_per_tile || (uint64_t)sample.sample_tiles * sample_keys_per_tile >= 8ull * k);
-    const int fs_env = env_int("LYNSE_HIP_FUSED_SAMPLE", 0);
+    const int fs_env = fused_sample_env();
     const bool fs = fs_env != 0 && !debug_flags_env() && i8c && !aug && !cosq && !l2n && !bin_mfma && !mid64 && !mid128 && h->ld8 % 128 == 0 && sample_threshold_only && plan.size() >= 2 && k <= 32 &&
                     sample.sample_tiles == (uint32_t)h->num_cu && (plan[1].r1 - plan[1].r0 + 255) / 256 >= (uint32_t)h->num_cu &&
                     (uint64_t)k * 50000ull > (uint64_t)sample.sample_tiles * plan_tile &&
@@ -1778,6 +1797,7 @@
             if (h16) tile_rows = narrow ? 128u : 256u;
             a.V16 = h->rows16; a.ld16 = h->ld16;
             if (i8c) { a.V16 = reinterpret_cast<const _Float16*>(bin_mfma ? (const int8_t*)h->bpm : (aug ? h->sq8a : (cosq ? h->sq8c : h->sq8))); a.ld16 = bin_mfma ? h->ld_bpm : (aug ? h->ld8a : h->ld8); }
+            if (sq7) a.V16 = reinterpret_cast<const _Float16*>(h->sq7);
             if (glds && !small && big_rows == 192 && metric == M_IP) tile_rows = 192u;
             a.qpad = qpad; a.nq = nq; a.nslab = nslab; a.ntiles = (s.r1 - s.r0 + tile_rows - 1) / tile_rows;
             if (s.sample_tiles) a.ntiles = s.sample_tiles;
@@ -1967,7 +1987,8 @@
         std::lock_guard<std::mutex> plk(h->prof_mu);
         h->prof.last_plan = (sample.sample_tiles ? 1u : 0u) | ((sample.sample_tiles && sample_threshold_only) ? 2u : 0u) | (i8c ? 4u : 0u) |
                             (plan_used_segments ? 8u : 0u) | (small ? 16u : 0u) | (fs ? 128u : 0u) | ((uint64_t)(plan.size() & 0xff) << 8) | (tiling << 16) |
-                            (sts ? (1ull << 24) : 0ull) | (plan_qs_sample ? (1ull << 25) : 0ull);
+                            (sts ? (1ull << 24) : 0ull) | (plan_qs_sample ? (1ull << 25) : 0ull) |
+                            (sq7 ? (1ull << 26) : 0ull);
     }
     FinalArgs fa{};
     fa.cand = w.cand; fa.count = w.count; fa.k = k; fa.out_k = out_k; fa.cap = w.cap; fa.metric = key_metric; fa.ip_form = ip_form;
@@ -2178,6 +2199,7 @@
         else hipLaunchKernelGGL(k_sq8_minmax<float>, dim3(gx, gy), dim3(256), 0, cur(h).stream, h->rows, h->ld, h->dim, h->n, h->sq8_mm, h->sq8_mm + h->dim);
     }
     if (r0 == 0) {
+        ++h->sq8_fit;
         LY_HIP(hipMemsetAsync(h->sq8_stats, 0, 16, cur(h).stream));
         hipLaunchKernelGGL(k_sq8_scales, dim3(gx), dim3(256), 0, cur(h).stream, h->sq8_mm, h->sq8_mm + h->dim, h->dim, h->sq8_mins, h->sq8_scales);
     }
@@ -2198,6 +2220,70 @@
     h->n_sq8 = h->n;
     return LYNSE_OK;
 }
+
+static int sq7_env() { return env_int("LYNSE_HIP_SQ7", -1); }
+static const uint64_t SQ7_AUTO_MIN_ROWS = 10000000ull;
+static bool sq7_wanted(const lynse_hip_flat* h, int metric, uint64_t nqc, bool masked) {
+    const int e = sq7_env();
+    if (e == 0 || metric != M_IP || masked || nqc <= 128 || nqc > QCHUNK || h->qchunk > QCHUNK) return false;
+    if (scan_variant() != 3 || qs_variant() < 1 || qs_variant() > 3 || !qs_width_ok(h->ld8, (h->dim + 127) / 128, false)) return false;
+    if (sts_env_on() || fused_sample_env() != 0) return false;
+    if (h->sq7_strikes.load() >= 3) return false;
+    return e == 1 || (h->rows_nonneg && h->n >= SQ7_AUTO_MIN_ROWS);
+}
+static void sq7_release_locked(lynse_hip_flat* h) {
+    if (h->sq7) (void)hipFree(h->sq7);
+    h->sq7 = nullptr; h->sq7_cap = 0; h->n_sq7 = 0;
+}
+static bool sq7_stale(const lynse_hip_flat* h) { return h->sq7 && (h->sq7_strikes.load() >= 3 || (!h->rows_nonneg && sq7_env() != 1)); }
+static int ensure_sq7_locked(lynse_hip_flat* h);
+static void sq7_sync_locked(lynse_hip_flat* h, int metric, uint64_t nqc, bool masked) {
+    if (sq7_stale(h)) sq7_release_locked(h);
+    if (!sq7_wanted(h, metric, nqc, masked) || !h->sq8 || h->n_sq8 != h->n || !h->sq8_finite) return;
+    if (ensure_sq7_locked(h) != LYNSE_OK) {
+        (void)hipGetLastError();
+        sq7_release_locked(h);
+        h->sq7_strikes.store(3);
+    }
+}
+static int ensure_sq7_locked(lynse_hip_flat* h) {
+    if (h->sq7 && h->n_sq7 == h->n && h->sq7_fit == h->sq8_fit) return LYNSE_OK;
+    if (!h->sq8 || h->n_sq8 != h->n) return set_error(LYNSE_ERR_INTERNAL, "the SQ7 copy is built from the fit of up-to-date SQ8 codes");
+    hipStream_t st = cur(h).stream;
+    const bool kept = h->sq7 != nullptr && h->sq7_cap >= h->n && h->sq7_fit == h->sq8_fit && h->n_sq7 < h->n;
+    if (h->sq7_cap < h->n) {
+        sq7_release_locked(h);
+        const uint64_t cap = std::max<uint64_t>(h->capacity, h->n);
+        LY_HIP(hipMalloc(&h->sq7, (size_t)cap * h->ld8 + 256));
+        h->sq7_cap = cap;
+    }
+    if (!h->sq7_scales) {
+        LY_HIP(hipMalloc(&h->sq7_scales, (size_t)h->dim * 4));
+        LY_HIP(hipMalloc(&h->sq7_stats, 16));
+    }
+    const uint64_t r0 = kept ? h->n_sq7 : 0;
+    if (r0 == 0) {
+        LY_HIP(hipMemsetAsync(h->sq7_stats, 0, 16, st));
+        hipLaunchKernelGGL(k_sq8_scales, dim3((h->dim + 255) / 256), dim3(256), 0, st, h->sq8_mm, h->sq8_mm + h->dim, h->dim, (float*)nullptr, h->sq7_scales, 127.0f);
+    }
+    const uint64_t nn = h->n - r0;
+    const uint32_t qgrid = (uint32_t)std::min<uint64_t>((nn + 3) / 4, (uint64_t)h->num_cu * 16);
+    if (is_f16(h)) hipLaunchKernelGGL(k_sq8_quantize<_Float16>, dim3(qgrid), dim3(256), 0, st, (const _Float16*)h->rows_h + r0 * h->ld16, h->ld16, h->dim, nn, h->sq8_mins, h->sq7_scales,
+                                      h->sq7 + r0 * h->ld8, h->ld8, (int*)nullptr, (int*)nullptr, h->sq7_stats, (const float*)nullptr, 0u, (const float*)nullptr, 1);
+    else hipLaunchKernelGGL(k_sq8_quantize<float>, dim3(qgrid), dim3(256), 0, st, h->rows + r0 * h->ld, h->ld, h->dim, nn, h->sq8_mins, h->sq7_scales,
+                            h->sq7 + r0 * h->ld8, h->ld8, (int*)nullptr, (int*)nullptr, h->sq7_stats, (const float*)nullptr, 0u, (const float*)nullptr, 1);
+    LY_HIP(hipGetLastError());
+    uint32_t qst[4] = {0, 0, 0, 0};
+    LY_HIP(hipMemcpyAsync(qst, h->sq7_stats, 16, hipMemcpyDeviceToHost, st));
+    LY_HIP(hipStreamSynchronize(st));
+    h->sq7_a1 = qst[0];
+    h->sq7_a2sq = qst[2];
+    memcpy(&h->sq7_eps2, &qst[3], 4);
+    h->n_sq7 = h->n;
+    h->sq7_fit = h->sq8_fit;
+    return LYNSE_OK;
+}
+static bool sq7_ready(const lynse_hip_flat* h) { return h->sq7 && h->n_sq7 == h->n && h->sq7_fit == h->sq8_fit && h->sq8 && h->n_sq8 == h->n; }
 
 static int ensure_sq8a_locked(lynse_hip_flat* h) {
     if (h->n_sq8a == h->n && h->sq8a) return LYNSE_OK;
@@ -2515,7 +2601,10 @@
         if (h->packed_only) return true;
         if (h->n_stats != h->n) return false;
         if (force_shadow && !shadow_ready(h)) return false;
-        if (i8c_eligible(h, metric, false, std::min<uint64_t>(nq, QCHUNK), caller_holds_exclusive, filtered)) return i8c_codes_ready(h, metric, std::min<uint64_t>(nq, QCHUNK), filtered);
+        if (i8c_eligible(h, metric, false, std::min<uint64_t>(nq, QCHUNK), caller_holds_exclusive, filtered)) {
+            if (sq7_stale(h) || (sq7_wanted(h, metric, std::min<uint64_t>(nq, QCHUNK), filtered) && h->sq8_finite && !sq7_ready(h))) return false;
+            return i8c_codes_ready(h, metric, std::min<uint64_t>(nq, QCHUNK), filtered);
+        }
         return shadow_ready(h) || small_path_ok(h, std::min<uint64_t>(nq, QCHUNK), (uint32_t)std::min<uint64_t>(k, h->n), metric, filtered);
     };
     auto needs_large_k = [&]() {
@@ -2726,7 +2815,7 @@
         bool i8c = i8c_eligible(h, metric, filtered && direct, nqc, caller_holds_exclusive, filtered && !direct);
         if (i8c) {
             const bool msk = filtered && !direct;
-            if (xlk.owns_lock()) LY_TRY(ensure_i8c_codes_locked(h, metric, nqc, msk));
+            if (xlk.owns_lock()) { LY_TRY(ensure_i8c_codes_locked(h, metric, nqc, msk)); sq7_sync_locked(h, metric, nqc, msk); }
             else if (!i8c_codes_ready(h, metric, nqc, msk)) i8c = false;
             if (i8c && !i8c_codes_finite(h, metric, nqc, msk)) { i8c_strike_counter(h, metric).store(-1); i8c = false; }
         }
@@ -2747,15 +2836,15 @@
             }
             continue;
         }
-        bool allow_sts = true;
+        bool allow_sts = true, allow_sq7 = true;
         for (int level = 0; level < 3; ++level) {
-            bool sampled = false, used_sts = false;
+            bool sampled = false, used_sts = false, used_sq7 = false;
             const size_t rows_b = (size_t)nqc * k * 8, dists_b = (size_t)nqc * k * 4;
             const bool staged = !on_device && rows_b + dists_b <= H_OUT_BYTES;
             uint64_t* r_dst = on_device ? out_rows + q0 * k : (staged ? reinterpret_cast<uint64_t*>(w.h_out) : nullptr);
             float* d_dst = on_device ? out_dists + q0 * k : (staged ? reinterpret_cast<float*>(w.h_out + rows_b) : nullptr);
             LY_TRY(run_chunk(h, nqc, kk, k, metric, level, st, &ev_used, &scan_events, &sampled, mask, direct ? h->g_ids32 : nullptr, i8c,
-                             r_dst, d_dst, on_device ? out_counts + q0 : nullptr, nullptr, qsrc, true, allow_sts, &used_sts));
+                             r_dst, d_dst, on_device ? out_counts + q0 : nullptr, nullptr, qsrc, true, allow_sts, &used_sts, allow_sq7, &used_sq7));
             if (!on_device && !staged) {
                 LY_HIP(hipMemcpyAsync(out_rows + q0 * k, w.out_rows, rows_b, out_kind, st));
                 LY_HIP(hipMemcpyAsync(out_dists + q0 * k, w.out_dists, dists_b, out_kind, st));
@@ -2774,6 +2863,12 @@
                 --level;
                 continue;
             }
+            if (used_sq7) {
+                allow_sq7 = false;
+                h->sq7_strikes.fetch_add(1);
+                --level;
+                continue;
+            }
             if (i8c) {
                 i8c = false;
                 i8c_add_strike(h, metric);
@@ -2797,8 +2892,8 @@
     return LYNSE_OK;
 }
 
-extern "C" int lynse_hip_flat_coarse_scores(lynse_hip_flat* h, const float* queries, uint64_t nq, int metric, int coarse,
-                                            float* out_scores, float* out_bound, int* out_form) {
+static int coarse_scores_impl(lynse_hip_flat* h, const float* queries, uint64_t nq, int metric, int coarse,
+                              float* out_scores, float* out_bound, int* out_form, bool want_sq7) {
     if (!h || !queries || !out_scores || !out_bound) return set_error(LYNSE_ERR_INVALID_ARGUMENT, "NULL argument");
     if (metric_additive(metric)) return metric_check(metric);
     if (metric < M_IP || metric > M_COS) return set_error(LYNSE_ERR_INVALID_ARGUMENT, "float metrics only");
@@ -2814,6 +2909,9 @@
     if (i8c) {
         LY_TRY(ensure_i8c_codes_locked(h, metric, nq));
         if (!i8c_codes_finite(h, metric, nq)) return set_error(LYNSE_ERR_UNSUPPORTED, "the shard holds non-finite values: no int8 pass");
+        if (want_sq7) sq7_sync_locked(h, metric, nq, false);
+        if (want_sq7 && !(sq7_wanted(h, metric, nq, false) && sq7_ready(h)))
+            return set_error(LYNSE_ERR_UNSUPPORTED, "no SQ7 scan for this shape (FLAT-IP, 129..256 queries, LYNSE_HIP_SQ7 not 0)");
     }
     Workspace& w = cur(h).ws;
     hipStream_t st = cur(h).stream;
@@ -2822,13 +2920,16 @@
     std::vector<std::pair<size_t, uint64_t>> scan_events;
     bool sampled = false;
     tl_coarse_dump = true;
-    const int rc = run_chunk(h, (uint32_t)nq, 1, 1, metric, 1, st, &ev_used, &scan_events, &sampled, nullptr, nullptr, i8c);
+    bool used_sq7 = false;
+    const int rc = run_chunk(h, (uint32_t)nq, 1, 1, metric, 1, st, &ev_used, &scan_events, &sampled, nullptr, nullptr, i8c,
+                             nullptr, nullptr, nullptr, nullptr, nullptr, false, true, nullptr, want_sq7, &used_sq7);
     tl_coarse_dump = false;
     LY_TRY(rc);
+    if (want_sq7 && !used_sq7) return set_error(LYNSE_ERR_INTERNAL, "the diagnostics chunk did not scan the SQ7 copy");
     LY_HIP(hipStreamSynchronize(st));
     const bool l2n = i8c && metric == M_L2 && l2_plain(h, nq, false);
     const bool aug = i8c && metric == M_L2 && !l2n, cosq = i8c && metric == M_COS;
-    if (out_form) *out_form = (i8c ? 1 : 0) | (aug ? 2 : 0) | (l2n ? 4 : 0) | (cosq ? 8 : 0);
+    if (out_form) *out_form = (i8c ? 1 : 0) | (aug ? 2 : 0) | (l2n ? 4 : 0) | (cosq ? 8 : 0) | (used_sq7 ? 16 : 0);
     const bool key_asc = metric_ascending((aug || cosq) ? (int)M_IP : metric);
     std::vector<uint64_t> keys(h->n);
     std::vector<float> m2(nq);
@@ -2842,6 +2943,21 @@
         }
         out_bound[q] = 0.5f * m2[q];
     }
+    return LYNSE_OK;
+}
+
+extern "C" int lynse_hip_flat_coarse_scores(lynse_hip_flat* h, const float* queries, uint64_t nq, int metric, int coarse,
+                                            float* out_scores, float* out_bound, int* out_form) {
+    return coarse_scores_impl(h, queries, nq, metric, coarse, out_scores, out_bound, out_form, false);
+}
+extern "C" int lynse_hip_flat_coarse_scores_sq7(lynse_hip_flat* h, const float* queries, uint64_t nq, float* out_scores, float* out_bound, int* out_form) {
+    return coarse_scores_impl(h, queries, nq, M_IP, 1, out_scores, out_bound, out_form, true);
+}
+extern "C" int lynse_hip_flat_sq7_state(lynse_hip_flat* h, uint64_t* out_rows, int* out_strikes) {
+    if (!h) return set_error(LYNSE_ERR_INVALID_ARGUMENT, "handle is NULL");
+    std::shared_lock<std::shared_mutex> lk(h->rw);
+    if (out_rows) *out_rows = h->sq7 ? h->n_sq7 : 0;
+    if (out_strikes) *out_strikes = h->sq7_strikes.load();
     return LYNSE_OK;
 }
 
@@ -2876,6 +2992,7 @@
     if (i8c_eligible(h, metric, false, nqc)) {
         LY_TRY(ensure_i8c_codes_locked(h, metric, nqc));
         if (!i8c_codes_finite(h, metric, nqc)) i8c_strike_counter(h, metric).store(-1);
+        else sq7_sync_locked(h, metric, nqc, false);
     }
     if (!i8c_eligible(h, metric, false, nqc) && !small_path_ok(h, nqc, 10, metric, false)) LY_TRY(ensure_shadow_locked(h));
     return LYNSE_OK;
@@ -2891,6 +3008,7 @@
     if (h->vn2) b += 2ull * (h->stats_capacity + 256) * 4;
     if (h->packed) b += h->packed_capacity * h->words * 8ull;
     if (h->sq8) b += h->sq8_cap * h->ld8 + 2ull * (h->sq8_cap + 256) * 4;
+    if (h->sq7) b += h->sq7_cap * h->ld8;
     if (h->sq8a) b += h->sq8a_cap * h->ld8a;
     if (h->sq8c) b += h->sq8c_cap * h->ld8;
     if (h->bpm) b += h->bpm_cap * h->ld_bpm;
@@ -3163,7 +3281,7 @@
     lynse_hip_flat* h = sc.h;
     {
         std::unique_lock<std::shared_mutex> lk(h->rw);
-        h->n = 0; h->n_stats = 0; h->n16 = 0; h->n_packed = 0; h->n_sq8 = 0; h->n_sq8a = 0; h->n_sq8c = 0; h->n_bpm = 0; h->i8c_strikes.store(0); h->i8c_strikes_l2.store(0); h->i8c_strikes_cos.store(0);
+        h->n = 0; h->n_stats = 0; h->n16 = 0; h->n_packed = 0; h->n_sq8 = 0; h->n_sq7 = 0; h->sq7_strikes.store(0); h->n_sq8a = 0; h->n_sq8c = 0; h->n_bpm = 0; h->i8c_strikes.store(0); h->i8c_strikes_l2.store(0); h->i8c_strikes_cos.store(0);
         h->amax = h->vmax = h->vmin = 0.f; h->sv = 1.f; h->cos_degenerate = 0; h->rows_integer = 0; h->rows_nonneg = 0;
         const uint32_t init[5] = {0u, 0u, 0x7f800000u, 0u, 0u};
         LY_TRY(use_device(h));
```
